# JARVIS-MoCap/JARVIS-HybridNet

Hardware: AMD Instinct MI355X
Metric: multi-view frames/s (12cam 1280x1024, 23kpt, 64^3 grid) (higher is better)
Workload: dtype f32; 1 GPU; BASELINE configs[2]: HybridNet 12-camera 1280x1024, 23 kpts, 64^3 grid, small/small; cameras=12, joints=23, grid=64, streams=3, parallelism=single GPU, 3 time batches in flight on 3 HIP streams, hipgraph=False

## Files before the change

include/jarvis_hip.h:

```cpp
#ifndef JARVIS_HIP_H
#define JARVIS_HIP_H
#include <stdint.h>

#ifdef __cplusplus
extern "C" {
#endif

#define JH_ABI_VERSION 4

const char* jh_last_error(void);
int jh_abi_version(void);

#define JH_PRECISION_DEFAULT (-1)
#define JH_PRECISION_F32 0
#define JH_PRECISION_BF16X3 1
#define JH_PRECISION_BF16X3_WIDE 2
int jh_set_precision(int mode);
int jh_get_precision(void);

typedef struct jh_params jh_params;
int jh_params_create(jh_params** out);
int jh_params_set(jh_params* p, const char* key, const float* host, int64_t numel);
void jh_params_destroy(jh_params* p);

typedef struct jh_efftrack jh_efftrack;
int jh_efftrack_create(const jh_params* p, const char* prefix, int model_size, int joints, int n,
                       int h, int w, int want_res1, jh_efftrack** out);
int jh_efftrack_forward(jh_efftrack* net, const float* x_dev, float* res1_dev, float* res2_dev,
                        void* stream);
int64_t jh_efftrack_launches(const jh_efftrack* net);
void jh_efftrack_destroy(jh_efftrack* net);

typedef struct jh_v2v jh_v2v;
int jh_v2v_create(const jh_params* p, const char* prefix, int joints, int t, int g, jh_v2v** out);
int jh_v2v_forward(jh_v2v* net, const float* x_dev, float* y_dev, void* stream);
void jh_v2v_destroy(jh_v2v* net);

int64_t jh_reproject_workspace_bytes(int cams, int joints, int hs, int grid_size);
int jh_reproject_forward(const float* heatmaps_padded_dev, int cams, int joints, int hs,
                         const int32_t* center3d_dev, const int32_t* center_hm_dev,
                         const float* cam_dev, const float* intr_dev, const float* dist_dev,
                         int grid_size, float grid_spacing, float* vol_dev, int32_t* idx_dev,
                         void* workspace_dev, int64_t workspace_bytes, void* stream);

int64_t jh_softargmax_workspace_bytes(int t, int joints, int gh);
int jh_softargmax(const float* v2v_out_dev, int t, int joints, int gh, float grid_spacing,
                  float roi_cube_size, const int32_t* center3d_dev, float* heatmap_final_dev,
                  float* points_dev, float* conf_dev, void* workspace_dev, int64_t workspace_bytes,
                  void* stream);

int jh_reproject_point(const float* points_dev, int npoints, int cams, const float* cam_dev,
                       const float* intr_dev, const float* dist_dev, float* uv_dev, void* stream);
int64_t jh_reconstruct_workspace_bytes(int cams);
int jh_reconstruct_point(const float* points2d_dev, const float* maxvals_dev, int cams,
                         const float* cam_dev, const float* intr_dev, const float* dist_dev,
                         float* point3d_dev, void* workspace_dev, int64_t workspace_bytes,
                         void* stream);

typedef struct jh_predictor jh_predictor;
typedef struct {
  int32_t num_cameras, num_joints;
  int32_t center_size;
  int32_t bbox;
  float roi_cube_size;
  float grid_spacing;
  int32_t center_model, kp_model;
  int32_t img_h, img_w;
  int32_t time_batch;
  int32_t time_batch_3d;
  int32_t cam_lo, cam_n;
  float mean[3], std[3];
  int32_t precision;
} jh_predictor_config;

int jh_predictor_create(const jh_params* center_params, const jh_params* hybrid_params,
                        const jh_predictor_config* cfg, jh_predictor** out);
void jh_predictor_destroy(jh_predictor* pr);
int64_t jh_predictor_launches(const jh_predictor* pr);
int64_t jh_predictor_device_bytes(const jh_predictor* pr);
int jh_predictor_precision(const jh_predictor* pr);

int jh_predictor_set_calibration(jh_predictor* pr, const float* cam_dev, const float* intr_dev,
                                 const float* dist_dev, void* stream);
int jh_predictor_set_calibration_frames(jh_predictor* pr, const float* cam_dev ,
                                        const float* intr_dev , const float* dist_dev ,
                                        void* stream);

int jh_predictor_stage_center(jh_predictor* pr, const float* frames_dev, float* det_dev,
                              void* stream);
int jh_predictor_stage_keypoints(jh_predictor* pr, const float* frames_dev,
                                 const float* det_all_dev, float* heat_dev, void* stream);
int jh_predictor_stage_3d(jh_predictor* pr, const float* heat_all_dev, int t0, float* points_dev,
                          float* conf_dev, int32_t* valid_dev, void* stream);
int jh_predictor_stage_keypoints_gathered(jh_predictor* pr, const void* frames_dev, int frames_u8,
                                          const float* det_gathered_dev, int n_blocks,
                                          float* heat_dev, void* stream);
int jh_predictor_stage_3d_blocks(jh_predictor* pr, const float* heat_blocks_dev, int n_blocks,
                                 int frames_per_block, int t_off, int t0, float* points_dev,
                                 float* conf_dev, int32_t* valid_dev, void* stream);
int jh_predictor_forward(jh_predictor* pr, const float* frames_dev, float* points_dev,
                         float* conf_dev, int32_t* valid_dev, void* stream);
int jh_predictor_set_graph_replay(jh_predictor* pr, int on);
int jh_predictor_graph_replay(const jh_predictor* pr);
int jh_predictor_stage_center_u8(jh_predictor* pr, const uint8_t* frames_dev, float* det_dev,
                                 void* stream);
int jh_predictor_stage_keypoints_u8(jh_predictor* pr, const uint8_t* frames_dev,
                                    const float* det_all_dev, float* heat_dev, void* stream);
int jh_predictor_forward_u8(jh_predictor* pr, const uint8_t* frames_dev, float* points_dev,
                            float* conf_dev, int32_t* valid_dev, void* stream);

#define JH_FRAME_RGB_F32 0
#define JH_FRAME_BGR_U8 1
#define JH_FRAME_I420 2
#define JH_FRAME_NV12 3
int jh_predictor_forward_yuv(jh_predictor* pr, const uint8_t* frames_dev, int format, float* points_dev,
                             float* conf_dev, int32_t* valid_dev, void* stream);

#define JH_YUV_BT601 0
#define JH_YUV_BT709 1
#define JH_YUV_LIMITED 0
#define JH_YUV_FULL 1
typedef struct jh_yuv_surface {
  int64_t image_stride;
  int64_t y_offset, y_pitch;
  int64_t u_offset, v_offset;
  int64_t c_pitch;
  int32_t c_step;
  int32_t matrix;
  int32_t range;
  int32_t reserved;
} jh_yuv_surface;
int jh_yuv_surface_check(const jh_yuv_surface* surface, int h, int w);
int jh_predictor_forward_surface(jh_predictor* pr, const uint8_t* frames_dev, const jh_yuv_surface* surface,
                                 const uint8_t* mask_dev, float* points_dev, float* conf_dev, int32_t* valid_dev,
                                 void* stream);

#define JH_SENSOR_MONO 0
#define JH_SENSOR_RGGB 1
#define JH_SENSOR_BGGR 2
#define JH_SENSOR_GRBG 3
#define JH_SENSOR_GBRG 4
typedef struct jh_sensor_surface {
  int64_t image_stride;
  int64_t offset, pitch;
  int32_t pattern;
  int32_t reserved;
} jh_sensor_surface;
int jh_sensor_surface_check(const jh_sensor_surface* surface, int h, int w);
int jh_predictor_forward_sensor(jh_predictor* pr, const uint8_t* frames_dev, const jh_sensor_surface* surface,
                                const uint8_t* mask_dev, float* points_dev, float* conf_dev, int32_t* valid_dev,
                                void* stream);

int jh_predictor_debug(jh_predictor* pr, float* center3d_f_dev, int32_t* center3d_i_dev,
                       int32_t* center_hm_dev, float* det_dev, void* stream);

int jh_predictor_forward_masked(jh_predictor* pr, const void* frames_dev, int format, const uint8_t* mask_dev,
                                float* points_dev, float* conf_dev, int32_t* valid_dev, void* stream);
int jh_predictor_stage_keypoints_masked(jh_predictor* pr, const void* frames_dev, int format,
                                        const float* det_all_dev, const uint8_t* mask_dev, float* heat_dev,
                                        void* stream);
int jh_predictor_stage_3d_masked(jh_predictor* pr, const float* heat_all_dev, int t0, const uint8_t* mask_dev,
                                 float* points_dev, float* conf_dev, int32_t* valid_dev, void* stream);
int jh_predictor_debug_mask(jh_predictor* pr, int32_t* n_active_dev, int32_t* num_cams_detect_dev, void* stream);

int jh_predictor_views2d(jh_predictor* pr, const float* heat_all_dev, int t0, const float* points_dev,
                         const uint8_t* mask_dev, int32_t* points2d_dev, float* conf2d_dev, float* reproj_dev,
                         float* err_dev, uint8_t* used_dev, void* stream);

#define JH_FRAME_SURFACE  4
#define JH_FRAME_SENSOR   5
int jh_predictor_forward_images(jh_predictor* pr, const void* const* images_host, int n_images, int format,
                                const jh_yuv_surface* yuv, const jh_sensor_surface* sensor, const uint8_t* mask_dev,
                                float* points_dev, float* conf_dev, int32_t* valid_dev, void* stream);

int jh_predictor_hybridnet_forward(jh_predictor* pr, const float* crops_dev,
                                   const int32_t* center_hm_dev, const int32_t* center3d_dev,
                                   float* heatmap_final_dev, float* heatmaps_padded_dev,
                                   float* points_dev, float* conf_dev, void* stream);

typedef struct jh_predictor2d jh_predictor2d;
int jh_predictor2d_create(const jh_params* center_params, const jh_params* kp_params,
                          const jh_predictor_config* cfg, jh_predictor2d** out);
void jh_predictor2d_destroy(jh_predictor2d* pr);
int jh_predictor2d_forward(jh_predictor2d* pr, const float* frames_dev, int32_t* points_dev,
                           float* conf_dev, int32_t* valid_dev, void* stream);
int jh_predictor2d_forward_u8(jh_predictor2d* pr, const uint8_t* frames_dev, int32_t* points_dev,
                              float* conf_dev, int32_t* valid_dev, void* stream);

int jh_predictor2d_forward_yuv(jh_predictor2d* pr, const uint8_t* frames_dev, int format, int32_t* points_dev,
                               float* conf_dev, int32_t* valid_dev, void* stream);
int jh_predictor2d_forward_surface(jh_predictor2d* pr, const uint8_t* frames_dev, const jh_yuv_surface* surface,
                                   int32_t* points_dev, float* conf_dev, int32_t* valid_dev, void* stream);
int jh_predictor2d_forward_sensor(jh_predictor2d* pr, const uint8_t* frames_dev, const jh_sensor_surface* surface,
                                  int32_t* points_dev, float* conf_dev, int32_t* valid_dev, void* stream);

int jh_predictor2d_forward_images(jh_predictor2d* pr, const void* const* images_host, int n_images, int format,
                                  const jh_yuv_surface* yuv, const jh_sensor_surface* sensor,
                                  int32_t* points_dev, float* conf_dev, int32_t* valid_dev, void* stream);

int jh_profile_begin(void);
int jh_profile_end(int* n_records);
int jh_profile_get(int i, char* name, int name_cap, double* ms, double* flops, double* bytes);

int jh_op_conv(int nd, int kind, int k, int stride, int pad, int cin, int cout,
               const float* w_host, const float* b_host, const float* x_dev, int n, int d, int h,
               int w, const float* gate_dev, int norm_act, float* y_dev, void* stream);
int jh_op_depthwise(int k, int c, const float* w_host, const float* x_dev, int n, int h, int w,
                    int norm_act, float* y_dev, void* stream);
int jh_op_depthwise_pool(int k, int c, const float* w_host, const float* x_dev, int n, int h, int w,
                         float* y_dev, float* pool_dev, void* stream);

int jh_op_yuv420_to_bgr(const uint8_t* frames_dev, int format, int n, int h, int w, uint8_t* out_bgr_dev,
                        void* stream);
int jh_op_yuv_surface_to_bgr(const uint8_t* frames_dev, const jh_yuv_surface* surface, int n, int h, int w,
                             uint8_t* out_bgr_dev, void* stream);
int jh_op_sensor_to_bgr(const uint8_t* frames_dev, const jh_sensor_surface* surface, int n, int h, int w,
                        uint8_t* out_bgr_dev, void* stream);

int64_t jh_joint_argmax_all_workspace_bytes(int n, int hh, int wh, int jp);
int jh_op_joint_argmax_all(const float* heat_dev, int n, int hh, int wh, int j, int jp, int32_t* idx_dev,
                           float* max_dev, void* workspace_dev, int64_t workspace_bytes, void* stream);

int jh_op_bifpn_node(int n_in, const int* modes, const float* weights, int act, int n, int c, int cout,
                     int h, int w, const float* x0_dev, const float* x1_dev, const float* x2_dev,
                     const float* dw_host, const float* pw_host, const float* bias_host, float* y_dev,
                     void* stream);

#ifdef __cplusplus
}
#endif
#endif
```

jarvis-hybridnet_amd/_native.py:

```python
import ctypes
import math
import os
from typing import NamedTuple

import torch

_HERE = os.path.dirname(os.path.abspath(__file__))
LIB_PATH = os.environ.get("JH_LIBRARY_PATH") or os.path.join(_HERE, "libjarvis_hip.so")
_lib = None

c_void_p, c_int, c_float, c_int64 = ctypes.c_void_p, ctypes.c_int, ctypes.c_float, ctypes.c_int64
c_char_p = ctypes.c_char_p


class PredictorConfig(ctypes.Structure):
    _fields_ = [("num_cameras", ctypes.c_int32), ("num_joints", ctypes.c_int32),
                ("center_size", ctypes.c_int32), ("bbox", ctypes.c_int32),
                ("roi_cube_size", c_float), ("grid_spacing", c_float),
                ("center_model", ctypes.c_int32), ("kp_model", ctypes.c_int32),
                ("img_h", ctypes.c_int32), ("img_w", ctypes.c_int32),
                ("time_batch", ctypes.c_int32), ("time_batch_3d", ctypes.c_int32),
                ("cam_lo", ctypes.c_int32),
                ("cam_n", ctypes.c_int32), ("mean", c_float * 3), ("std", c_float * 3),
                ("precision", ctypes.c_int32)]


class YuvSurfaceStruct(ctypes.Structure):
    _fields_ = [("image_stride", ctypes.c_int64), ("y_offset", ctypes.c_int64), ("y_pitch", ctypes.c_int64),
                ("u_offset", ctypes.c_int64), ("v_offset", ctypes.c_int64), ("c_pitch", ctypes.c_int64),
                ("c_step", ctypes.c_int32), ("matrix", ctypes.c_int32), ("range", ctypes.c_int32),
                ("reserved", ctypes.c_int32)]


assert ctypes.sizeof(YuvSurfaceStruct) == 64


class SensorSurfaceStruct(ctypes.Structure):
    _fields_ = [("image_stride", ctypes.c_int64), ("offset", ctypes.c_int64), ("pitch", ctypes.c_int64),
                ("pattern", ctypes.c_int32), ("reserved", ctypes.c_int32)]


assert ctypes.sizeof(SensorSurfaceStruct) == 32

ABI_VERSION = 4
assert ctypes.sizeof(PredictorConfig) == 84

_WORKSPACES = {}


def workspace(nbytes, device):
    key = (str(device), torch.cuda.current_stream(device).cuda_stream)
    bufs = _WORKSPACES.setdefault(key, [])
    if not bufs or bufs[-1].numel() < nbytes:
        bufs.append(torch.empty((max(int(nbytes), 256),), dtype=torch.uint8, device=device))
    return bufs[-1]


_SIGS = {
    "jh_last_error": (c_char_p, []),
    "jh_abi_version": (c_int, []),
    "jh_set_precision": (c_int, [c_int]),
    "jh_get_precision": (c_int, []),
    "jh_params_create": (c_int, [ctypes.POINTER(c_void_p)]),
    "jh_params_set": (c_int, [c_void_p, c_char_p, c_void_p, c_int64]),
    "jh_params_destroy": (None, [c_void_p]),
    "jh_efftrack_create": (c_int, [c_void_p, c_char_p, c_int, c_int, c_int, c_int, c_int, c_int,
                                   ctypes.POINTER(c_void_p)]),
    "jh_efftrack_forward": (c_int, [c_void_p, c_void_p, c_void_p, c_void_p, c_void_p]),
    "jh_efftrack_launches": (c_int64, [c_void_p]),
    "jh_efftrack_destroy": (None, [c_void_p]),
    "jh_v2v_create": (c_int, [c_void_p, c_char_p, c_int, c_int, c_int, ctypes.POINTER(c_void_p)]),
    "jh_v2v_forward": (c_int, [c_void_p, c_void_p, c_void_p, c_void_p]),
    "jh_v2v_destroy": (None, [c_void_p]),
    "jh_reproject_workspace_bytes": (c_int64, [c_int, c_int, c_int, c_int]),
    "jh_reproject_forward": (c_int, [c_void_p, c_int, c_int, c_int, c_void_p, c_void_p, c_void_p,
                                     c_void_p, c_void_p, c_int, c_float, c_void_p, c_void_p,
                                     c_void_p, c_int64, c_void_p]),
    "jh_softargmax_workspace_bytes": (c_int64, [c_int, c_int, c_int]),
    "jh_softargmax": (c_int, [c_void_p, c_int, c_int, c_int, c_float, c_float, c_void_p, c_void_p,
                              c_void_p, c_void_p, c_void_p, c_int64, c_void_p]),
    "jh_reproject_point": (c_int, [c_void_p, c_int, c_int, c_void_p, c_void_p, c_void_p, c_void_p,
                                   c_void_p]),
    "jh_reconstruct_workspace_bytes": (c_int64, [c_int]),
    "jh_reconstruct_point": (c_int, [c_void_p, c_void_p, c_int, c_void_p, c_void_p, c_void_p,
                                     c_void_p, c_void_p, c_int64, c_void_p]),
    "jh_predictor_create": (c_int, [c_void_p, c_void_p, ctypes.POINTER(PredictorConfig),
                                    ctypes.POINTER(c_void_p)]),
    "jh_predictor_destroy": (None, [c_void_p]),
    "jh_predictor_set_graph_replay": (c_int, [c_void_p, c_int]),
    "jh_predictor_graph_replay": (c_int, [c_void_p]),
    "jh_predictor_launches": (c_int64, [c_void_p]),
    "jh_predictor_device_bytes": (c_int64, [c_void_p]),
    "jh_predictor_precision": (c_int, [c_void_p]),
    "jh_predictor_set_calibration": (c_int, [c_void_p, c_void_p, c_void_p, c_void_p, c_void_p]),
    "jh_predictor_set_calibration_frames": (c_int, [c_void_p, c_void_p, c_void_p, c_void_p, c_void_p]),
    "jh_predictor_stage_center": (c_int, [c_void_p, c_void_p, c_void_p, c_void_p]),
    "jh_predictor_stage_keypoints": (c_int, [c_void_p, c_void_p, c_void_p, c_void_p, c_void_p]),
    "jh_predictor_stage_3d": (c_int, [c_void_p, c_void_p, c_int, c_void_p, c_void_p, c_void_p,
                                      c_void_p]),
    "jh_predictor_stage_keypoints_gathered": (c_int, [c_void_p, c_void_p, c_int, c_void_p, c_int, c_void_p,
                                                      c_void_p]),
    "jh_predictor_stage_3d_blocks": (c_int, [c_void_p, c_void_p, c_int, c_int, c_int, c_int, c_void_p,
                                             c_void_p, c_void_p, c_void_p]),
    "jh_profile_begin": (c_int, []),
    "jh_profile_end": (c_int, [ctypes.POINTER(c_int)]),
    "jh_profile_get": (c_int, [c_int, c_char_p, c_int, ctypes.POINTER(ctypes.c_double),
                               ctypes.POINTER(ctypes.c_double), ctypes.POINTER(ctypes.c_double)]),
    "jh_predictor_forward": (c_int, [c_void_p, c_void_p, c_void_p, c_void_p, c_void_p, c_void_p]),
    "jh_predictor_stage_center_u8": (c_int, [c_void_p, c_void_p, c_void_p, c_void_p]),
    "jh_predictor_stage_keypoints_u8": (c_int, [c_void_p, c_void_p, c_void_p, c_void_p, c_void_p]),
    "jh_predictor_forward_u8": (c_int, [c_void_p, c_void_p, c_void_p, c_void_p, c_void_p, c_void_p]),
    "jh_predictor_forward_yuv": (c_int, [c_void_p, c_void_p, c_int, c_void_p, c_void_p, c_void_p, c_void_p]),
    "jh_yuv_surface_check": (c_int, [ctypes.POINTER(YuvSurfaceStruct), c_int, c_int]),
    "jh_predictor_forward_surface": (c_int, [c_void_p, c_void_p, ctypes.POINTER(YuvSurfaceStruct), c_void_p, c_void_p,
                                             c_void_p, c_void_p, c_void_p]),
    "jh_predictor2d_forward_surface": (c_int, [c_void_p, c_void_p, ctypes.POINTER(YuvSurfaceStruct), c_void_p,
                                               c_void_p, c_void_p, c_void_p]),
    "jh_op_yuv_surface_to_bgr": (c_int, [c_void_p, ctypes.POINTER(YuvSurfaceStruct), c_int, c_int, c_int, c_void_p,
                                         c_void_p]),
    "jh_sensor_surface_check": (c_int, [ctypes.POINTER(SensorSurfaceStruct), c_int, c_int]),
    "jh_predictor_forward_sensor": (c_int, [c_void_p, c_void_p, ctypes.POINTER(SensorSurfaceStruct), c_void_p, c_void_p,
                                            c_void_p, c_void_p, c_void_p]),
    "jh_predictor2d_forward_sensor": (c_int, [c_void_p, c_void_p, ctypes.POINTER(SensorSurfaceStruct), c_void_p,
                                              c_void_p, c_void_p, c_void_p]),
    "jh_op_sensor_to_bgr": (c_int, [c_void_p, ctypes.POINTER(SensorSurfaceStruct), c_int, c_int, c_int, c_void_p,
                                    c_void_p]),
    "jh_predictor_forward_masked": (c_int, [c_void_p, c_void_p, c_int, c_void_p, c_void_p, c_void_p, c_void_p,
                                            c_void_p]),
    "jh_predictor_forward_images": (c_int, [c_void_p, ctypes.POINTER(c_void_p), c_int, c_int,
                                            ctypes.POINTER(YuvSurfaceStruct), ctypes.POINTER(SensorSurfaceStruct),
                                            c_void_p, c_void_p, c_void_p, c_void_p, c_void_p]),
    "jh_predictor2d_forward_images": (c_int, [c_void_p, ctypes.POINTER(c_void_p), c_int, c_int,
                                              ctypes.POINTER(YuvSurfaceStruct), ctypes.POINTER(SensorSurfaceStruct),
                                              c_void_p, c_void_p, c_void_p, c_void_p]),
    "jh_predictor_stage_keypoints_masked": (c_int, [c_void_p, c_void_p, c_int, c_void_p, c_void_p, c_void_p,
                                                    c_void_p]),
    "jh_predictor_stage_3d_masked": (c_int, [c_void_p, c_void_p, c_int, c_void_p, c_void_p, c_void_p, c_void_p,
                                             c_void_p]),
    "jh_predictor_debug_mask": (c_int, [c_void_p, c_void_p, c_void_p, c_void_p]),
    "jh_predictor_views2d": (c_int, [c_void_p, c_void_p, c_int] + [c_void_p] * 8),
    "jh_joint_argmax_all_workspace_bytes": (c_int64, [c_int, c_int, c_int, c_int]),
    "jh_op_joint_argmax_all": (c_int, [c_void_p, c_int, c_int, c_int, c_int, c_int, c_void_p, c_void_p, c_void_p,
                                       c_int64, c_void_p]),
    "jh_predictor2d_create": (c_int, [c_void_p, c_void_p, ctypes.POINTER(PredictorConfig),
                                      ctypes.POINTER(c_void_p)]),
    "jh_predictor2d_destroy": (None, [c_void_p]),
    "jh_predictor2d_forward": (c_int, [c_void_p] * 6),
    "jh_predictor2d_forward_u8": (c_int, [c_void_p] * 6),
    "jh_predictor2d_forward_yuv": (c_int, [c_void_p, c_void_p, c_int, c_void_p, c_void_p, c_void_p, c_void_p]),
    "jh_predictor_debug": (c_int, [c_void_p, c_void_p, c_void_p, c_void_p, c_void_p, c_void_p]),
    "jh_predictor_hybridnet_forward": (c_int, [c_void_p] * 9),
    "jh_op_conv": (c_int, [c_int] * 7 + [c_void_p, c_void_p, c_void_p] + [c_int] * 4 +
                   [c_void_p, c_int, c_void_p, c_void_p]),
    "jh_op_depthwise": (c_int, [c_int, c_int, c_void_p, c_void_p, c_int, c_int, c_int, c_int,
                                c_void_p, c_void_p]),
    "jh_op_depthwise_pool": (c_int, [c_int, c_int, c_void_p, c_void_p, c_int, c_int, c_int, c_void_p, c_void_p,
                                     c_void_p]),
    "jh_op_yuv420_to_bgr": (c_int, [c_void_p, c_int, c_int, c_int, c_int, c_void_p, c_void_p]),
    "jh_op_bifpn_node": (c_int, [c_int, ctypes.POINTER(c_int), ctypes.POINTER(c_float), c_int, c_int, c_int,
                                 c_int, c_int, c_int, c_void_p, c_void_p, c_void_p, c_void_p, c_void_p,
                                 c_void_p, c_void_p, c_void_p]),
}


def symbols():
    return sorted(_SIGS)


def lib():
    global _lib
    if _lib is None:
        if not os.path.isfile(LIB_PATH):
            raise RuntimeError(
                "jarvis_hybridnet_amd: %s is missing -- build it with "
                "`python -c 'import __graft_entry__ as g; g.build()'` (hipcc, gfx950). "
                "There is no CPU fallback." % LIB_PATH)
        handle = ctypes.CDLL(LIB_PATH)
        for name, (res, args) in _SIGS.items():
            fn = getattr(handle, name)
            fn.restype, fn.argtypes = res, args
        if handle.jh_abi_version() != ABI_VERSION:
            raise RuntimeError("libjarvis_hip.so ABI version mismatch")
        _lib = handle
    return _lib


FRAME_CODES = {"rgb": 0, "bgr": 1, "i420": 2, "nv12": 3, "surface": 4, "sensor": 5}
FRAME_FORMATS = {k: FRAME_CODES[k] for k in ("bgr", "i420", "nv12")}
YUV_FORMATS = ("i420", "nv12")
FRAME_SURFACE, FRAME_SENSOR = FRAME_CODES["surface"], FRAME_CODES["sensor"]


class Frames(NamedTuple):
    fmt: int
    height: int
    width: int
    layout: object
    lead: tuple
    data: object = None
    images: object = None

    @property
    def device(self):
        return self.data.device if self.images is None else self.images[0].device


def yuv_format(name):
    if name not in YUV_FORMATS:
        raise ValueError("frame_format must be one of %s, got %r" % (list(YUV_FORMATS), name))
    return name


def surface(layout):
    if layout is None:
        raise ValueError("surface must be a YuvSurface or a SensorSurface, got None")
    return layout


def check_layout(layout, frame_format=None, hw=None):
    if layout is None:
        return None
    from .sensor_surface import SensorSurface
    from .yuv_surface import YuvSurface
    if not isinstance(layout, (YuvSurface, SensorSurface)):
        raise ValueError("frame_layout must be a YuvSurface or a SensorSurface or None, got %r"
                         % (type(layout).__name__,))
    if frame_format in YUV_FORMATS:
        raise ValueError("frame_layout describes the bytes itself: do not combine it with frame_format=%r"
                         % (frame_format,))
    if hw is not None and (layout.height, layout.width) != tuple(hw):
        raise ValueError("frame_layout is %d x %d; this predictor is %d x %d" % (layout.height, layout.width, *hw))
    return layout


def describe_shape(shape, dtype, lead, frame_format=None, frame_layout=None, hw=None, error=ValueError,
                   in_place=False, at_least=False):
    if frame_format is not None and frame_format not in FRAME_FORMATS:
        raise ValueError("frame_format must be one of %s or None, got %r" % (sorted(FRAME_FORMATS), frame_format))
    layout = check_layout(frame_layout, frame_format, hw)
    H, W = hw if hw is not None else ("H", "W")
    hint = ""
    if layout is not None:
        from .sensor_surface import SensorSurface
# ... 223 lines not shown
```

jarvis-hybridnet_amd/_predictor.py:

```python
import collections
import ctypes

import torch

from . import _native as N
from . import arch


Views2D = collections.namedtuple("Views2D", "points2D confidences2D reprojections errors used")


class NativePredictor:

    def __init__(self, center_state, hybrid_state, *, num_cameras, num_joints, center_size, bbox,
                 roi_cube_size, grid_spacing, img_h, img_w, mean, std, center_model="small",
                 kp_model="small", time_batch=1, time_batch_3d=0, cam_lo=0, cam_n=None, precision=None):
        cam_n = num_cameras if cam_n is None else cam_n
        cfg = N.PredictorConfig(
            num_cameras, num_joints, center_size, bbox, float(roi_cube_size), float(grid_spacing),
            arch.SIZE_IDS[center_model], arch.SIZE_IDS[kp_model], img_h, img_w, time_batch,
            time_batch_3d, cam_lo, cam_n, (ctypes.c_float * 3)(*mean), (ctypes.c_float * 3)(*std),
            N.precision_id(precision))
        self.cfg = cfg
        self.T, self.C, self.Cloc, self.J = time_batch, num_cameras, cam_n, num_joints
        self.T3 = time_batch_3d if time_batch_3d > 0 else time_batch
        self.Jp = (num_joints + 7) // 8 * 8
        self.Hh = bbox // 2
        self.handle = ctypes.c_void_p()
        pc = N.Params(center_state) if center_state is not None else None
        ph = N.Params(hybrid_state)
        N.check(N.lib().jh_predictor_create(pc.handle if pc else None, ph.handle,
                                            ctypes.byref(cfg), ctypes.byref(self.handle)))
        self.precision = {v: k for k, v in N.PRECISIONS.items()}[N.lib().jh_predictor_precision(self.handle)]
        self.launches = N.lib().jh_predictor_launches(self.handle)
        self.device_bytes = N.lib().jh_predictor_device_bytes(self.handle)

    def close(self):
        if getattr(self, "handle", None) and N is not None and N._lib is not None:
            N.lib().jh_predictor_destroy(self.handle)
            self.handle = None

    __del__ = close

    @property
    def graph_replay(self):
        return bool(N.lib().jh_predictor_graph_replay(self.handle))

    @graph_replay.setter
    def graph_replay(self, on):
        N.check(N.lib().jh_predictor_set_graph_replay(self.handle, int(bool(on))))

    def set_calibration(self, cam, intr, dist):
        N.check(N.lib().jh_predictor_set_calibration(
            self.handle, N.ptr(N.dev(cam)), N.ptr(N.dev(intr)), N.ptr(N.dev(dist)), N.stream()))

    def set_calibration_frames(self, cam, intr, dist):
        form, cam, intr, dist = N.calibration((cam, intr, dist), self.T, self.C)
        if form != "frames":
            raise ValueError("set_calibration_frames takes (%d, %d, 4, 3) / (%d, %d, 3, 3) / (%d, %d, 1, 5) tensors; "
                             "got %s" % (self.T, self.C, self.T, self.C, self.T, self.C, tuple(cam.shape)))
        N.check(N.lib().jh_predictor_set_calibration_frames(
            self.handle, N.ptr(N.dev(cam)), N.ptr(N.dev(intr)), N.ptr(N.dev(dist)), N.stream()))

    def forward(self, frames, out=None, frame_format=None, camera_mask=None, frame_layout=None):
        return self._forward(self._describe(frames, frame_format, frame_layout), out,
                             N.camera_mask(camera_mask, (self.T, self.C)))

    def forward_images(self, frames, out=None, camera_mask=None):
        if len(frames.images) != self.T * self.C:
            raise ValueError("expected %d images (time_batch * num_cameras), got %d" % (self.T * self.C,
                                                                                         len(frames.images)))
        return self._forward(frames, out, N.camera_mask(camera_mask, (self.T, self.C)))

    def _describe(self, frames, frame_format=None, frame_layout=None):
        return N.describe_frames(frames, (self.T, self.Cloc), frame_format, frame_layout,
                                 (self.cfg.img_h, self.cfg.img_w), error=RuntimeError, in_place=True)

    def _forward(self, frames, out, mask):
        dev = frames.device
        if out is None:
            out = (torch.empty((self.T, self.J, 3), device=dev),
                   torch.empty((self.T, self.J), device=dev),
                   torch.empty((self.T,), device=dev, dtype=torch.int32))
        if mask is not None:
            mask = mask.to(dev, non_blocking=True)
        N.call_forward("jh_predictor", self.handle, frames, mask, out)
        if mask is not None and mask.is_cuda:
            mask.record_stream(torch.cuda.current_stream())
        return out

    def stage_center(self, frames, det):
        frames = self._describe(frames).data
        fn = N.lib().jh_predictor_stage_center_u8 if frames.dtype == torch.uint8 else \
            N.lib().jh_predictor_stage_center
        N.check(fn(self.handle, N.ptr(frames), N.ptr(det), N.stream()))

    def stage_keypoints(self, frames, det_all, heat, camera_mask=None):
        frames = self._describe(frames).data
        if camera_mask is not None:
            mask = self._device_mask(camera_mask)
            N.check(N.lib().jh_predictor_stage_keypoints_masked(
                self.handle, N.ptr(frames), int(frames.dtype == torch.uint8), N.ptr(det_all), N.ptr(mask), N.ptr(heat),
                N.stream()))
            return
        fn = N.lib().jh_predictor_stage_keypoints_u8 if frames.dtype == torch.uint8 else \
            N.lib().jh_predictor_stage_keypoints
        N.check(fn(self.handle, N.ptr(frames), N.ptr(det_all), N.ptr(heat), N.stream()))

    def _device_mask(self, camera_mask):
        if not (torch.is_tensor(camera_mask) and camera_mask.is_cuda and camera_mask.dtype == torch.uint8
                and camera_mask.is_contiguous() and tuple(camera_mask.shape) == (self.T, self.C)):
            raise ValueError("the staged calls take camera_mask as a contiguous (%d, %d) uint8 device tensor"
                             % (self.T, self.C))
        return camera_mask

    def stage_3d(self, heat_all, t0, points, conf, valid, camera_mask=None):
        if camera_mask is not None:
            mask = self._device_mask(camera_mask)
            N.check(N.lib().jh_predictor_stage_3d_masked(self.handle, N.ptr(heat_all), t0, N.ptr(mask), N.ptr(points),
                                                         N.ptr(conf), N.ptr(valid), N.stream()))
            return
        N.check(N.lib().jh_predictor_stage_3d(self.handle, N.ptr(heat_all), t0, N.ptr(points),
                                              N.ptr(conf), N.ptr(valid), N.stream()))

    def stage_keypoints_gathered(self, frames, det_gathered, n_blocks, heat):
        frames = self._describe(frames).data
        N.check(N.lib().jh_predictor_stage_keypoints_gathered(
            self.handle, N.ptr(frames), int(frames.dtype == torch.uint8), N.ptr(det_gathered), n_blocks,
            N.ptr(heat), N.stream()))

    def stage_3d_blocks(self, heat_blocks, n_blocks, frames_per_block, t_off, t0, points, conf, valid):
        N.check(N.lib().jh_predictor_stage_3d_blocks(
            self.handle, N.ptr(heat_blocks), n_blocks, frames_per_block, t_off, t0, N.ptr(points),
            N.ptr(conf), N.ptr(valid), N.stream()))

    def views2d(self, points, heat=None, t0=0, camera_mask=None, out=None):
        dev, T3 = points.device, self.T3
        if not (points.is_cuda and points.is_contiguous() and points.dtype == torch.float32
                and tuple(points.shape) == (T3, self.J, 3)):
            raise ValueError("points must be the contiguous (%d, %d, 3) float32 device tensor of the 3D stage" % (T3, self.J))
        if heat is not None and not (heat.is_cuda and heat.is_contiguous() and heat.dtype == torch.float32 and
                                     tuple(heat.shape) == (T3, self.C, self.Hh, self.Hh, self.Jp)):
            raise ValueError("heat must be a contiguous (%d, %d, %d, %d, %d) float32 device tensor"
                             % (T3, self.C, self.Hh, self.Hh, self.Jp))
        mask = N.camera_mask(camera_mask, (self.T, self.C))
        if mask is not None:
            mask = mask.to(dev, non_blocking=True)
        if out is None:
            out = Views2D(torch.empty((T3, self.C, self.J, 2), device=dev, dtype=torch.int32),
                          torch.empty((T3, self.C, self.J), device=dev),
                          torch.empty((T3, self.C, self.J, 2), device=dev),
                          torch.empty((T3, self.C, self.J), device=dev),
                          torch.empty((T3, self.C), device=dev, dtype=torch.uint8))
        N.check(N.lib().jh_predictor_views2d(self.handle, N.ptr(heat), int(t0), N.ptr(points), N.ptr(mask),
                                             *(N.ptr(t) for t in out), N.stream()))
        if mask is not None:
            mask.record_stream(torch.cuda.current_stream())
        return Views2D(*out)

    def debug(self, device):
        c3f = torch.empty((self.T, 3), device=device)
        c3i = torch.empty((self.T, 3), device=device, dtype=torch.int32)
        chm = torch.empty((self.T, self.C, 2), device=device, dtype=torch.int32)
        det = torch.empty((self.T, self.C, 3), device=device)
        N.check(N.lib().jh_predictor_debug(self.handle, N.ptr(c3f), N.ptr(c3i), N.ptr(chm),
                                           N.ptr(det), N.stream()))
        return dict(center3d=c3f, center3d_int=c3i, center_hm=chm, det=det)

    def debug_mask(self, device):
        n_act = torch.empty((self.T,), device=device, dtype=torch.int32)
        n_det = torch.empty((self.T,), device=device, dtype=torch.int32)
        N.check(N.lib().jh_predictor_debug_mask(self.handle, N.ptr(n_act), N.ptr(n_det), N.stream()))
        return dict(n_active=n_act, num_cams_detect=n_det)

    def hybridnet_forward(self, crops, center_hm, center3d, want_final=True, want_padded=True):
        dev = crops.device
        Gh = int(self.cfg.roi_cube_size / self.cfg.grid_spacing) // 2
        hs = self.Hh + 2
        final = torch.empty((self.T, self.J, Gh, Gh, Gh), device=dev) if want_final else None
        padded = torch.empty((self.T, self.C, self.J, hs, hs), device=dev) if want_padded else None
        pts = torch.empty((self.T, self.J, 3), device=dev)
        conf = torch.empty((self.T, self.J), device=dev)
        N.check(N.lib().jh_predictor_hybridnet_forward(
            self.handle, N.ptr(crops), N.ptr(center_hm), N.ptr(center3d), N.ptr(final),
            N.ptr(padded), N.ptr(pts), N.ptr(conf), N.stream()))
        return final, padded, pts, conf


class MultiStreamPredictor:

    def __init__(self, make_predictor, streams=3, timing=False):
        self.timing = timing
        self.preds = [make_predictor() for _ in range(streams)]
        self.streams = [torch.cuda.Stream() for _ in range(streams)]
        self.events = [None] * streams
        self._next = 0
        self._calib = None
        self._calib_of = [None] * streams

    def set_calibration(self, *calib):
        p0 = self.preds[0]
        form = N.calibration(calib, p0.T, p0.C)[0] if len(calib) == 3 and calib[0].dim() == 4 else "shared"
        key = (form,) + tuple((t.data_ptr(), t._version, tuple(t.shape)) for t in calib)
# ... 59 lines not shown
```

jarvis-hybridnet_amd/csrc/api.hip:

```cpp
#include <cstring>
#include <memory>
#include "../../include/jarvis_hip.h"
#include <cstdlib>
#include "nets.h"
#include "bifpn_node.h"
#include "camera_mask.h"
#include "views2d.h"

namespace jh {
static thread_local std::string g_err;
void set_error(const std::string& msg) { g_err = msg; }
}

using namespace jh;

struct jh_params { ParamMap map; };
struct jh_efftrack { EffTrackPlan plan; };
struct jh_v2v { V2VPlan plan; };

namespace {

struct Scratch {
  std::vector<void*> ptrs;
  ~Scratch() { for (void* p : ptrs) (void)hipFree(p); }
// ... 8 lines not shown
  }
};

struct Carver {
  char* base;
  size_t cap, off = 0;
  Carver(void* b, size_t c) : base(static_cast<char*>(b)), cap(c) {}
  template <typename T> T* take(size_t count) {
    const size_t at = off;
    off += (count * sizeof(T) + 255) / 256 * 256;
    return base ? reinterpret_cast<T*>(base + at) : nullptr;
  }
  void act(int N, int D, int H, int W, int C, Act* a) {
    a->N = N; a->D = D; a->H = H; a->W = W; a->C = C; a->Cp = cpad(C);
    a->p = take<float>(a->elems());
  }
  bool fits() const { return off <= cap; }
};

struct ReproWs { Act heat, vol; float2* coarse; };
static size_t carve_reproject(Carver& c, int cams, int joints, int hs, int g, ReproWs* w) {
  const int gh = g / 2;
  c.act(cams, 1, hs, hs, joints, &w->heat);
  c.act(1, g, g, g, joints, &w->vol);
  w->coarse = c.take<float2>((size_t)cams * gh * gh * gh);
  return c.off;
}
struct SoftWs { Act x; double* partial; int* pmax; };
static size_t carve_softargmax(Carver& c, int t, int joints, int gh, SoftWs* w) {
  c.act(t, gh, gh, gh, joints, &w->x);
  w->partial = c.take<double>((size_t)t * w->x.Cp * 4 * kLimbs);
  w->pmax = c.take<int>((size_t)t * w->x.Cp);
  return c.off;
}
struct ReconWs { float* det; int *c3i, *chm, *valid; };
static size_t carve_reconstruct(Carver& c, int cams, ReconWs* w) {
  w->det = c.take<float>((size_t)cams * 3);
  w->c3i = c.take<int>(3);
  w->chm = c.take<int>((size_t)cams * 2);
  w->valid = c.take<int>(1);
  return c.off;
}

__global__ void export_padded_kernel(const float* __restrict__ heat, float* __restrict__ out, int N,
                                     int J, int Jp, int Hh) {
  const int hs = Hh + 2;
  const size_t total = (size_t)N * J * hs * hs;
  for (size_t i = (size_t)blockIdx.x * blockDim.x + threadIdx.x; i < total;
       i += (size_t)gridDim.x * blockDim.x) {
    const int x = (int)(i % hs), y = (int)((i / hs) % hs);
    const int j = (int)((i / ((size_t)hs * hs)) % J);
    const size_t n = i / ((size_t)hs * hs * J);
    float v = 0.f;
    if (x >= 1 && y >= 1 && x <= Hh && y <= Hh)
      v = heat[((n * Hh + (y - 1)) * Hh + (x - 1)) * Jp + j];
    out[i] = v;
  }
}

__global__ void det_unblock_kernel(const float* __restrict__ src, float* __restrict__ dst, int T, int C,
                                   int cpb) {
  const int i = blockIdx.x * blockDim.x + threadIdx.x;
  if (i >= T * C * 3) return;
  const int k = i % 3, c = (i / 3) % C, t = i / (3 * C);
  dst[i] = src[(((size_t)(c / cpb) * T + t) * cpb + c % cpb) * 3 + k];
}

__global__ void set_cell_kernel(const void** cell, const void* value) { *cell = value; }
constexpr int kPtrChunk = 256;
struct PtrChunk { const void* p[kPtrChunk]; };
__global__ __launch_bounds__(kPtrChunk) void set_table_kernel(const void** table, int count, PtrChunk c) {
  const int i = threadIdx.x;
  if (i < count) table[i] = c.p[i];
}
__global__ void copy_out_kernel(const float* __restrict__ gp, const float* __restrict__ gc,
                                const int* __restrict__ gv, float* __restrict__ points,
                                float* __restrict__ conf, int* __restrict__ valid, int n_pts, int n_conf,
                                int n_valid) {
  const int i = blockIdx.x * blockDim.x + threadIdx.x;
  if (i < n_pts) points[i] = gp[i];
  if (i < n_conf) conf[i] = gc[i];
  if (valid && i < n_valid) valid[i] = gv[i];
}

__global__ void pack_det_kernel(const float* __restrict__ pts2d, const float* __restrict__ maxvals,
                                float* __restrict__ det, int C) {
  const int c = threadIdx.x;
  if (c < C) {
    det[c * 3 + 0] = pts2d[c];
    det[c * 3 + 1] = pts2d[C + c];
    det[c * 3 + 2] = maxvals[c];
  }
}

}

extern "C" {

const char* jh_last_error(void) { return g_err.c_str(); }
int jh_abi_version(void) { return JH_ABI_VERSION; }

int jh_set_precision(int mode) {
  JH_REQUIRE(mode == JH_PRECISION_F32 || mode == JH_PRECISION_BF16X3 || mode == JH_PRECISION_BF16X3_WIDE,
             "unknown precision mode");
  set_precision_mode(mode);
  return 0;
}
int jh_get_precision(void) { return precision_mode(); }

int jh_params_create(jh_params** out) {
  *out = new jh_params();
  return 0;
}
int jh_params_set(jh_params* p, const char* key, const float* host, int64_t numel) {
  JH_REQUIRE(p && key && host && numel >= 0, "bad argument");
  p->map[key] = std::vector<float>(host, host + numel);
  return 0;
}
void jh_params_destroy(jh_params* p) { delete p; }

int jh_efftrack_create(const jh_params* p, const char* prefix, int model_size, int joints, int n,
                       int h, int w, int want_res1, jh_efftrack** out) {
  JH_REQUIRE(p && out, "bad argument");
  std::unique_ptr<jh_efftrack> net(new jh_efftrack());
  if (net->plan.build(p->map, prefix ? prefix : "", model_size, joints, n, h, w, want_res1 != 0)) return 1;
  *out = net.release();
  return 0;
}
int jh_efftrack_forward(jh_efftrack* net, const float* x_dev, float* res1_dev, float* res2_dev,
                        void* stream) {
  hipStream_t s = static_cast<hipStream_t>(stream);
  JH_REQUIRE(net && x_dev && res2_dev, "bad argument");
  JH_REQUIRE(!res1_dev || net->plan.res1.p, "res1 requested from a network created with want_res1 = 0");
  if (launch_to_channel_last(x_dev, net->plan.input, s)) return 1;
  if (net->plan.run(s)) return 1;
  if (res1_dev && launch_from_channel_last(net->plan.res1, res1_dev, s)) return 1;
  return launch_from_channel_last(net->plan.heat, res2_dev, s);
}
int64_t jh_efftrack_launches(const jh_efftrack* net) { return (int64_t)net->plan.launches(); }
void jh_efftrack_destroy(jh_efftrack* net) { delete net; }

int jh_v2v_create(const jh_params* p, const char* prefix, int joints, int t, int g, jh_v2v** out) {
  JH_REQUIRE(p && out, "bad argument");
  std::unique_ptr<jh_v2v> net(new jh_v2v());
  if (net->plan.build(p->map, prefix ? prefix : "", joints, t, g)) return 1;
  *out = net.release();
  return 0;
}
int jh_v2v_forward(jh_v2v* net, const float* x_dev, float* y_dev, void* stream) {
  hipStream_t s = static_cast<hipStream_t>(stream);
  if (launch_to_channel_last(x_dev, net->plan.input, s)) return 1;
  if (net->plan.run(s)) return 1;
  return launch_from_channel_last(net->plan.output, y_dev, s);
}
void jh_v2v_destroy(jh_v2v* net) { delete net; }

int64_t jh_reproject_workspace_bytes(int cams, int joints, int hs, int grid_size) {
  Carver c(nullptr, 0);
  ReproWs w;
  return (int64_t)carve_reproject(c, cams, joints, hs, grid_size, &w);
}

int jh_reproject_forward(const float* heatmaps_padded_dev, int cams, int joints, int hs,
                         const int32_t* center3d_dev, const int32_t* center_hm_dev,
                         const float* cam_dev, const float* intr_dev, const float* dist_dev,
                         int grid_size, float grid_spacing, float* vol_dev, int32_t* idx_dev,
                         void* workspace_dev, int64_t workspace_bytes, void* stream) {
  hipStream_t s = static_cast<hipStream_t>(stream);
  JH_REQUIRE(workspace_dev && workspace_bytes >= 0, "workspace (see jh_reproject_workspace_bytes)");
  JH_REQUIRE(grid_size > 0 && grid_size % 2 == 0, "grid size must be even");
  Carver c(workspace_dev, (size_t)workspace_bytes);
  ReproWs w;
  carve_reproject(c, cams, joints, hs, grid_size, &w);
  JH_REQUIRE(c.fits(), "workspace smaller than jh_reproject_workspace_bytes()");
  if (launch_to_channel_last(heatmaps_padded_dev, w.heat, s)) return 1;
  if (launch_reproject(cam_dev, intr_dev, dist_dev, 0, center3d_dev, center_hm_dev, w.heat.p, w.coarse,
                       w.vol.p, idx_dev, 1, cams, grid_size, grid_spacing, hs, w.heat.Cp,
                       1, 0, s)) return 1;
  return launch_from_channel_last(w.vol, vol_dev, s);
}

int64_t jh_softargmax_workspace_bytes(int t, int joints, int gh) {
  Carver c(nullptr, 0);
  SoftWs w;
  return (int64_t)carve_softargmax(c, t, joints, gh, &w);
}

int jh_softargmax(const float* v2v_out_dev, int t, int joints, int gh, float grid_spacing,
                  float roi_cube_size, const int32_t* center3d_dev, float* heatmap_final_dev,
                  float* points_dev, float* conf_dev, void* workspace_dev, int64_t workspace_bytes,
                  void* stream) {
  hipStream_t s = static_cast<hipStream_t>(stream);
  JH_REQUIRE(workspace_dev && workspace_bytes >= 0, "workspace (see jh_softargmax_workspace_bytes)");
  Carver c(workspace_dev, (size_t)workspace_bytes);
  SoftWs w;
  carve_softargmax(c, t, joints, gh, &w);
  JH_REQUIRE(c.fits(), "workspace smaller than jh_softargmax_workspace_bytes()");
  if (launch_to_channel_last(v2v_out_dev, w.x, s)) return 1;
  return launch_softargmax(w.x.p, center3d_dev, w.partial, w.pmax, points_dev, conf_dev,
                           heatmap_final_dev, t, joints, w.x.Cp, gh, grid_spacing, roi_cube_size, s);
}

int jh_reproject_point(const float* points_dev, int npoints, int cams, const float* cam_dev,
                       const float* intr_dev, const float* dist_dev, float* uv_dev, void* stream) {
  return launch_project_points(points_dev, cam_dev, intr_dev, dist_dev, uv_dev, npoints, cams,
                               static_cast<hipStream_t>(stream));
}

int64_t jh_reconstruct_workspace_bytes(int cams) {
  Carver c(nullptr, 0);
  ReconWs w;
  return (int64_t)carve_reconstruct(c, cams, &w);
}

int jh_reconstruct_point(const float* points2d_dev, const float* maxvals_dev, int cams,
                         const float* cam_dev, const float* intr_dev, const float* dist_dev,
                         float* point3d_dev, void* workspace_dev, int64_t workspace_bytes,
                         void* stream) {
  hipStream_t s = static_cast<hipStream_t>(stream);
  JH_REQUIRE(cams >= 1 && cams <= 64, "at most 64 cameras");
  JH_REQUIRE(workspace_dev && workspace_bytes >= 0, "workspace (see jh_reconstruct_workspace_bytes)");
  Carver c(workspace_dev, (size_t)workspace_bytes);
  ReconWs w;
  carve_reconstruct(c, cams, &w);
  JH_REQUIRE(c.fits(), "workspace smaller than jh_reconstruct_workspace_bytes()");
  hipLaunchKernelGGL(pack_det_kernel, dim3(1), dim3(64), 0, s, points2d_dev, maxvals_dev, w.det, cams);
  JH_CHECK_HIP(hipGetLastError());
  return launch_triangulate(w.det, cam_dev, intr_dev, dist_dev, 0, point3d_dev, w.c3i, w.chm, w.valid, 1,
                            cams, 1.f, 1.f, 1.f, 0, 1 << 20, 1 << 20, s);
}

}

#define JH_PROF(name, flops, bytes, call)                      \
  do {                                                         \
    Profiler& _pf = profiler();                                \
    if (_pf.on) _pf.begin(name, flops, bytes, s);              \
    if (call) return 1;                                        \
    if (_pf.on) _pf.end(s);                                    \
  } while (0)

static int yuv_surface_check(const jh_yuv_surface* sp, int h, int w) {
  JH_REQUIRE(sp, "null jh_yuv_surface");
  const jh_yuv_surface& q = *sp;
  JH_REQUIRE(h > 0 && w > 0 && h % 2 == 0 && w % 2 == 0, "YUV 4:2:0 frames need an even, positive height and width");
  JH_REQUIRE(q.c_step == 1 || q.c_step == 2, "jh_yuv_surface.c_step must be 1 (planar) or 2 (semi-planar)");
  JH_REQUIRE(q.y_pitch >= w, "jh_yuv_surface.y_pitch is smaller than the width");
  JH_REQUIRE(q.c_pitch >= (int64_t)(w / 2) * q.c_step, "jh_yuv_surface.c_pitch is smaller than a chroma row");
  JH_REQUIRE(q.y_offset >= 0 && q.u_offset >= 0 && q.v_offset >= 0 && q.image_stride >= 0,
             "jh_yuv_surface offsets must not be negative");
  if (q.c_step == 2) {
    JH_REQUIRE(q.u_offset - q.v_offset == 1 || q.v_offset - q.u_offset == 1,
               "jh_yuv_surface: semi-planar U and V are neighbouring bytes");
    JH_REQUIRE((q.u_offset < q.v_offset ? q.u_offset : q.v_offset) % 2 == 0 && q.c_pitch % 2 == 0,
               "jh_yuv_surface: a semi-planar chroma pair starts at an even offset and c_pitch is even");
  }
  const __int128 y_end = (__int128)q.y_offset + (__int128)(h - 1) * q.y_pitch + w;
  const __int128 c_span = (__int128)(h / 2 - 1) * q.c_pitch + (__int128)(w / 2 - 1) * q.c_step + 1;
  JH_REQUIRE(y_end <= q.image_stride && q.u_offset + c_span <= q.image_stride && q.v_offset + c_span <= q.image_stride,
             "jh_yuv_surface: a plane ends beyond image_stride");
  JH_REQUIRE(q.matrix == JH_YUV_BT601 || q.matrix == JH_YUV_BT709, "jh_yuv_surface.matrix: unknown");
  JH_REQUIRE(q.range == JH_YUV_LIMITED || q.range == JH_YUV_FULL, "jh_yuv_surface.range: unknown");
  JH_REQUIRE(q.reserved == 0, "jh_yuv_surface.reserved must be 0");
  return 0;
}

static int frame_source(const jh_yuv_surface* sp, int h, int w, FrameSource* out) {
  if (yuv_surface_check(sp, h, w)) return 1;
  const jh_yuv_surface& q = *sp;
  static const int k[2][2][6] = {{{16, 1220542, 1673527, 2116026, -409993, -852492},
                                  {0, 1048576, 1470104, 1858077, -360853, -748826}},
                                 {{16, 1220945, 1879825, 2215014, -223607, -558796},
                                  {0, 1048576, 1651297, 1945738, -196424, -490864}}};
  const int* c = k[q.matrix][q.range];
  SrcDesc<kSrcYuvSurface> a;
  a.image_stride = q.image_stride; a.y_offset = q.y_offset; a.y_pitch = q.y_pitch;
  a.u_offset = q.u_offset; a.v_offset = q.v_offset; a.c_pitch = q.c_pitch; a.c_step = q.c_step;
  a.pair = q.c_step == 2 && q.image_stride % 2 == 0;
  a.y0 = c[0]; a.cy = c[1]; a.cvr = c[2]; a.cub = c[3]; a.cug = c[4]; a.cvg = c[5];
  out->fmt = kSrcYuvSurface; out->desc = a;
  return 0;
}

static int sensor_surface_check(const jh_sensor_surface* sp, int h, int w) {
  JH_REQUIRE(sp, "null jh_sensor_surface");
  const jh_sensor_surface& q = *sp;
  JH_REQUIRE(h > 0 && w > 0, "raw sensor frames need a positive height and width");
  JH_REQUIRE(q.pattern >= JH_SENSOR_MONO && q.pattern <= JH_SENSOR_GBRG, "jh_sensor_surface.pattern: unknown");
  if (q.pattern != JH_SENSOR_MONO)
    JH_REQUIRE(h % 2 == 0 && w % 2 == 0 && h >= 4 && w >= 4,
               "Bayer frames need an even height and width of at least 4");
  JH_REQUIRE(q.pitch >= w, "jh_sensor_surface.pitch is smaller than the width");
  JH_REQUIRE(q.offset >= 0, "jh_sensor_surface.offset must not be negative");
  JH_REQUIRE((__int128)q.offset + (__int128)(h - 1) * q.pitch + w <= q.image_stride,
             "jh_sensor_surface: the image ends beyond image_stride");
  JH_REQUIRE(q.reserved == 0, "jh_sensor_surface.reserved must be 0");
  return 0;
}

static int frame_source(const jh_sensor_surface* sp, int h, int w, FrameSource* out) {
  if (sensor_surface_check(sp, h, w)) return 1;
  const jh_sensor_surface& q = *sp;
  SrcDesc<kSrcSensor> a;
  a.image_stride = q.image_stride; a.offset = q.offset; a.pitch = q.pitch; a.pattern = q.pattern; a.h = h; a.w = w;
  out->fmt = kSrcSensor; out->desc = a;
  return 0;
}

static_assert(JH_FRAME_RGB_F32 == kSrcRgbF32 && JH_FRAME_BGR_U8 == kSrcBgrU8 && JH_FRAME_I420 == kSrcI420 &&
                  JH_FRAME_NV12 == kSrcNV12, "frame format codes of the C ABI are preprocess.h's SRC");

static FrameSource fixed_source(int format) {
  FrameSource fs;
  fs.fmt = format;
  return fs;
}
static int frame_source(int format, int h, int w, FrameSource* out) {
  JH_REQUIRE(format >= JH_FRAME_RGB_F32 && format <= JH_FRAME_NV12, "frame format");
  if (format == JH_FRAME_I420 || format == JH_FRAME_NV12)
    JH_REQUIRE(h % 2 == 0 && w % 2 == 0, "YUV 4:2:0 frames need an even height and width");
  *out = fixed_source(format);
  return 0;
}

static_assert(JH_FRAME_SURFACE == kSrcYuvSurface && JH_FRAME_SENSOR == kSrcSensor,
              "frame format codes of the C ABI are preprocess.h's SRC");

static int images_source(int format, const jh_yuv_surface* yuv, const jh_sensor_surface* sensor, int h, int w,
                         FrameSource* out) {
  JH_REQUIRE(format >= JH_FRAME_RGB_F32 && format <= JH_FRAME_SENSOR, "forward_images: unknown frame format");
  JH_REQUIRE((yuv != nullptr) == (format == JH_FRAME_SURFACE),
             "forward_images: JH_FRAME_SURFACE, and no other format, comes with a jh_yuv_surface");
  JH_REQUIRE((sensor != nullptr) == (format == JH_FRAME_SENSOR),
             "forward_images: JH_FRAME_SENSOR, and no other format, comes with a jh_sensor_surface");
  if (format == JH_FRAME_SURFACE) {
    if (frame_source(yuv, h, w, out)) return 1;
    auto& d = std::get<SrcDesc<kSrcYuvSurface>>(out->desc);
    d.pair = d.c_step == 2;
  } else if (format == JH_FRAME_SENSOR) {
    if (frame_source(sensor, h, w, out)) return 1;
  } else if (frame_source(format, h, w, out)) {
    return 1;
  }
  out->per_image = true;
  return 0;
}

static int upload_images(Scratch& mem, const void*** table, const void* const* images_host, int n_images, int want,
                         int format, hipStream_t s) {
  JH_REQUIRE(images_host, "forward_images: null image table");
  JH_REQUIRE(n_images == want, "forward_images: n_images must be time_batch * num_cameras (2D predictor: time_batch)");
  for (int i = 0; i < n_images; ++i) {
    JH_REQUIRE(images_host[i], "forward_images: a null image pointer");
    JH_REQUIRE(format != JH_FRAME_RGB_F32 || reinterpret_cast<uintptr_t>(images_host[i]) % 4 == 0,
               "forward_images: an fp32 image that is not 4-byte aligned");
  }
  if (!*table) {
    hipStreamCaptureStatus cs = hipStreamCaptureStatusNone;
    (void)hipStreamIsCapturing(s, &cs);
    JH_REQUIRE(cs == hipStreamCaptureStatusNone, "the first forward_images call of a predictor allocates its pointer "
               "table: make it outside a stream capture");
    if (mem.get(reinterpret_cast<void**>(table), (size_t)want * sizeof(void*))) return 1;
  }
  for (int off = 0; off < n_images; off += kPtrChunk) {
    PtrChunk c{};
    const int count = n_images - off < kPtrChunk ? n_images - off : kPtrChunk;
    for (int i = 0; i < count; ++i) c.p[i] = images_host[off + i];
    hipLaunchKernelGGL(set_table_kernel, dim3(1), dim3(kPtrChunk), 0, s, *table + off, count, c);
  }
  JH_CHECK_HIP(hipGetLastError());
  return 0;
}

struct jh_predictor {
  jh_predictor_config cfg{};
  int T3 = 0;
  int T = 0, C = 0, Cloc = 0, J = 0, Jp = 0, B = 0, Hh = 0, G = 0, Gh = 0, hs = 0;
  std::unique_ptr<EffTrackPlan> center, kp;
  std::unique_ptr<V2VPlan> v2v;
  Scratch mem;
  float *cam = nullptr, *intr = nullptr, *dist = nullptr;
  float *cam_f = nullptr, *intr_f = nullptr, *dist_f = nullptr;
  int calib_fs = 0;
  const float* cam_at(int t0) const { return calib_fs ? cam_f + (size_t)t0 * calib_fs * 12 : cam; }
  const float* intr_at(int t0) const { return calib_fs ? intr_f + (size_t)t0 * calib_fs * 9 : intr; }
  const float* dist_at(int t0) const { return calib_fs ? dist_f + (size_t)t0 * calib_fs * 5 : dist; }
  float *det_all = nullptr, *c3f = nullptr;
  int *c3i_[2] = {nullptr, nullptr}, *chm_[2] = {nullptr, nullptr}, *valid_[2] = {nullptr, nullptr};
  int slot = 0;
  int* c3i_cur() const { return c3i_[slot]; }
  int* chm_cur() const { return chm_[slot]; }
  int* valid_cur() const { return valid_[slot]; }
  float2* coarse = nullptr;
  double* sa_partial = nullptr;
  int* sa_max = nullptr;
  int use_graph = 0;
  const void** frames_cell = nullptr;
  const void* const* cur_cell = nullptr;
  const void** frames_table = nullptr;
  const void* const* cell_for(const FrameSource& fs) const { return fs.per_image ? frames_table : cur_cell; }
  float *g_points = nullptr, *g_conf = nullptr;
  hipStream_t gstream = nullptr;
  static constexpr int kGraphFmts = kSrcSensor + 1;
  struct GraphSlot { hipGraphExec_t exec = nullptr; FrameSource src; int calib_fs = 0; };
  GraphSlot gslot[4 * kGraphFmts];
  unsigned char* mask_buf = nullptr;
  const unsigned char* mask_cur = nullptr;
  int *n_active = nullptr, *n_detect = nullptr;
  float* v2d_max = nullptr;
  int* v2d_idx = nullptr;
  ~jh_predictor() {
    for (auto& g : gslot) if (g.exec) (void)hipGraphExecDestroy(g.exec);
    if (gstream) (void)hipStreamDestroy(gstream);
  }

  int run_3d(const float* heat_all, int t0, float* heatmap_final, float* points, float* conf,
             hipStream_t s, const HeatLayout* layout = nullptr) {
    const double g3 = (double)G * G * G;
    if (mask_cur) {
      JH_PROF("reproject_gather_masked", 0.0, 4.0 * T3 * ((double)C * Hh * Hh * J + g3 * J),
              launch_reproject_masked(cam_at(t0), intr_at(t0), dist_at(t0), calib_fs, c3i_cur() + t0 * 3,
                                      chm_cur() + t0 * C * 2, heat_all, coarse, v2v->input.p, nullptr, T3, C, G,
                                      cfg.grid_spacing, hs, Jp,
                                      0, 1, mask_cur + (size_t)t0 * C, s, layout));
    } else {
    JH_PROF("reproject_gather", 0.0, 4.0 * T3 * ((double)C * Hh * Hh * J + g3 * J),
            launch_reproject(cam_at(t0), intr_at(t0), dist_at(t0), calib_fs, c3i_cur() + t0 * 3,
                             chm_cur() + t0 * C * 2, heat_all, coarse, v2v->input.p, nullptr, T3, C, G,
                             cfg.grid_spacing, hs, Jp,
                             0, 1, s, layout));
    }
    if (v2v->run(s)) return 1;
    JH_PROF("softargmax", 0.0, 4.0 * T3 * (g3 / 8) * J,
            launch_softargmax(v2v->output.p, c3i_cur() + t0 * 3, sa_partial, sa_max, points, conf,
                              heatmap_final, T3, J, Jp, Gh, cfg.grid_spacing, cfg.roi_cube_size, s));
    return 0;
  }
};

extern "C" {

int jh_predictor_create(const jh_params* center_params, const jh_params* hybrid_params,
                        const jh_predictor_config* cfg, jh_predictor** out) {
  JH_REQUIRE(hybrid_params && cfg && out, "bad argument");
  std::unique_ptr<jh_predictor> pr(new jh_predictor());
  pr->cfg = *cfg;
  pr->T = cfg->time_batch; pr->C = cfg->num_cameras; pr->Cloc = cfg->cam_n;
  pr->T3 = cfg->time_batch_3d > 0 ? cfg->time_batch_3d : cfg->time_batch;
  JH_REQUIRE(pr->T3 <= pr->T, "time_batch_3d must not exceed time_batch");
  pr->J = cfg->num_joints; pr->Jp = cpad(cfg->num_joints);
  pr->B = cfg->bbox; pr->Hh = cfg->bbox / 2; pr->hs = cfg->bbox / 2 + 2;
  pr->G = (int)(cfg->roi_cube_size / cfg->grid_spacing);
  pr->Gh = pr->G / 2;
  JH_REQUIRE(pr->T >= 1 && pr->C >= 1 && pr->C <= 64, "time batch / camera count");
  JH_REQUIRE(cfg->cam_lo >= 0 && cfg->cam_n >= 1 && cfg->cam_lo + cfg->cam_n <= pr->C, "camera range");
  JH_REQUIRE(pr->G % 4 == 0, "ROI_CUBE_SIZE / GRID_SPACING must be a multiple of 4");
  const int N = pr->T * pr->Cloc;
  const int node_rows = pr->T >= 8 ? 1 : 0;
  const int norm_kb = node_rows && JH_ENV_KNOB("JH_NODE_ROWS") != 0 ? 64 : 0;
  JH_REQUIRE(cfg->precision >= JH_PRECISION_DEFAULT && cfg->precision <= JH_PRECISION_BF16X3_WIDE,
             "jh_predictor_config.precision: unknown mode");
  const int precision = cfg->precision == JH_PRECISION_DEFAULT ? precision_mode() : cfg->precision;
  pr->cfg.precision = precision;
  if (center_params) {
    pr->center.reset(new EffTrackPlan());
    pr->center->precision = precision;
    pr->center->node_rows = node_rows;
    pr->center->norm_block_kb = norm_kb;
    if (pr->center->build(center_params->map, "", cfg->center_model, 1, N, cfg->center_size,
                          cfg->center_size)) return 1;
  }
  pr->kp.reset(new EffTrackPlan());
  pr->kp->precision = precision;
  pr->kp->node_rows = node_rows;
  pr->kp->norm_block_kb = norm_kb;
  if (pr->kp->build(hybrid_params->map, "effTrack.", cfg->kp_model, pr->J, N, pr->B, pr->B)) return 1;
  pr->v2v.reset(new V2VPlan());
  pr->v2v->precision = precision;
  pr->v2v->norm_block_kb = norm_kb;
  if (pr->v2v->build(hybrid_params->map, "v2vNet.", pr->J, pr->T3, pr->G)) return 1;
  auto& m = pr->mem;
  const int T = pr->T, C = pr->C;
  if (m.get(reinterpret_cast<void**>(&pr->cam), (size_t)C * 12 * sizeof(float))) return 1;
  if (m.get(reinterpret_cast<void**>(&pr->intr), (size_t)C * 9 * sizeof(float))) return 1;
  if (m.get(reinterpret_cast<void**>(&pr->dist), (size_t)C * 5 * sizeof(float))) return 1;
  if (m.get(reinterpret_cast<void**>(&pr->det_all), (size_t)T * C * 3 * sizeof(float))) return 1;
  if (m.get(reinterpret_cast<void**>(&pr->c3f), (size_t)T * 3 * sizeof(float))) return 1;
  for (int k = 0; k < 2; ++k) {
    if (m.get(reinterpret_cast<void**>(&pr->c3i_[k]), (size_t)T * 3 * sizeof(int))) return 1;
    if (m.get(reinterpret_cast<void**>(&pr->chm_[k]), (size_t)T * C * 2 * sizeof(int))) return 1;
    if (m.get(reinterpret_cast<void**>(&pr->valid_[k]), (size_t)T * sizeof(int))) return 1;
  }
  if (m.get(reinterpret_cast<void**>(&pr->coarse),
            (size_t)pr->T3 * C * pr->Gh * pr->Gh * pr->Gh * sizeof(float2))) return 1;
  {
    const size_t pb = (size_t)T * pr->Jp * 4 * kLimbs * sizeof(double), mb = (size_t)T * pr->Jp * sizeof(int);
    if (m.get(reinterpret_cast<void**>(&pr->sa_partial), pb + mb)) return 1;
    pr->sa_max = reinterpret_cast<int*>(reinterpret_cast<char*>(pr->sa_partial) + pb);
  }
  for (int k = 0; k < 2; ++k) JH_CHECK_HIP(hipMemset(pr->valid_[k], 0, (size_t)T * sizeof(int)));
  if (m.get(reinterpret_cast<void**>(&pr->mask_buf), (size_t)T * C)) return 1;
  if (m.get(reinterpret_cast<void**>(&pr->n_active), (size_t)T * sizeof(int))) return 1;
  if (m.get(reinterpret_cast<void**>(&pr->n_detect), (size_t)T * sizeof(int))) return 1;
  JH_CHECK_HIP(hipMemset(pr->mask_buf, 1, (size_t)T * C));
  JH_CHECK_HIP(hipMemset(pr->n_active, 0, (size_t)T * sizeof(int)));
  JH_CHECK_HIP(hipMemset(pr->n_detect, 0, (size_t)T * sizeof(int)));
  const int knob = JH_ENV_KNOB("JH_GRAPH");
  pr->use_graph = knob >= 0 ? (knob != 0) : (pr->T == 1);
  if (pr->Cloc == pr->C && pr->T3 == pr->T && pr->center) {
    if (m.get(reinterpret_cast<void**>(&pr->frames_cell), 256)) return 1;
    if (m.get(reinterpret_cast<void**>(&pr->g_points), (size_t)T * pr->J * 3 * sizeof(float))) return 1;
    if (m.get(reinterpret_cast<void**>(&pr->g_conf), (size_t)T * pr->J * sizeof(float))) return 1;
  } else {
    pr->use_graph = 0;
  }
  JH_CHECK_HIP(hipDeviceSynchronize());
  *out = pr.release();
  return 0;
}

void jh_predictor_destroy(jh_predictor* pr) { delete pr; }

int jh_predictor_set_graph_replay(jh_predictor* pr, int on) {
  JH_REQUIRE(pr, "bad argument");
  JH_REQUIRE(!on || pr->frames_cell, "graph replay needs a predictor that owns all cameras and CenterDetect");
  pr->use_graph = on != 0;
  return 0;
}
int jh_predictor_graph_replay(const jh_predictor* pr) { return pr ? pr->use_graph : 0; }

int64_t jh_predictor_launches(const jh_predictor* pr) {
  return (int64_t)((pr->center ? pr->center->launches() : 0) + pr->kp->launches() +
                   pr->v2v->launches());
}
int jh_predictor_precision(const jh_predictor* pr) { return pr ? pr->cfg.precision : -1; }

int64_t jh_predictor_device_bytes(const jh_predictor* pr) {
  return (int64_t)((pr->center ? pr->center->device_bytes() : 0) + pr->kp->device_bytes() +
                   pr->v2v->device_bytes());
}

int jh_predictor_set_calibration(jh_predictor* pr, const float* cam_dev, const float* intr_dev,
                                 const float* dist_dev, void* stream) {
  hipStream_t s = static_cast<hipStream_t>(stream);
  JH_CHECK_HIP(hipMemcpyAsync(pr->cam, cam_dev, (size_t)pr->C * 12 * sizeof(float), hipMemcpyDeviceToDevice, s));
  JH_CHECK_HIP(hipMemcpyAsync(pr->intr, intr_dev, (size_t)pr->C * 9 * sizeof(float), hipMemcpyDeviceToDevice, s));
  JH_CHECK_HIP(hipMemcpyAsync(pr->dist, dist_dev, (size_t)pr->C * 5 * sizeof(float), hipMemcpyDeviceToDevice, s));
  pr->calib_fs = 0;
  return 0;
}

int jh_predictor_set_calibration_frames(jh_predictor* pr, const float* cam_dev, const float* intr_dev,
                                        const float* dist_dev, void* stream) {
  hipStream_t s = static_cast<hipStream_t>(stream);
  JH_REQUIRE(pr, "jh_predictor_set_calibration_frames: null predictor");
  JH_REQUIRE(cam_dev && intr_dev && dist_dev, "jh_predictor_set_calibration_frames: null calibration pointer");
  const size_t rows = (size_t)pr->T * pr->C;
  if (!pr->cam_f) {
    hipStreamCaptureStatus cs = hipStreamCaptureStatusNone;
    (void)hipStreamIsCapturing(s, &cs);
    JH_REQUIRE(cs == hipStreamCaptureStatusNone, "the first jh_predictor_set_calibration_frames call of a predictor "
               "allocates its per-frame calibration: make it outside a stream capture");
    float* base = nullptr;
    if (pr->mem.get(reinterpret_cast<void**>(&base), rows * 26 * sizeof(float))) return 1;
    pr->intr_f = base + rows * 12;
    pr->dist_f = base + rows * 21;
    pr->cam_f = base;
  }
  JH_CHECK_HIP(hipMemcpyAsync(pr->cam_f, cam_dev, rows * 12 * sizeof(float), hipMemcpyDeviceToDevice, s));
  JH_CHECK_HIP(hipMemcpyAsync(pr->intr_f, intr_dev, rows * 9 * sizeof(float), hipMemcpyDeviceToDevice, s));
  JH_CHECK_HIP(hipMemcpyAsync(pr->dist_f, dist_dev, rows * 5 * sizeof(float), hipMemcpyDeviceToDevice, s));
  pr->calib_fs = pr->C;
  return 0;
}

static int stage_center_impl(jh_predictor* pr, const void* frames_dev, const FrameSource& fs, float* det_dev,
                             void* stream) {
  hipStream_t s = static_cast<hipStream_t>(stream);
  JH_REQUIRE(pr->center, "predictor was created without CenterDetect weights");
  const int N = pr->T * pr->Cloc, S = pr->cfg.center_size;
  if (pr->center->stem_fusable) {
    StemSource& src = pr->center->stem_src;
    src.mode = 1; src.frames = frames_dev; src.frames_cell = pr->cell_for(fs); src.source = fs;
    src.H = pr->cfg.img_h; src.W = pr->cfg.img_w;
    for (int i = 0; i < 3; ++i) { src.mean[i] = pr->cfg.mean[i]; src.stdv[i] = pr->cfg.std[i]; }
    pr->center->set_stem_traffic((double)N * S * S * (4.0 * fs.px_bytes() + pr->center->stem_channels()));
  } else {
    JH_PROF("preprocess_resize", 0.0, (double)N * S * S * (4.0 * fs.px_bytes() + 3 * 4),
            launch_preprocess_resize(frames_dev, fs, pr->center->input.p, N, pr->cfg.img_h,
                                     pr->cfg.img_w, S, pr->cfg.mean, pr->cfg.std, s, pr->cell_for(fs)));
  }
  if (pr->center->run(s)) return 1;
  const Act& h = pr->center->heat;
  JH_PROF("center_argmax", 0.0, 4.0 * N * h.H * h.W,
          launch_center_argmax(h.p, det_dev, N, h.H, h.W, h.Cp, s));
  return 0;
}

int jh_predictor_stage_center(jh_predictor* pr, const float* frames_dev, float* det_dev,
                              void* stream) {
  return stage_center_impl(pr, frames_dev, fixed_source(kSrcRgbF32), det_dev, stream);
}
int jh_predictor_stage_center_u8(jh_predictor* pr, const uint8_t* frames_dev, float* det_dev,
                                 void* stream) {
  return stage_center_impl(pr, frames_dev, fixed_source(kSrcBgrU8), det_dev, stream);
}

static int stage_keypoints_impl(jh_predictor* pr, const void* frames_dev, const FrameSource& fs,
                                const float* det_all_dev, float* heat_dev, void* stream,
                                int det_blocks = 1, bool next_centre_set = false) {
  hipStream_t s = static_cast<hipStream_t>(stream);
  const auto& c = pr->cfg;
  if (next_centre_set) pr->slot ^= 1;
  if (det_blocks > 1) {
    JH_REQUIRE(pr->C % det_blocks == 0, "cameras must divide evenly over the detection blocks");
    const int n = pr->T * pr->C * 3;
    hipLaunchKernelGGL(det_unblock_kernel, dim3((n + 255) / 256), dim3(256), 0, s, det_all_dev, pr->det_all,
                       pr->T, pr->C, pr->C / det_blocks);
    JH_CHECK_HIP(hipGetLastError());
    det_all_dev = pr->det_all;
  }
  const float sx2 = (float)((double)c.img_w / (double)c.center_size) * 2.f;
  const float sy2 = (float)((double)c.img_h / (double)c.center_size) * 2.f;
  if (pr->mask_cur) {
    JH_PROF("triangulate_masked", 0.0, 0.0,
            launch_triangulate_masked(det_all_dev, pr->cam_at(0), pr->intr_at(0), pr->dist_at(0), pr->calib_fs, pr->c3f,
                                      pr->c3i_cur(), pr->chm_cur(), pr->valid_cur(), pr->T, pr->C, sx2, sy2, 255.f,
                                      pr->B / 2,
                                      c.img_w, c.img_h, pr->mask_cur, pr->n_active, pr->n_detect, s));
  } else {
  JH_PROF("triangulate", 0.0, 0.0,
          launch_triangulate(det_all_dev, pr->cam_at(0), pr->intr_at(0), pr->dist_at(0), pr->calib_fs, pr->c3f,
                             pr->c3i_cur(), pr->chm_cur(), pr->valid_cur(), pr->T, pr->C, sx2, sy2, 255.f, pr->B / 2,
                             c.img_w, c.img_h, s));
  }
  if (det_all_dev != pr->det_all)
    JH_CHECK_HIP(hipMemcpyAsync(pr->det_all, det_all_dev, (size_t)pr->T * pr->C * 3 * sizeof(float),
                                hipMemcpyDeviceToDevice, s));
  if (pr->kp->stem_fusable) {
    StemSource& src = pr->kp->stem_src;
    src.mode = 2; src.frames = frames_dev; src.frames_cell = pr->cell_for(fs); src.source = fs;
    src.center_hm = pr->chm_cur(); src.Cloc = pr->Cloc; src.C = pr->C; src.cam0 = c.cam_lo;
    src.H = c.img_h; src.W = c.img_w;
    for (int i = 0; i < 3; ++i) { src.mean[i] = c.mean[i]; src.stdv[i] = c.std[i]; }
    pr->kp->set_stem_traffic((double)pr->T * pr->Cloc * pr->B * pr->B * (fs.px_bytes() + pr->kp->stem_channels()));
  } else {
    JH_PROF("preprocess_crop", 0.0, (double)pr->T * pr->Cloc * pr->B * pr->B * (fs.px_bytes() + 12.0),
            launch_preprocess_crop(frames_dev, fs, pr->chm_cur(), pr->kp->input.p, pr->T, pr->Cloc, pr->C,
                                   c.cam_lo, c.img_h, c.img_w, pr->B, c.mean, c.std, s, pr->cell_for(fs)));
  }
  if (pr->kp->run(s)) return 1;
  if (heat_dev && heat_dev != pr->kp->heat.p)
    JH_CHECK_HIP(hipMemcpyAsync(heat_dev, pr->kp->heat.p, pr->kp->heat.bytes(),
                                hipMemcpyDeviceToDevice, s));
  return 0;
}

int jh_predictor_stage_keypoints(jh_predictor* pr, const float* frames_dev,
                                 const float* det_all_dev, float* heat_dev, void* stream) {
  return stage_keypoints_impl(pr, frames_dev, fixed_source(kSrcRgbF32), det_all_dev, heat_dev, stream, 1, true);
}
int jh_predictor_stage_keypoints_u8(jh_predictor* pr, const uint8_t* frames_dev,
                                    const float* det_all_dev, float* heat_dev, void* stream) {
  return stage_keypoints_impl(pr, frames_dev, fixed_source(kSrcBgrU8), det_all_dev, heat_dev, stream, 1, true);
}

int jh_predictor_stage_keypoints_gathered(jh_predictor* pr, const void* frames_dev, int frames_u8,
                                          const float* det_gathered_dev, int n_blocks, float* heat_dev,
                                          void* stream) {
  JH_REQUIRE(n_blocks >= 1, "block count");
  return stage_keypoints_impl(pr, frames_dev, fixed_source(frames_u8 ? kSrcBgrU8 : kSrcRgbF32), det_gathered_dev, heat_dev,
                              stream, n_blocks, true);
}

int jh_predictor_stage_3d(jh_predictor* pr, const float* heat_all_dev, int t0, float* points_dev,
                          float* conf_dev, int32_t* valid_dev, void* stream) {
  hipStream_t s = static_cast<hipStream_t>(stream);
  JH_REQUIRE(t0 >= 0 && t0 + pr->T3 <= pr->T, "frame range of the 3D stage");
  if (pr->run_3d(heat_all_dev, t0, nullptr, points_dev, conf_dev, s)) return 1;
  if (valid_dev)
    JH_CHECK_HIP(hipMemcpyAsync(valid_dev, pr->valid_cur() + t0, (size_t)pr->T3 * sizeof(int),
                                hipMemcpyDeviceToDevice, s));
  return 0;
}

int jh_predictor_stage_3d_blocks(jh_predictor* pr, const float* heat_blocks_dev, int n_blocks,
                                 int frames_per_block, int t_off, int t0, float* points_dev,
                                 float* conf_dev, int32_t* valid_dev, void* stream) {
  hipStream_t s = static_cast<hipStream_t>(stream);
  JH_REQUIRE(t0 >= 0 && t0 + pr->T3 <= pr->T, "frame range of the 3D stage");
  JH_REQUIRE(n_blocks >= 1 && pr->C % n_blocks == 0, "cameras must divide evenly over the blocks");
  JH_REQUIRE(t_off >= 0 && t_off + pr->T3 <= frames_per_block, "frame range inside a block");
  HeatLayout lay;
  const size_t plane = (size_t)pr->Hh * pr->Hh * pr->Jp;
  lay.cams_per_block = pr->C / n_blocks;
  lay.frame_stride = (size_t)lay.cams_per_block * plane;
  lay.block_stride = (size_t)frames_per_block * lay.frame_stride;
  if (pr->run_3d(heat_blocks_dev + (size_t)t_off * lay.frame_stride, t0, nullptr, points_dev, conf_dev, s,
                 &lay)) return 1;
  if (valid_dev)
    JH_CHECK_HIP(hipMemcpyAsync(valid_dev, pr->valid_cur() + t0, (size_t)pr->T3 * sizeof(int),
                                hipMemcpyDeviceToDevice, s));
  return 0;
}

static int forward_eager(jh_predictor* pr, const void* frames_dev, const FrameSource& fs, float* points_dev,
                         float* conf_dev, int32_t* valid_dev, void* stream) {
  if (stage_center_impl(pr, frames_dev, fs, pr->det_all, stream)) return 1;
  if (stage_keypoints_impl(pr, frames_dev, fs, pr->det_all, nullptr, stream)) return 1;
  return jh_predictor_stage_3d(pr, pr->kp->heat.p, 0, points_dev, conf_dev, valid_dev, stream);
}

static int forward_graph(jh_predictor* pr, const void* frames_dev, const FrameSource& fs, float* points_dev,
                         float* conf_dev, int32_t* valid_dev, hipStream_t s) {
  jh_predictor::GraphSlot& slot = pr->gslot[fs.fmt + (pr->mask_cur ? jh_predictor::kGraphFmts : 0) +
                                            (fs.per_image ? 2 * jh_predictor::kGraphFmts : 0)];
  if (slot.exec && (slot.src != fs || slot.calib_fs != pr->calib_fs)) {
    JH_CHECK_HIP(hipStreamSynchronize(s));
    (void)hipGraphExecDestroy(slot.exec);
    slot.exec = nullptr;
  }
  if (!slot.exec) {
    hipGraph_t g = nullptr;
    if (!pr->gstream) JH_CHECK_HIP(hipStreamCreateWithFlags(&pr->gstream, hipStreamNonBlocking));
    JH_CHECK_HIP(hipStreamBeginCapture(pr->gstream, hipStreamCaptureModeRelaxed));
    pr->cur_cell = pr->frames_cell;
    const int rc = forward_eager(pr, nullptr, fs, pr->g_points, pr->g_conf, nullptr, pr->gstream);
    pr->cur_cell = nullptr;
    const hipError_t e = hipStreamEndCapture(pr->gstream, &g);
    if (rc) { if (g) (void)hipGraphDestroy(g); return 1; }
    JH_CHECK_HIP(e);
    const hipError_t ei = hipGraphInstantiate(&slot.exec, g, nullptr, nullptr, 0);
    (void)hipGraphDestroy(g);
    if (ei != hipSuccess) slot.exec = nullptr;
    JH_CHECK_HIP(ei);
    slot.src = fs;
    slot.calib_fs = pr->calib_fs;
  }
  if (!fs.per_image) hipLaunchKernelGGL(set_cell_kernel, dim3(1), dim3(1), 0, s, pr->frames_cell, frames_dev);
  JH_CHECK_HIP(hipGetLastError());
  JH_CHECK_HIP(hipGraphLaunch(slot.exec, s));
  const int n_pts = pr->T * pr->J * 3;
  hipLaunchKernelGGL(copy_out_kernel, dim3((n_pts + 255) / 256), dim3(256), 0, s, pr->g_points, pr->g_conf,
                     pr->valid_[0], points_dev, conf_dev, valid_dev, n_pts, pr->T * pr->J, pr->T);
  JH_CHECK_HIP(hipGetLastError());
  return 0;
}

static int forward_unmasked(jh_predictor* pr, const void* frames_dev, const FrameSource& fs, float* points_dev,
                            float* conf_dev, int32_t* valid_dev, void* stream) {
  JH_REQUIRE(pr->Cloc == pr->C && pr->cfg.cam_lo == 0, "forward needs all cameras local");
  JH_REQUIRE(pr->T3 == pr->T, "forward needs time_batch_3d == time_batch");
  JH_REQUIRE(frames_dev && points_dev && conf_dev, "null frame / output pointer");
  pr->slot = 0;
  hipStreamCaptureStatus cs = hipStreamCaptureStatusNone;
  if (pr->use_graph && !profiler().on) (void)hipStreamIsCapturing(static_cast<hipStream_t>(stream), &cs);
  if (!pr->use_graph || profiler().on || cs != hipStreamCaptureStatusNone)
    return forward_eager(pr, frames_dev, fs, points_dev, conf_dev, valid_dev, stream);
  return forward_graph(pr, frames_dev, fs, points_dev, conf_dev, valid_dev, static_cast<hipStream_t>(stream));
}

static int forward_impl(jh_predictor* pr, const void* frames_dev, const FrameSource& fs, float* points_dev,
                        float* conf_dev, int32_t* valid_dev, void* stream,
                        const unsigned char* mask_dev = nullptr) {
  if (!mask_dev) return forward_unmasked(pr, frames_dev, fs, points_dev, conf_dev, valid_dev, stream);
  JH_CHECK_HIP(hipMemcpyAsync(pr->mask_buf, mask_dev, (size_t)pr->T * pr->C, hipMemcpyDeviceToDevice,
                              static_cast<hipStream_t>(stream)));
  pr->mask_cur = pr->mask_buf;
  const int rc = forward_unmasked(pr, frames_dev, fs, points_dev, conf_dev, valid_dev, stream);
  pr->mask_cur = nullptr;
  return rc;
}
int jh_predictor_forward(jh_predictor* pr, const float* frames_dev, float* points_dev,
                         float* conf_dev, int32_t* valid_dev, void* stream) {
  return forward_impl(pr, frames_dev, fixed_source(kSrcRgbF32), points_dev, conf_dev, valid_dev, stream);
}
int jh_predictor_forward_u8(jh_predictor* pr, const uint8_t* frames_dev, float* points_dev,
                            float* conf_dev, int32_t* valid_dev, void* stream) {
  return forward_impl(pr, frames_dev, fixed_source(kSrcBgrU8), points_dev, conf_dev, valid_dev, stream);
}

int jh_predictor_forward_yuv(jh_predictor* pr, const uint8_t* frames_dev, int format, float* points_dev,
                             float* conf_dev, int32_t* valid_dev, void* stream) {
  JH_REQUIRE(format == JH_FRAME_I420 || format == JH_FRAME_NV12, "jh_predictor_forward_yuv: format must be "
             "JH_FRAME_I420 or JH_FRAME_NV12");
  JH_REQUIRE(pr, "bad argument");
  FrameSource fs;
  if (frame_source(format, pr->cfg.img_h, pr->cfg.img_w, &fs)) return 1;
  return forward_impl(pr, frames_dev, fs, points_dev, conf_dev, valid_dev, stream);
}

int jh_yuv_surface_check(const jh_yuv_surface* surface, int h, int w) { return yuv_surface_check(surface, h, w); }

int jh_predictor_forward_surface(jh_predictor* pr, const uint8_t* frames_dev, const jh_yuv_surface* surface,
                                 const uint8_t* mask_dev, float* points_dev, float* conf_dev, int32_t* valid_dev,
                                 void* stream) {
  JH_REQUIRE(pr, "bad argument");
  FrameSource fs;
  if (frame_source(surface, pr->cfg.img_h, pr->cfg.img_w, &fs)) return 1;
  return forward_impl(pr, frames_dev, fs, points_dev, conf_dev, valid_dev, stream, mask_dev);
}

int jh_sensor_surface_check(const jh_sensor_surface* surface, int h, int w) {
  return sensor_surface_check(surface, h, w);
}

int jh_predictor_forward_sensor(jh_predictor* pr, const uint8_t* frames_dev, const jh_sensor_surface* surface,
                                const uint8_t* mask_dev, float* points_dev, float* conf_dev, int32_t* valid_dev,
                                void* stream) {
  JH_REQUIRE(pr, "bad argument");
  FrameSource fs;
  if (frame_source(surface, pr->cfg.img_h, pr->cfg.img_w, &fs)) return 1;
  return forward_impl(pr, frames_dev, fs, points_dev, conf_dev, valid_dev, stream, mask_dev);
}

int jh_predictor_forward_masked(jh_predictor* pr, const void* frames_dev, int format, const uint8_t* mask_dev,
                                float* points_dev, float* conf_dev, int32_t* valid_dev, void* stream) {
  JH_REQUIRE(pr, "bad argument");
  JH_REQUIRE(format >= JH_FRAME_RGB_F32 && format <= JH_FRAME_NV12, "jh_predictor_forward_masked: unknown frame format");
  FrameSource fs;
  if (frame_source(format, pr->cfg.img_h, pr->cfg.img_w, &fs)) return 1;
  return forward_impl(pr, frames_dev, fs, points_dev, conf_dev, valid_dev, stream, mask_dev);
}

int jh_predictor_forward_images(jh_predictor* pr, const void* const* images_host, int n_images, int format,
                                const jh_yuv_surface* yuv, const jh_sensor_surface* sensor, const uint8_t* mask_dev,
                                float* points_dev, float* conf_dev, int32_t* valid_dev, void* stream) {
  JH_REQUIRE(pr, "bad argument");
  JH_REQUIRE(pr->Cloc == pr->C && pr->cfg.cam_lo == 0, "forward needs all cameras local");
  FrameSource fs;
  if (images_source(format, yuv, sensor, pr->cfg.img_h, pr->cfg.img_w, &fs)) return 1;
  if (upload_images(pr->mem, &pr->frames_table, images_host, n_images, pr->T * pr->C, format,
                    static_cast<hipStream_t>(stream))) return 1;
  return forward_impl(pr, pr->frames_table, fs, points_dev, conf_dev, valid_dev, stream, mask_dev);
}

int jh_predictor_stage_keypoints_masked(jh_predictor* pr, const void* frames_dev, int format,
                                        const float* det_all_dev, const uint8_t* mask_dev, float* heat_dev,
                                        void* stream) {
  JH_REQUIRE(pr && mask_dev, "bad argument");
  JH_REQUIRE(format == JH_FRAME_RGB_F32 || format == JH_FRAME_BGR_U8, "masked stage 2: fp32 RGB or uint8 BGR frames");
  JH_REQUIRE(pr->Cloc == pr->C && pr->cfg.cam_lo == 0, "masked stage 2 needs all cameras local");
  pr->mask_cur = mask_dev;
  const int rc = stage_keypoints_impl(pr, frames_dev, fixed_source(format), det_all_dev, heat_dev, stream, 1, true);
  pr->mask_cur = nullptr;
  return rc;
}

int jh_predictor_stage_3d_masked(jh_predictor* pr, const float* heat_all_dev, int t0, const uint8_t* mask_dev,
                                 float* points_dev, float* conf_dev, int32_t* valid_dev, void* stream) {
  JH_REQUIRE(pr && mask_dev, "bad argument");
  JH_REQUIRE(pr->Cloc == pr->C && pr->cfg.cam_lo == 0, "masked stage 3 needs all cameras local");
  pr->mask_cur = mask_dev;
  const int rc = jh_predictor_stage_3d(pr, heat_all_dev, t0, points_dev, conf_dev, valid_dev, stream);
  pr->mask_cur = nullptr;
  return rc;
}

int jh_predictor_debug_mask(jh_predictor* pr, int32_t* n_active_dev, int32_t* num_cams_detect_dev, void* stream) {
  hipStream_t s = static_cast<hipStream_t>(stream);
  JH_REQUIRE(pr, "bad argument");
  const size_t T = pr->T;
  if (n_active_dev) JH_CHECK_HIP(hipMemcpyAsync(n_active_dev, pr->n_active, T * sizeof(int), hipMemcpyDeviceToDevice, s));
  if (num_cams_detect_dev) JH_CHECK_HIP(hipMemcpyAsync(num_cams_detect_dev, pr->n_detect, T * sizeof(int), hipMemcpyDeviceToDevice, s));
  return 0;
}

int jh_predictor_views2d(jh_predictor* pr, const float* heat_all_dev, int t0, const float* points_dev,
                         const uint8_t* mask_dev, int32_t* points2d_dev, float* conf2d_dev, float* reproj_dev,
                         float* err_dev, uint8_t* used_dev, void* stream) {
  hipStream_t s = static_cast<hipStream_t>(stream);
  JH_REQUIRE(pr && points_dev && points2d_dev && conf2d_dev && reproj_dev && err_dev && used_dev,
             "null pointer");
  JH_REQUIRE(t0 >= 0 && t0 + pr->T3 <= pr->T, "frame range of the 2D views");
  const int N = pr->T3 * pr->C;
  if (!heat_all_dev) {
    JH_REQUIRE(pr->Cloc == pr->C && pr->cfg.cam_lo == 0, "the predictor's own heat maps hold all cameras only when "
               "all cameras are local");
    heat_all_dev = pr->kp->heat.p + (size_t)t0 * pr->C * pr->Hh * pr->Hh * pr->Jp;
  }
  if (!pr->v2d_max) {
    hipStreamCaptureStatus cs = hipStreamCaptureStatusNone;
    (void)hipStreamIsCapturing(s, &cs);
    JH_REQUIRE(cs == hipStreamCaptureStatusNone, "the first jh_predictor_views2d call of a predictor allocates its "
               "workspace: make it outside a stream capture");
    const size_t n = joint_argmax_all_partials(N, pr->Hh, pr->Hh, pr->Jp);
    if (pr->mem.get(reinterpret_cast<void**>(&pr->v2d_max), n * sizeof(float))) return 1;
    if (pr->mem.get(reinterpret_cast<void**>(&pr->v2d_idx), n * sizeof(int))) return 1;
  }
  const double bytes = 4.0 * N * pr->Hh * pr->Hh * pr->Jp;
// ... 445 lines not shown
```

jarvis-hybridnet_amd/csrc/elementwise.hip:

```cpp
#include "jh_common.h"

namespace jh {

__device__ __forceinline__ float act_apply(float v, int act) {
  if (act == ACT_RELU) return fmaxf(v, 0.f);
  if (act == ACT_SILU) return v / (1.f + expf(-v));
  return v;
}

__device__ __forceinline__ void block_channel_reduce(float4 s1, float4 s2, int nvals, int q,
                                                     int rows, int tid, bool active,
                                                     double* dst, int dst_stride, float* sm) {
  if (active) {
    const int c4 = tid % q, r = tid / q;
    float4* p = reinterpret_cast<float4*>(sm) + ((size_t)r * q + c4) * nvals;
    p[0] = s1;
    if (nvals == 2) p[1] = s2;
  }
  __syncthreads();
  for (int i = tid; i < q * 4 * nvals; i += blockDim.x) {
    const int comp = i & 3, v = (i >> 2) % nvals, c4 = (i >> 2) / nvals;
    float acc = 0.f;
    for (int r = 0; r < rows; ++r) acc += sm[(((size_t)r * q + c4) * nvals + v) * 4 + comp];
    exact_add(dst + ((size_t)(c4 * 4 + comp) * dst_stride + v) * kLimbs, (double)acc);
  }
}

template <int ACT, bool R1, bool R2, bool Y, bool R1N = false>
__global__ __launch_bounds__(1024) void norm_apply_kernel(
    const float* __restrict__ x, const double* __restrict__ stats, double eps,
    const float* __restrict__ r1, const float* __restrict__ r2, float* __restrict__ y,
    double* __restrict__ pool, int P, int Cp, int ppb, const double* __restrict__ stats1 = nullptr) {
  extern __shared__ __attribute__((aligned(16))) float sm[];
  const int q = Cp >> 2;
  const int BT = blockDim.x;
  const int rows = BT / q;
  const int tid = threadIdx.x;
  const bool active = tid < rows * q;
  const int c4 = tid % q, row = tid / q;
  const int n = blockIdx.y;
  float4 mean = make_float4(0, 0, 0, 0), rstd = make_float4(1, 1, 1, 1);
  if (stats) {
    float* mr = sm + (pool ? rows * q * 4 : 0);
    for (int c = tid; c < Cp; c += BT) {
      const double* st = stats + ((size_t)n * Cp + c) * kStatW;
      const double mu = exact_read(st) / (double)P;
      double var = exact_read(st + kLimbs) / (double)P - mu * mu;
      if (var < 0.0) var = 0.0;
      mr[c] = (float)mu;
      mr[Cp + c] = (float)(1.0 / sqrt(var + eps));
    }
    __syncthreads();
    if (active) {
      mean = *reinterpret_cast<const float4*>(mr + c4 * 4);
      rstd = *reinterpret_cast<const float4*>(mr + Cp + c4 * 4);
    }
    __syncthreads();
  }
  float4 mean1 = make_float4(0, 0, 0, 0), rstd1 = make_float4(1, 1, 1, 1);
  if (R1N) {
    float* mr = sm + (pool ? rows * q * 4 : 0);
    for (int c = tid; c < Cp; c += BT) {
      const double* st = stats1 + ((size_t)n * Cp + c) * kStatW;
      const double mu = exact_read(st) / (double)P;
      double var = exact_read(st + kLimbs) / (double)P - mu * mu;
      if (var < 0.0) var = 0.0;
      mr[c] = (float)mu;
      mr[Cp + c] = (float)(1.0 / sqrt(var + eps));
    }
    __syncthreads();
    if (active) {
      mean1 = *reinterpret_cast<const float4*>(mr + c4 * 4);
      rstd1 = *reinterpret_cast<const float4*>(mr + Cp + c4 * 4);
    }
    __syncthreads();
  }
  const size_t base = (size_t)n * P * Cp + c4 * 4;
  const int p0 = blockIdx.x * ppb;
  const int p1 = min(P, p0 + ppb);
  float4 ps = make_float4(0, 0, 0, 0);
  auto act1 = [](float v) __attribute__((always_inline)) {
    if (ACT == ACT_RELU) return fmaxf(v, 0.f);
    if (ACT == ACT_SILU) return silu_fast(v);
    return v;
  };
  auto finish = [&](float4 v, float4 a1, float4 a2, size_t off) __attribute__((always_inline)) {
    v.x = (v.x - mean.x) * rstd.x; v.y = (v.y - mean.y) * rstd.y;
    v.z = (v.z - mean.z) * rstd.z; v.w = (v.w - mean.w) * rstd.w;
    if (R1N) {
      a1.x = fmaxf((a1.x - mean1.x) * rstd1.x, 0.f); a1.y = fmaxf((a1.y - mean1.y) * rstd1.y, 0.f);
      a1.z = fmaxf((a1.z - mean1.z) * rstd1.z, 0.f); a1.w = fmaxf((a1.w - mean1.w) * rstd1.w, 0.f);
    }
    if (R1) { v.x += a1.x; v.y += a1.y; v.z += a1.z; v.w += a1.w; }
    v.x = act1(v.x); v.y = act1(v.y); v.z = act1(v.z); v.w = act1(v.w);
    if (R2) { v.x += a2.x; v.y += a2.y; v.z += a2.z; v.w += a2.w; }
    if (Y) *reinterpret_cast<float4*>(y + off) = v;
    ps.x += v.x; ps.y += v.y; ps.z += v.z; ps.w += v.w;
  };
  if (active) {
    constexpr int UN = 4;
    int p = p0 + row;
    for (; p + (UN - 1) * rows < p1; p += UN * rows) {
      float4 v[UN], a1[UN], a2[UN];
#pragma unroll
      for (int u = 0; u < UN; ++u) {
        const size_t off = base + (size_t)(p + u * rows) * Cp;
        v[u] = *reinterpret_cast<const float4*>(x + off);
        if (R1) a1[u] = *reinterpret_cast<const float4*>(r1 + off);
        if (R2) a2[u] = *reinterpret_cast<const float4*>(r2 + off);
      }
#pragma unroll
      for (int u = 0; u < UN; ++u) finish(v[u], a1[u], a2[u], base + (size_t)(p + u * rows) * Cp);
    }
    for (; p < p1; p += rows) {
      const size_t off = base + (size_t)p * Cp;
      float4 a1 = make_float4(0, 0, 0, 0), a2 = a1;
      if (R1) a1 = *reinterpret_cast<const float4*>(r1 + off);
      if (R2) a2 = *reinterpret_cast<const float4*>(r2 + off);
      finish(*reinterpret_cast<const float4*>(x + off), a1, a2, off);
    }
  }
  if (pool)
    block_channel_reduce(ps, ps, 1, q, rows, tid, active, pool + (size_t)n * Cp * kLimbs, 1, sm);
}

int launch_norm_apply(const Act& x, const double* stats, double eps, int act, const float* r1,
                      const float* r2, float* y, double* pool, hipStream_t s, const double* r1_stats,
                      int min_block_kb) {
  const int P = (int)x.pixels();
  const int q = x.Cp / 4;
  JH_REQUIRE(q >= 1 && q <= 256, "channel count out of range for norm_apply");
  int bt = 256;
  for (int cand = 512; cand <= 1024; cand *= 2)
    if ((cand / q) * q * bt > (bt / q) * q * cand + cand * bt / 16) bt = cand;
  const int rows = bt / q;
  int iters = 8;
  while ((P + rows * iters - 1) / (rows * iters) > 64 && iters < 64) iters *= 2;
  while ((long)rows * iters * x.Cp * 4 < (long)min_block_kb * 1024 && iters < 64 && rows * iters < P) iters *= 2;
  const int ppb = rows * iters;
  dim3 grid((P + ppb - 1) / ppb, x.N);
  const size_t sm = ((pool ? (size_t)rows * q * 4 : 0) + (stats ? (size_t)2 * x.Cp : 0)) * sizeof(float);
  if (r1_stats) {
    JH_REQUIRE(stats && r1 && y && act == ACT_RELU && !pool, "norm_apply: normalised residual operand");
    if (r2)
      hipLaunchKernelGGL((norm_apply_kernel<ACT_RELU, true, true, true, true>), grid, dim3(bt), sm, s, x.p, stats, eps,
                         r1, r2, y, pool, P, x.Cp, ppb, r1_stats);
    else
      hipLaunchKernelGGL((norm_apply_kernel<ACT_RELU, true, false, true, true>), grid, dim3(bt), sm, s, x.p, stats, eps,
                         r1, r2, y, pool, P, x.Cp, ppb, r1_stats);
    JH_CHECK_HIP(hipGetLastError());
    return 0;
  }
#define JH_NA(A, B1, B2, BY)                                                                              \
  if (act == A && (r1 != nullptr) == B1 && (r2 != nullptr) == B2 && (y != nullptr) == BY) {             \
    hipLaunchKernelGGL((norm_apply_kernel<A, B1, B2, BY>), grid, dim3(bt), sm, s, x.p, stats, eps, r1, r2, y, \
                       pool, P, x.Cp, ppb, nullptr);                                                               \
    JH_CHECK_HIP(hipGetLastError());                                                                      \
    return 0;                                                                                             \
  }
#define JH_NA_ACT(A) JH_NA(A, false, false, false) JH_NA(A, false, false, true) JH_NA(A, true, false, true) \
                     JH_NA(A, true, true, true) JH_NA(A, false, true, true)
  JH_NA_ACT(ACT_NONE) JH_NA_ACT(ACT_RELU) JH_NA_ACT(ACT_SILU)
#undef JH_NA_ACT
#undef JH_NA
  JH_REQUIRE(false, "norm_apply: residual inputs without an output tensor");
}

__global__ __launch_bounds__(256) void se_gate_kernel(
    const double* __restrict__ pool, int C, int Cp, int S, float inv_hw,
    const float* __restrict__ wr, const float* __restrict__ br, const float* __restrict__ we,
    const float* __restrict__ be, float* __restrict__ gate) {
  extern __shared__ __attribute__((aligned(16))) float sm[];
  float* mean = sm;
  float* hid = sm + C;
  const int n = blockIdx.x;
  for (int c = threadIdx.x; c < C; c += blockDim.x)
    mean[c] = (float)(exact_read(pool + ((size_t)n * Cp + c) * kLimbs) * (double)inv_hw);
  __syncthreads();
  for (int j = threadIdx.x; j < S; j += blockDim.x) {
    float acc = br[j];
    for (int c = 0; c < C; ++c) acc = fmaf(wr[j * C + c], mean[c], acc);
    hid[j] = acc / (1.f + expf(-acc));
  }
  __syncthreads();
  for (int c = threadIdx.x; c < Cp; c += blockDim.x) {
    float g = 0.f;
    if (c < C) {
      float acc = be[c];
      for (int j = 0; j < S; ++j) acc = fmaf(we[c * S + j], hid[j], acc);
      g = 1.f / (1.f + expf(-acc));
    }
    gate[(size_t)n * Cp + c] = g;
  }
}

int launch_se_gate(const double* pool, int N, int C, int Cp, int S, float inv_hw, const float* wr,
                   const float* br, const float* we, const float* be, float* gate,
                   hipStream_t s) {
  hipLaunchKernelGGL(se_gate_kernel, dim3(N), dim3(256), (C + S) * sizeof(float), s, pool, C, Cp,
                     S, inv_hw, wr, br, we, be, gate);
  JH_CHECK_HIP(hipGetLastError());
  return 0;
}

template <int K, int CC, bool POOL = false, int TT = 16>
__global__ __launch_bounds__(256) void depthwise_lds_kernel(
    const float* __restrict__ x, const float* __restrict__ w, float* __restrict__ y,
    double* __restrict__ stats, int H, int W, int Cp, double* __restrict__ pool = nullptr) {
  constexpr int T = TT, HT = T + K - 1, SP = CC + 4;
  static_assert(T % 4 == 0, "tiles are made of 4-pixel strips");
  constexpr int QN = CC / 4, SL = 256 / QN;
  constexpr int QS = QN == 8 ? 3 : 2;
  static_assert(CC == 32 || CC == 16, "channel chunk");
  extern __shared__ __attribute__((aligned(16))) float sm[];
  float* wl = sm + HT * HT * SP;
  const int tid = threadIdx.x;
  const int tiles_x = (W + T - 1) / T;
  const BlockId bid = xcd_block();
  const int ox0 = (bid.x % tiles_x) * T, oy0 = (bid.x / tiles_x) * T;
  const int c0 = bid.y * CC;
  const int n = bid.z;
  const int q = min(CC, Cp - c0) >> 2;
  typedef float df2 __attribute__((ext_vector_type(2)));
  typedef float df4 __attribute__((ext_vector_type(4)));
  const int lc4 = tid & (QN - 1), slot = tid >> QS;
  df4 wv = (df4){0.f, 0.f, 0.f, 0.f};
  if (tid < K * K * QN && lc4 < q)
    wv = *reinterpret_cast<const df4*>(w + (size_t)(tid >> QS) * Cp + c0 + lc4 * 4);
  const __amdgpu_buffer_rsrc_t rs = __builtin_amdgcn_make_buffer_rsrc(
      const_cast<float*>(x + (size_t)n * H * W * Cp), 0, (int)((size_t)H * W * Cp * 4), 0x00020000);
  constexpr int NPX = HT * HT, ITERS = (NPX + SL - 1) / SL;
  df4 v[ITERS];
#pragma unroll
  for (int u = 0; u < ITERS; ++u) {
    const int pix = u * SL + slot;
    const int px = pix % HT, py = pix / HT;
    const int iy = oy0 + py - K / 2, ix = ox0 + px - K / 2;
    const bool ok = pix < NPX && lc4 < q && iy >= 0 && iy < H && ix >= 0 && ix < W;
    const int off = ok ? ((iy * W + ix) * Cp + c0 + lc4 * 4) * 4 : (int)0x80000000;
    v[u] = __builtin_bit_cast(df4, __builtin_amdgcn_raw_buffer_load_b128(rs, off, 0, 0));
  }
  if (tid < K * K * QN) *reinterpret_cast<df4*>(wl + (tid >> QS) * CC + lc4 * 4) = wv;
#pragma unroll
  for (int u = 0; u < ITERS; ++u) {
    const int pix = u * SL + slot;
    if (pix < NPX) *reinterpret_cast<df4*>(sm + pix * SP + lc4 * 4) = v[u];
  }
  const int c4 = tid & (QN - 1);
// ... 316 lines not shown
```

jarvis-hybridnet_amd/csrc/geometry.hip:

```cpp
#include "jh_common.h"
#include "preprocess.h"
#include "camera_mask.h"
#include "views2d.h"

namespace jh {

template <int SRC>
__global__ __launch_bounds__(256) void preprocess_resize_kernel(
    const void* __restrict__ frames, float* __restrict__ out, int N, int H, int W, int S,
    float sy, float sx, float3 mean, float3 stdv, const void* const* __restrict__ frames_cell, int per_image,
    SrcDesc<SRC> d) {
  if (frames_cell && !per_image) frames = *frames_cell;
  const size_t total = (size_t)N * S * S;
  for (size_t i = (size_t)blockIdx.x * blockDim.x + threadIdx.x; i < total;
       i += (size_t)gridDim.x * blockDim.x) {
    const int ox = (int)(i % S), oy = (int)((i / S) % S);
    int n = (int)(i / ((size_t)S * S));
    const void* base = image_base(frames, frames_cell, per_image, n);
    *reinterpret_cast<float4*>(out + i * 4) = resize_px<SRC>(base, n, oy, ox, H, W, sy, sx, mean, stdv, d);
  }
}

int launch_preprocess_resize(const void* frames, const FrameSource& src, float* out, int N, int H, int W, int S,
                             const float* mean, const float* stdv, hipStream_t s,
                             const void* const* frames_cell) {
  const size_t total = (size_t)N * S * S;
  int blocks = (int)((total + 255) / 256);
  if (blocks > 8192) blocks = 8192;
  const float3 m = make_float3(mean[0], mean[1], mean[2]), sd = make_float3(stdv[0], stdv[1], stdv[2]);
  JH_REQUIRE(!src.per_image || frames_cell, "per-image frames come with their pointer table");
  if (dispatch_src(src, [&](auto tag, const auto& d) {
        hipLaunchKernelGGL(preprocess_resize_kernel<decltype(tag)::value>, dim3(blocks), dim3(256), 0, s, frames, out,
                           N, H, W, S, (float)H / (float)S, (float)W / (float)S, m, sd, frames_cell,
                           (int)src.per_image, d);
        return 0;
      }))
    return 1;
  JH_CHECK_HIP(hipGetLastError());
  return 0;
}

template <int SRC>
__global__ __launch_bounds__(256) void preprocess_crop_kernel(
    const void* __restrict__ frames, const int* __restrict__ center_hm, float* __restrict__ out,
    int T, int Cloc, int C, int cam0, int H, int W, int B, float3 mean, float3 stdv,
    const void* const* __restrict__ frames_cell, int per_image, SrcDesc<SRC> d) {
  if (frames_cell && !per_image) frames = *frames_cell;
  const size_t total = (size_t)T * Cloc * B * B;
  for (size_t i = (size_t)blockIdx.x * blockDim.x + threadIdx.x; i < total;
       i += (size_t)gridDim.x * blockDim.x) {
    const int ox = (int)(i % B), oy = (int)((i / B) % B);
    int n = (int)(i / ((size_t)B * B));
    const int t = n / Cloc, cl = n % Cloc;
    const int cx = center_hm[(t * C + cam0 + cl) * 2 + 0], cy = center_hm[(t * C + cam0 + cl) * 2 + 1];
    const void* base = image_base(frames, frames_cell, per_image, n);
    *reinterpret_cast<float4*>(out + i * 4) = crop_px<SRC>(base, n, cx, cy, oy, ox, H, W, B, mean, stdv, d);
  }
}

int launch_preprocess_crop(const void* frames, const FrameSource& src, const int* center_hm, float* out, int T,
                           int Cloc, int C, int cam0, int H, int W, int B, const float* mean,
                           const float* stdv, hipStream_t s, const void* const* frames_cell) {
  const size_t total = (size_t)T * Cloc * B * B;
  int blocks = (int)((total + 255) / 256);
  if (blocks > 8192) blocks = 8192;
  const float3 m = make_float3(mean[0], mean[1], mean[2]), sd = make_float3(stdv[0], stdv[1], stdv[2]);
  JH_REQUIRE(!src.per_image || frames_cell, "per-image frames come with their pointer table");
  if (dispatch_src(src, [&](auto tag, const auto& d) {
        hipLaunchKernelGGL(preprocess_crop_kernel<decltype(tag)::value>, dim3(blocks), dim3(256), 0, s, frames,
                           center_hm, out, T, Cloc, C, cam0, H, W, B, m, sd, frames_cell, (int)src.per_image, d);
        return 0;
      }))
    return 1;
  JH_CHECK_HIP(hipGetLastError());
  return 0;
}

template <int SRC>
__global__ __launch_bounds__(256) void frames_to_bgr_kernel(const void* __restrict__ frames,
                                                            unsigned char* __restrict__ out, int N, int H, int W,
                                                            SrcDesc<SRC> d) {
  const size_t total = (size_t)N * H * W;
  for (size_t i = (size_t)blockIdx.x * blockDim.x + threadIdx.x; i < total;
       i += (size_t)gridDim.x * blockDim.x) {
    const int x = (int)(i % W), y = (int)((i / W) % H);
    const size_t n = i / ((size_t)H * W);
    const Rgb8 p = rgb8_px<SRC>(frames, n, y, x, H, W, d);
    out[i * 3 + 0] = (unsigned char)p.b;
    out[i * 3 + 1] = (unsigned char)p.g;
    out[i * 3 + 2] = (unsigned char)p.r;
  }
}

int launch_frames_to_bgr(const void* frames, const FrameSource& src, unsigned char* out, int N, int H, int W,
                         hipStream_t s) {
  const size_t total = (size_t)N * H * W;
  const int blocks = (int)((total + 255) / 256 < 8192 ? (total + 255) / 256 : 8192);
  JH_REQUIRE(!src.per_image, "the to-BGR helper reads contiguous frames");
  if (dispatch_src(src, [&](auto tag, const auto& d) {
        constexpr int SRC = decltype(tag)::value;
        if constexpr (!kIsRgb8<SRC>) {
          JH_REQUIRE(kIsRgb8<SRC>, "YUV 4:2:0 format");
        } else {
          if constexpr (SRC == kSrcSensor)
            JH_REQUIRE(N >= 1 && H >= 1 && W >= 1 && d.h == H && d.w == W, "raw sensor frames: image size");
          else
            JH_REQUIRE(N >= 1 && H >= 2 && W >= 2 && H % 2 == 0 && W % 2 == 0,
                       "YUV 4:2:0 frames need an even height and width");
          hipLaunchKernelGGL(frames_to_bgr_kernel<SRC>, dim3(blocks), dim3(256), 0, s, frames, out, N, H, W, d);
        }
        return 0;
      }))
    return 1;
  JH_CHECK_HIP(hipGetLastError());
  return 0;
}

__global__ __launch_bounds__(1024) void center_argmax_kernel(const float* __restrict__ heat,
                                                            float* __restrict__ det, int Hh,
                                                            int Wh, int Cp) {
  __shared__ float sv[1024];
  __shared__ int si[1024];
  const int n = blockIdx.x;
  const int P = Hh * Wh;
  const float* h = heat + (size_t)n * P * Cp;
  float best = -INFINITY;
  int bi = 0x7fffffff;
  constexpr int U = 8;
  int p = threadIdx.x;
  for (; p + (U - 1) * (int)blockDim.x < P; p += U * blockDim.x) {
    float v[U];
#pragma unroll
    for (int u = 0; u < U; ++u) v[u] = h[(size_t)(p + u * blockDim.x) * Cp];
#pragma unroll
    for (int u = 0; u < U; ++u) {
      const int pp = p + u * blockDim.x;
      if (v[u] > best || (v[u] == best && pp < bi)) { best = v[u]; bi = pp; }
    }
  }
  for (; p < P; p += blockDim.x) {
    const float v = h[(size_t)p * Cp];
    if (v > best || (v == best && p < bi)) { best = v; bi = p; }
  }
  sv[threadIdx.x] = best; si[threadIdx.x] = bi;
  __syncthreads();
  for (int s = 512; s > 0; s >>= 1) {
    if (threadIdx.x < s) {
      const float v = sv[threadIdx.x + s];
      const int ii = si[threadIdx.x + s];
      if (v > sv[threadIdx.x] || (v == sv[threadIdx.x] && ii < si[threadIdx.x])) {
        sv[threadIdx.x] = v; si[threadIdx.x] = ii;
      }
    }
    __syncthreads();
  }
  if (threadIdx.x == 0) {
// ... 316 lines not shown
      argmax_take(v[u].w, pp, best[3], bi[3]);
    }
  }
  for (; p < p1; p += rows) {
    const float4 v = h[(size_t)p * q];
    argmax_take(v.x, p, best[0], bi[0]);
    argmax_take(v.y, p, best[1], bi[1]);
    argmax_take(v.z, p, best[2], bi[2]);
    argmax_take(v.w, p, best[3], bi[3]);
  }
  *reinterpret_cast<float4*>(sv + tid * 4) = make_float4(best[0], best[1], best[2], best[3]);
  *reinterpret_cast<int4*>(si + tid * 4) = make_int4(bi[0], bi[1], bi[2], bi[3]);
  __syncthreads();
  const int parts = blockDim.x / Jp, ch = tid % Jp, part = tid / Jp;
  float b = -INFINITY;
  int i = 0x7fffffff;
  if (part < parts)
    for (int r = part; r < rows; r += parts) argmax_take(sv[r * Jp + ch], si[r * Jp + ch], b, i);
  __syncthreads();
  if (part < parts) { sv[tid] = b; si[tid] = i; }
  __syncthreads();
  if (tid < Jp) {
    for (int k = 1; k < parts; ++k) argmax_take(sv[k * Jp + tid], si[k * Jp + tid], b, i);
    const size_t o = ((size_t)n * gridDim.x + slice) * Jp + tid;
    pmax[o] = b;
    pidx[o] = i;
  }
}

__device__ __forceinline__ void argmax_combine(const float* __restrict__ pmax, const int* __restrict__ pidx,
                                               int n, int slices, int Jp, int j, float* best, int* bi) {
  float b = -INFINITY;
  int i = 0x7fffffff;
  for (int k = 0; k < slices; ++k) {
    const size_t o = ((size_t)n * slices + k) * Jp + j;
    argmax_take(pmax[o], pidx[o], b, i);
  }
  *best = b;
  *bi = i;
}

__global__ void joint_argmax_all_combine_kernel(const float* __restrict__ pmax, const int* __restrict__ pidx,
                                                int* __restrict__ idx, float* __restrict__ maxv, int slices,
                                                int J, int Jp) {
  const int n = blockIdx.x, j = threadIdx.x;
  if (j >= J) return;
  float b;
  int i;
  argmax_combine(pmax, pidx, n, slices, Jp, j, &b, &i);
  idx[(size_t)n * J + j] = i;
  maxv[(size_t)n * J + j] = b;
}

__global__ void views2d_final_kernel(const float* __restrict__ pmax, const int* __restrict__ pidx,
                                     const int* __restrict__ center_hm, const int* __restrict__ valid,
                                     const unsigned char* __restrict__ mask, const float* __restrict__ pts3d,
                                     const float* __restrict__ cam, const float* __restrict__ intr,
                                     const float* __restrict__ dist, int fs, int* __restrict__ points2d,
                                     float* __restrict__ conf2d, float* __restrict__ reproj, float* __restrict__ err,
                                     unsigned char* __restrict__ used, int C, int J, int Jp, int slices, int Hh,
                                     int Wh, int hw) {
  const int n = blockIdx.x, t = n / C, c = n % C, j = threadIdx.x;
  const bool ok = valid[t] != 0;
  const bool use = ok && (mask == nullptr || mask[(size_t)t * C + c] != 0);
  if (j == 0) used[n] = use ? 1 : 0;
  if (j >= J) return;
  const size_t o = (size_t)n * J + j;
  const float nan = __int_as_float(0x7fc00000);
  float u = nan, v = nan;
  if (ok) {
    const float* p = pts3d + ((size_t)t * J + j) * 3;
    const size_t row = (size_t)t * fs + c;
    project_one(cam + row * 12, intr + row * 9, dist + row * 5, p[0], p[1], p[2], &u, &v);
  }
  reproj[o * 2 + 0] = u;
  reproj[o * 2 + 1] = v;
  if (!use) {
    points2d[o * 2 + 0] = -1;
    points2d[o * 2 + 1] = -1;
    conf2d[o] = 0.f;
    err[o] = nan;
    return;
  }
  float b;
  int m;
  argmax_combine(pmax, pidx, n, slices, Jp, j, &b, &m);
  const int x = (m % Hh) * 2 + center_hm[(size_t)n * 2 + 0] - hw;
  const int y = (m / Wh) * 2 + center_hm[(size_t)n * 2 + 1] - hw;
  points2d[o * 2 + 0] = x;
  points2d[o * 2 + 1] = y;
  conf2d[o] = __fdiv_rn(fminf(b, 255.f), 255.f);
  const float dx = __fsub_rn(u, (float)x), dy = __fsub_rn(v, (float)y);
  err[o] = __fsqrt_rn(__fadd_rn(__fmul_rn(dx, dx), __fmul_rn(dy, dy)));
}

ScanShape joint_argmax_all_shape(int N, int Hh, int Wh, int Jp) {
  ScanShape sh;
  const int q = Jp / 4, rows = kScanThreads / q, P = Hh * Wh;
  sh.threads = rows * q;
  int steps = 4;
  while (steps > 1 && (long long)N * ((P + rows * kScanUnroll * steps - 1) / (rows * kScanUnroll * steps)) < 1024)
    steps /= 2;
  sh.ppb = rows * kScanUnroll * steps;
  sh.slices = (P + sh.ppb - 1) / sh.ppb;
  return sh;
}

size_t joint_argmax_all_partials(int N, int Hh, int Wh, int Jp) {
  return (size_t)N * joint_argmax_all_shape(N, Hh, Wh, Jp).slices * Jp;
}

static int check_scan_shape(int N, int Hh, int Wh, int J, int Jp) {
  JH_REQUIRE(N >= 1 && Hh >= 1 && Wh >= 1, "heat map shape");
  JH_REQUIRE(Jp >= 8 && Jp % 8 == 0 && Jp <= kScanThreads && J >= 1 && J <= Jp, "channel count: J <= Jp, Jp a "
             "multiple of 8 up to 256");
  JH_REQUIRE((long long)Hh * Wh < (1ll << 30) && N <= 65535, "heat map too large for the all-joint argmax");
  return 0;
}

int launch_joint_argmax_all(const float* heat, float* pmax, int* pidx, int N, int Hh, int Wh, int J, int Jp,
                            hipStream_t s) {
  if (check_scan_shape(N, Hh, Wh, J, Jp)) return 1;
  const ScanShape sh = joint_argmax_all_shape(N, Hh, Wh, Jp);
  hipLaunchKernelGGL(joint_argmax_all_kernel, dim3(sh.slices, N), dim3(sh.threads), 0, s, heat, pmax, pidx,
                     Hh * Wh, Jp, sh.ppb);
  JH_CHECK_HIP(hipGetLastError());
  return 0;
}

int launch_joint_argmax_all_combine(const float* pmax, const int* pidx, int* idx, float* maxv, int N, int Hh,
                                    int Wh, int J, int Jp, hipStream_t s) {
  if (check_scan_shape(N, Hh, Wh, J, Jp)) return 1;
  const ScanShape sh = joint_argmax_all_shape(N, Hh, Wh, Jp);
  hipLaunchKernelGGL(joint_argmax_all_combine_kernel, dim3(N), dim3(round_up(J, kWave)), 0, s, pmax, pidx, idx,
                     maxv, sh.slices, J, Jp);
  JH_CHECK_HIP(hipGetLastError());
  return 0;
}

int launch_views2d_final(const float* pmax, const int* pidx, const int* center_hm, const int* valid,
                         const unsigned char* mask, const float* pts3d, const float* cam, const float* intr,
                         const float* dist, int calib_fs, int* points2d, float* conf2d, float* reproj, float* err,
                         unsigned char* used, int T, int C, int J, int Jp, int Hh, int Wh, int hw, hipStream_t s) {
  if (check_scan_shape(T * C, Hh, Wh, J, Jp)) return 1;
  JH_REQUIRE(calib_fs == 0 || calib_fs == C, "calibration frame stride: 0 (shared) or the camera count");
  const ScanShape sh = joint_argmax_all_shape(T * C, Hh, Wh, Jp);
  hipLaunchKernelGGL(views2d_final_kernel, dim3(T * C), dim3(round_up(J, kWave)), 0, s, pmax, pidx, center_hm,
                     valid, mask, pts3d, cam, intr, dist, calib_fs, points2d, conf2d, reproj, err, used, C, J, Jp,
                     sh.slices, Hh, Wh, hw);
  JH_CHECK_HIP(hipGetLastError());
  return 0;
}

__device__ __forceinline__ float softplus_f(float x) { return x > 20.f ? x : log1pf(expf(x)); }

__global__ __launch_bounds__(256) void softargmax_partial_kernel(
    const float* __restrict__ x, double* __restrict__ partial, int* __restrict__ pmax, int Gh,
    int Jp, int ppb) {
  extern __shared__ __attribute__((aligned(16))) float sm[];
  const int q = Jp >> 2, rows = 256 / q, tid = threadIdx.x;
  const bool active = tid < rows * q;
  const int c4 = tid % q, row = tid / q;
  const int t = blockIdx.y;
  const int P = Gh * Gh * Gh;
  const int p0 = blockIdx.x * ppb, p1 = min(P, p0 + ppb);
  float4 s0 = make_float4(0, 0, 0, 0), si = s0, sj = s0, sk = s0, mx = s0;
  if (active) {
    for (int p = p0 + row; p < p1; p += rows) {
      const float4 v = *reinterpret_cast<const float4*>(x + ((size_t)t * P + p) * Jp + c4 * 4);
      const float4 h = make_float4(softplus_f(v.x), softplus_f(v.y), softplus_f(v.z), softplus_f(v.w));
      const float fk = (float)(p % Gh), fj = (float)((p / Gh) % Gh), fi = (float)(p / (Gh * Gh));
      s0.x += h.x; s0.y += h.y; s0.z += h.z; s0.w += h.w;
      si.x += h.x * fi; si.y += h.y * fi; si.z += h.z * fi; si.w += h.w * fi;
      sj.x += h.x * fj; sj.y += h.y * fj; sj.z += h.z * fj; sj.w += h.w * fj;
      sk.x += h.x * fk; sk.y += h.y * fk; sk.z += h.z * fk; sk.w += h.w * fk;
      mx.x = fmaxf(mx.x, h.x); mx.y = fmaxf(mx.y, h.y); mx.z = fmaxf(mx.z, h.z); mx.w = fmaxf(mx.w, h.w);
    }
  }
  if (active) {
    float4* p = reinterpret_cast<float4*>(sm) + ((size_t)row * q + c4) * 5;
    p[0] = s0; p[1] = si; p[2] = sj; p[3] = sk; p[4] = mx;
  }
  __syncthreads();
  for (int i = tid; i < q * 4 * 5; i += 256) {
    const int comp = i & 3, v = (i >> 2) % 5, cq = (i >> 2) / 5;
    const int ch = cq * 4 + comp;
    if (v < 4) {
      float acc = 0.f;
      for (int r = 0; r < rows; ++r) acc += sm[(((size_t)r * q + cq) * 5 + v) * 4 + comp];
      exact_add(partial + (((size_t)t * Jp + ch) * 4 + v) * kLimbs, (double)acc);
    } else {
      float m = 0.f;
      for (int r = 0; r < rows; ++r) m = fmaxf(m, sm[(((size_t)r * q + cq) * 5 + v) * 4 + comp]);
      atomicMax(pmax + (size_t)t * Jp + ch, __float_as_int(m));
    }
  }
}

__global__ void softargmax_final_kernel(const double* __restrict__ partial,
                                        const int* __restrict__ pmax,
                                        const int* __restrict__ center3d, float* __restrict__ points,
                                        float* __restrict__ conf, int J, int Jp, float spacing,
                                        float roi) {
  const int t = blockIdx.x, j = threadIdx.x;
  if (j >= J) return;
  const double* pl = partial + ((size_t)t * Jp + j) * 4 * kLimbs;
  const double p[4] = {exact_read(pl), exact_read(pl + kLimbs), exact_read(pl + 2 * kLimbs),
                       exact_read(pl + 3 * kLimbs)};
  const float norm = (float)p[0];
#pragma unroll
  for (int a = 0; a < 3; ++a) {
    const float idx = __fdiv_rn((float)p[1 + a], norm);
    const float mm = __fadd_rn(__fsub_rn(__fmul_rn(__fmul_rn(idx, spacing), 2.f), __fdiv_rn(roi, 2.f)),
                               (float)center3d[t * 3 + a]);
    points[((size_t)t * J + j) * 3 + a] = mm;
  }
  const float m = __int_as_float(pmax[(size_t)t * Jp + j]);
  conf[(size_t)t * J + j] = __fdiv_rn(fminf(m, 255.f), 255.f);
}

__global__ __launch_bounds__(256) void heatmap_final_kernel(const float* __restrict__ x,
                                                            float* __restrict__ out, int J, int Jp,
                                                            size_t P, int T) {
  const size_t total = (size_t)T * J * P;
  for (size_t i = (size_t)blockIdx.x * blockDim.x + threadIdx.x; i < total;
       i += (size_t)gridDim.x * blockDim.x) {
    const size_t p = i % P;
    const int j = (int)((i / P) % J);
    const size_t t = i / (P * J);
    out[i] = softplus_f(softplus_f(x[(t * P + p) * Jp + j]));
  }
}

int launch_softargmax(const float* x, const int* center3d, double* partial, int* pmax,
                      float* points, float* conf, float* heatmap_final, int T, int J, int Jp,
                      int Gh, float spacing, float roi, hipStream_t s) {
  const int P = Gh * Gh * Gh;
  const int q = Jp / 4;
  JH_REQUIRE(q >= 1 && q <= 64 && J <= 256, "soft-argmax joint count");
  const int rows = 256 / q;
  const size_t pbytes = (size_t)T * Jp * 4 * kLimbs * sizeof(double), mbytes = (size_t)T * Jp * sizeof(int);
  if (reinterpret_cast<char*>(pmax) == reinterpret_cast<char*>(partial) + pbytes) {
    if (launch_zero(partial, pbytes + mbytes, s)) return 1;
  } else {
    if (launch_zero(partial, pbytes, s)) return 1;
    if (launch_zero(pmax, mbytes, s)) return 1;
  }
  const int ppb = rows * 8;
  dim3 grid((P + ppb - 1) / ppb, T);
  hipLaunchKernelGGL(softargmax_partial_kernel, grid, dim3(256), (size_t)rows * q * 20 * sizeof(float),
                     s, x, partial, pmax, Gh, Jp, ppb);
  JH_CHECK_HIP(hipGetLastError());
  hipLaunchKernelGGL(softargmax_final_kernel, dim3(T), dim3(256), 0, s, partial, pmax, center3d,
                     points, conf, J, Jp, spacing, roi);
  JH_CHECK_HIP(hipGetLastError());
  if (heatmap_final) {
    const size_t total = (size_t)T * J * P;
    int blocks = (int)((total + 255) / 256);
    if (blocks > 8192) blocks = 8192;
    hipLaunchKernelGGL(heatmap_final_kernel, dim3(blocks), dim3(256), 0, s, x, heatmap_final, J, Jp,
                       (size_t)P, T);
    JH_CHECK_HIP(hipGetLastError());
  }
  return 0;
}

}
```

jarvis-hybridnet_amd/csrc/nets.h:

```cpp
#pragma once
#include <functional>
#include <map>
#include <string>
#include <vector>
#include "jh_common.h"
#include "preprocess.h"

namespace jh {

int launch_reproject(const float* cam, const float* intr, const float* dist, int calib_fs, const int* center3d,
                     const int* center_hm, const float* heat, float2* coarse, float* vol,
                     int* idx_out, int T, int C, int G, float spacing, int hs, int Jp,
                     int heat_pad, int div255, hipStream_t s, const HeatLayout* layout = nullptr);
int launch_preprocess_resize(const void* frames, const FrameSource& src, float* out, int N, int H, int W, int S,
                             const float* mean, const float* stdv, hipStream_t s,
                             const void* const* frames_cell = nullptr);
int launch_preprocess_crop(const void* frames, const FrameSource& src, const int* center_hm, float* out, int T,
                           int Cloc, int C, int cam0, int H, int W, int B, const float* mean,
                           const float* stdv, hipStream_t s, const void* const* frames_cell = nullptr);
int launch_frames_to_bgr(const void* frames, const FrameSource& src, unsigned char* out, int N, int H, int W,
                         hipStream_t s);
int launch_center_argmax(const float* heat, float* det, int N, int Hh, int Wh, int Cp,
                         hipStream_t s);
int launch_center2d(const float* det, int* center_hm, int* valid, int T, float sx, float sy, int hw,
                    int W, int H, hipStream_t s);
int launch_joint_argmax(const float* heat, const int* center_hm, int* points, float* conf, int T,
                        int J, int Jp, int Hh, int Wh, int hw, hipStream_t s);
int launch_triangulate(const float* det, const float* cam, const float* intr, const float* dist, int calib_fs,
                       float* center3d_f, int* center3d_i, int* center_hm, int* valid, int T, int C,
                       float sx2, float sy2, float wdiv, int hw, int W, int H, hipStream_t s);
int launch_project_points(const float* pts, const float* cam, const float* intr, const float* dist,
                          float* uv, int P, int C, hipStream_t s);
int launch_softargmax(const float* x, const int* center3d, double* partial, int* pmax,
                      float* points, float* conf, float* heatmap_final, int T, int J, int Jp,
                      int Gh, float spacing, float roi, hipStream_t s);

typedef std::map<std::string, std::vector<float>> ParamMap;

class Plan {
 public:
  ~Plan();
  int run(hipStream_t s);
  size_t launches() const { return ops_.size(); }
  size_t device_bytes() const { return bytes_; }
  int precision = precision_mode();
  int norm_block_kb = 0;

 protected:
  int alloc(void** p, size_t bytes);
  int new_act(int N, int D, int H, int W, int C, Act* out);
  size_t scratch(size_t doubles);
  int finish();
  double* sc(size_t off) const { return arena_ + off; }
  int upload(const std::vector<float>& host, float** dev);
  int get(const ParamMap& pm, const std::string& key, size_t numel, const float** out);

  struct Op { std::function<int(hipStream_t)> fn; std::string name; double flops, bytes; };
  std::vector<Op> ops_;
  void push(const std::string& name, double flops, double bytes, std::function<int(hipStream_t)> fn) {
    ops_.push_back(Op{std::move(fn), name, flops, bytes});
  }
  std::vector<void*> owned_;
  std::vector<ConvWeights> convs_;
  double* arena_ = nullptr;
  size_t arena_doubles_ = 0;
  size_t bytes_ = 0;

  int add_conv(const ParamMap& pm, const ConvDesc& d, const std::string& wkey,
               const std::string& bkey, bool transposed, const Act& x, const Act& y,
               const float* gate, bool want_stats, size_t* stats_off, long in_stats_off = -1,
               float in_inv = 0.f, int in_act = 0, const SeGate* se = nullptr, long se_pool_off = -1);
  void add_norm(const Act& x, size_t stats_off, int act, const float* r1, const float* r2,
                float* y, long pool_off, long r1_stats_off = -1);
};

struct Ref {
  Act a;
  long st = -1;
  float inv = 0.f;
  int act = 0;
};

class EffTrackPlan : public Plan {
 public:
  int build(const ParamMap& pm, const std::string& prefix, int size, int J, int N, int H, int W,
            bool want_res1 = false);
  bool stem_fusable = false;
  StemSource stem_src;
  void set_stem_traffic(double bytes);
  int stem_channels() const { return stem_ch_; }
  int node_rows = -1;
  Act input;
  Act heat;
  Act res1;
  int J = 0;
  int stem_op_ = -1, stem_ch_ = 16;

 private:
  int mbconv(const ParamMap& pm, const std::string& p, int stage, int k, int stride, int cin,
             int cout, int expand, Ref* x, Ref* out);
  void materialise(Ref* x);
  int lateral(const ParamMap& pm, const std::string& p, int cout, const Ref& x, Ref* out);
  int pool(const Ref& x, Ref* out);
  int node(const ParamMap& pm, const std::string& conv_prefix, int n_in, const Ref* ins,
           const int* modes, const float* w, int act, const Act& like, int cout, Ref* out,
           Ref* pooled = nullptr);
};

class V2VPlan : public Plan {
 public:
  int build(const ParamMap& pm, const std::string& prefix, int J, int T, int G);
  Act input;
  Act output;

 private:
  int res_block(const ParamMap& pm, const std::string& p, int c, const Act& x, const float* extra,
                Act* out, long x_stats = -1);
};

}
```

jarvis-hybridnet_amd/csrc/nets.hip:

```cpp
#include <cmath>
#include <cstring>
#include <cstdlib>
#include "nets.h"
#include "bifpn_node.h"
#include "conv3d_wino.h"

namespace jh {

Profiler& profiler() {
  static Profiler p;
  return p;
}
void Profiler::begin(const std::string& name, double flops, double bytes, hipStream_t s) {
  ProfRec r{name, flops, bytes, nullptr, nullptr, 0.f};
  (void)hipEventCreate(&r.e0);
  (void)hipEventCreate(&r.e1);
  (void)hipEventRecord(r.e0, s);
  recs.push_back(r);
}
void Profiler::end(hipStream_t s) { (void)hipEventRecord(recs.back().e1, s); }
int Profiler::finish() {
  JH_CHECK_HIP(hipDeviceSynchronize());
  for (auto& r : recs) {
    if (!r.e0) continue;
    JH_CHECK_HIP(hipEventElapsedTime(&r.ms, r.e0, r.e1));
    (void)hipEventDestroy(r.e0);
    (void)hipEventDestroy(r.e1);
    r.e0 = r.e1 = nullptr;
  }
  return 0;
}

Plan::~Plan() {
  for (void* p : owned_) (void)hipFree(p);
  for (auto& c : convs_) free_conv_weights(&c);
}

int Plan::alloc(void** p, size_t bytes) {
  JH_CHECK_HIP(hipMalloc(p, bytes));
  owned_.push_back(*p);
  bytes_ += bytes;
  return 0;
}

int Plan::new_act(int N, int D, int H, int W, int C, Act* out) {
  out->N = N; out->D = D; out->H = H; out->W = W; out->C = C; out->Cp = cpad(C);
  if (alloc(reinterpret_cast<void**>(&out->p), out->bytes())) return 1;
  JH_CHECK_HIP(hipMemset(out->p, 0, out->bytes()));
  return 0;
}

size_t Plan::scratch(size_t doubles) {
  const size_t off = arena_doubles_;
  arena_doubles_ += (doubles + 7) / 8 * 8;
  return off;
}

int Plan::finish() {
  if (arena_doubles_ == 0) arena_doubles_ = 8;
  return alloc(reinterpret_cast<void**>(&arena_), arena_doubles_ * sizeof(double));
}

static int g_precision = [] {
  const char* e = getenv("JH_PRECISION");
  if (!e) return 0;
  return std::string(e) == "bf16x3" ? 1 : (std::string(e) == "bf16x3_wide" ? 2 : 0);
}();
int precision_mode() { return g_precision; }
void set_precision_mode(int m) { g_precision = m; }

int Plan::run(hipStream_t s) {
  if (launch_zero(arena_, arena_doubles_ * sizeof(double), s)) return 1;
  Profiler& pf = profiler();
  for (auto& op : ops_) {
    if (pf.on) pf.begin(op.name, op.flops, op.bytes, s);
    if (op.fn(s)) return 1;
    if (pf.on) pf.end(s);
  }
  return 0;
}

int Plan::upload(const std::vector<float>& host, float** dev) {
  if (alloc(reinterpret_cast<void**>(dev), host.size() * sizeof(float))) return 1;
  JH_CHECK_HIP(hipMemcpy(*dev, host.data(), host.size() * sizeof(float), hipMemcpyHostToDevice));
  return 0;
}

int Plan::get(const ParamMap& pm, const std::string& key, size_t numel, const float** out) {
  auto it = pm.find(key);
  JH_REQUIRE(it != pm.end(), "missing parameter " + key);
  JH_REQUIRE(it->second.size() == numel, "wrong element count for parameter " + key);
  *out = it->second.data();
  return 0;
}

int Plan::add_conv(const ParamMap& pm, const ConvDesc& d, const std::string& wkey,
                   const std::string& bkey, bool transposed, const Act& x, const Act& y,
                   const float* gate, bool want_stats, size_t* stats_off, long in_stats_off,
                   float in_inv, int in_act, const SeGate* se, long se_pool_off) {
  size_t taps;
  if (d.ostride > 1) taps = (d.nd == 2) ? 16 : 8;
  else taps = (size_t)d.k * d.k * (d.nd == 3 ? d.k : 1);
  const float *w = nullptr, *b = nullptr;
  ConvDesc dd = d;
  dd.latency_class = norm_block_kb == 0 ? 1 : 0;
  if (get(pm, wkey, (size_t)d.cin * d.cout * taps, &w)) return 1;
  if (!bkey.empty() && get(pm, bkey, d.cout, &b)) return 1;
  bool wino = d.nd == 3 && d.k == 3 && d.stride == 1 && d.ostride == 1 && !transposed && !gate;
  if (const char* e = getenv("JH_WINO")) wino = wino && atoi(e) != 0;
  const int wino_variant = wino ? wino_variant_from_env() : 0;
  const bool b3 = wino && precision >= 1;
  const bool d4b = d.nd == 2 && d.ostride > 1 && transposed && !b && !want_stats && !gate &&
                   precision >= 1 && deconv4_bf16x3_eligible(d.cout);
  const bool xb = !wino && !d4b && !transposed && !gate && !se && conv_bf16x3_eligible(d) && x.Cp == cpad(d.cin) &&
                  (precision == 2 || (precision == 1 && d.nd == 3));
  ConvWeights cw;
  if (xb) {
    if (pack_conv_bf16x3_weights(d, w, b, &cw)) return 1;
  } else if (d4b) {
    if (pack_deconv4_bf16x3_weights(d.cin, d.cout, w, &cw)) return 1;
  } else if (b3) {
    if (pack_bf16x3_weights(d.cin, d.cout, w, b, &cw)) return 1;
  } else if (wino) {
    if (pack_wino_weights(d.cin, d.cout, w, b, &cw)) return 1;
  } else {
    if (pack_conv_weights(d, w, b, transposed, &cw)) return 1;
  }
  convs_.push_back(cw);
  bytes_ += cw.phase_stride * d.nphase * sizeof(float);
  size_t off = 0;
  if (want_stats) {
    off = scratch((size_t)y.N * y.Cp * kStatW);
    if (stats_off) *stats_off = off;
  }
  const double opix = (double)y.N * y.pixels();
  const double taps_per_out = (d.ostride > 1) ? (double)taps / d.nphase : (double)taps;
  const double flops = 2.0 * opix * d.cin * d.cout * taps_per_out;
  const double bytes = 4.0 * ((double)x.N * x.pixels() * d.cin + opix * d.cout + (double)d.cin * d.cout * taps);
  const int* wino_tiles = nullptr;
  if (wino && !b3) {
    const std::vector<int> tt = wino_tables(y.D, y.H, y.W, x.Cp);
    if (!tt.empty()) {
      void* dev = nullptr;
      if (alloc(&dev, tt.size() * sizeof(int))) return 1;
      JH_CHECK_HIP(hipMemcpy(dev, tt.data(), tt.size() * sizeof(int), hipMemcpyHostToDevice));
      wino_tiles = static_cast<const int*>(dev);
    }
  }
  char nm[96];
  snprintf(nm, sizeof nm, "conv%dd_k%ds%d%s_%dx%d@%d", d.nd, d.ostride > 1 ? (d.nd == 2 ? 4 : 2) : d.k,
           d.ostride > 1 ? 2 : d.stride, d.ostride > 1 ? (d4b ? "Tbf16x3" : "T") : (b3 || xb ? "bf16x3" : (wino ? "wino" : "")), d.cin, d.cout, y.W);
  push(nm, flops, bytes,
       [this, d = dd, cw, x, y, gate, want_stats, off, in_stats_off, in_inv, in_act, wino, wino_variant, b3, d4b, xb,
        wino_tiles, sev = se ? *se : SeGate(), se_pool_off](hipStream_t s) {
    InNorm in;
    if (in_stats_off >= 0) { in.stats = sc((size_t)in_stats_off); in.inv = in_inv; in.act = in_act; }
    SeGate seg = sev;
    if (se_pool_off >= 0) seg.pool = sc((size_t)se_pool_off);
    if (xb) return launch_conv_bf16x3(d, cw, x, y, want_stats ? sc(off) : nullptr, s, &in);
    if (d4b) return launch_deconv4_bf16x3(cw, x, y, s, &in);
    if (b3) return launch_conv3d_bf16x3(cw, x, y, want_stats ? sc(off) : nullptr, s, &in);
    if (wino) return launch_conv3d_wino(cw, x, y, want_stats ? sc(off) : nullptr, s, &in, wino_variant, wino_tiles);
    return launch_conv(d, cw, x, y, gate, want_stats ? sc(off) : nullptr, s, &in, se_pool_off >= 0 ? &seg : nullptr);
  });
  return 0;
}

void Plan::add_norm(const Act& x, size_t stats_off, int act, const float* r1, const float* r2,
                    float* y, long pool_off, long r1_stats_off) {
  const double el = (double)x.N * x.pixels() * x.C;
  push("norm_apply", 8.0 * el, 4.0 * el * (1 + (y ? 1 : 0) + (r1 ? 1 : 0) + (r2 ? 1 : 0)),
       [this, x, stats_off, act, r1, r2, y, pool_off, r1_stats_off](hipStream_t s) {
    return launch_norm_apply(x, sc(stats_off), 1e-5, act, r1, r2, y,
                             pool_off >= 0 ? sc((size_t)pool_off) : nullptr, s,
                             r1_stats_off >= 0 ? sc((size_t)r1_stats_off) : nullptr, norm_block_kb);
  });
}

namespace {
struct SizeSpec { double width, depth; int fpn, cells, head; };
const SizeSpec kSizes[3] = {{0.5, 0.5, 56, 3, 64}, {1.0, 1.0, 88, 4, 88}, {1.1, 1.2, 160, 6, 160}};
const int kStages[7][6] = {{3, 1, 32, 16, 1, 1}, {3, 2, 16, 24, 6, 2}, {5, 2, 24, 40, 6, 2},
                           {3, 3, 40, 80, 6, 2}, {5, 3, 80, 112, 6, 1}, {5, 4, 112, 192, 6, 2},
                           {3, 1, 192, 320, 6, 1}};
struct Block { int stage, k, stride, cin, cout, expand; };

int scale_ch(int c, double width) {
  const double f = c * width;
  int o = std::max(8, (int)(f + 4) / 8 * 8);
  if (o < 0.9 * f) o += 8;
  return o;
}

void trunk(int size, int* stem, std::vector<Block>* blocks, int taps[3]) {
  const SizeSpec& s = kSizes[size];
  std::vector<Block> all;
  for (int st = 0; st < 7; ++st) {
    const int cin = scale_ch(kStages[st][2], s.width), cout = scale_ch(kStages[st][3], s.width);
    const int rep = (int)std::ceil(s.depth * kStages[st][1]);
    for (int r = 0; r < rep; ++r)
      all.push_back({st, kStages[st][0], r == 0 ? kStages[st][5] : 1, r == 0 ? cin : cout, cout,
                     kStages[st][4]});
  }
  int seen = 0, nt = 0;
  for (size_t i = 0; i < all.size() && nt < 3; ++i)
    if (all[i].stride == 2 && seen++ >= 1) taps[nt++] = (int)i - 1;
  blocks->assign(all.begin(), all.begin() + taps[2] + 1);
  *stem = scale_ch(32, s.width);
}

void fuse_weights(const float* p, int n, float* w) {
  float r[3], sum = 0.f;
  for (int i = 0; i < n; ++i) { r[i] = p[i] > 0.f ? p[i] : 0.f; sum += r[i]; }
  for (int i = 0; i < n; ++i) w[i] = r[i] / (sum + 1e-4f);
}
}

void EffTrackPlan::materialise(Ref* x) {
  if (x->st < 0) return;
  add_norm(x->a, (size_t)x->st, x->act, nullptr, nullptr, x->a.p, -1);
  x->st = -1;
}

int EffTrackPlan::mbconv(const ParamMap& pm, const std::string& p, int stage, int k, int stride,
                         int cin, int cout, int expand, Ref* xin, Ref* outr) {
  const bool skip = (stride == 1 && cin == cout);
  if (skip || (stage >= 4 && expand == 1)) materialise(xin);
  const Ref xr = *xin;
  const Act& x = xr.a;
  Act* out = &outr->a;
// ... 179 lines not shown
  st = scratch((size_t)N * stem * kStatW);
  const Act xin = input, xo = x.a;
  const double opix = (double)N * xo.pixels();
  stem_op_ = (int)ops_.size();
  stem_ch_ = stem;
  push("stem_conv_k3s2_3x" + std::to_string(stem) + "@" + std::to_string(xo.W), 2.0 * opix * 27 * stem,
       4.0 * ((double)N * xin.pixels() * 3 + opix * stem + 27 * stem),
       [this, xin, xo, wd, st](hipStream_t s) {
         if (stem_src.mode) return launch_stem_conv_src(stem_src, xin, wd, xo, sc(st), s);
         return launch_stem_conv(xin, wd, xo, sc(st), s);
       });
  const char* fuse = getenv("JH_STEM_FUSE");
  stem_fusable = !(fuse && atoi(fuse) == 0);
  x.st = (long)st;
  x.inv = 1.f / (float)((H / 2) * (W / 2));
  x.act = ACT_SILU;
  std::vector<Ref> outs(blocks.size() + 1);
  outs[0] = x;
  for (size_t i = 0; i < blocks.size(); ++i) {
    const Block& b = blocks[i];
    if (mbconv(pm, bb + "_blocks." + std::to_string(i) + ".", b.stage, b.k, b.stride, b.cin,
               b.cout, b.expand, &outs[i], &outs[i + 1])) return 1;
  }
  Ref feats[3];
  for (int f = 0; f < 3; ++f) {
    JH_REQUIRE(taps[f] >= 0 && taps[f] < (int)blocks.size(), "feature taps");
    feats[f] = outs[taps[f] + 1];
  }

  const int Wf = ss.fpn;
  Ref p3, p4, p5, p6, p7;
  for (int cell = 0; cell < ss.cells; ++cell) {
    const std::string p = pre + "bifpn." + std::to_string(cell) + ".";
    Ref p3_in, p4_in, p5_in, p6_in, p7_in, p4_in2, p5_in2;
    if (cell == 0) {
      Ref t6;
      if (lateral(pm, p + "p5_to_p6", Wf, feats[2], &t6)) return 1;
      if (pool(t6, &p6_in)) return 1;
      if (pool(p6_in, &p7_in)) return 1;
      if (lateral(pm, p + "p3_down_channel", Wf, feats[0], &p3_in)) return 1;
      if (lateral(pm, p + "p4_down_channel", Wf, feats[1], &p4_in)) return 1;
      if (lateral(pm, p + "p5_down_channel", Wf, feats[2], &p5_in)) return 1;
      if (lateral(pm, p + "p4_down_channel_2", Wf, feats[1], &p4_in2)) return 1;
      if (lateral(pm, p + "p5_down_channel_2", Wf, feats[2], &p5_in2)) return 1;
    } else {
      p3_in = p3; p4_in = p4; p5_in = p5; p6_in = p6; p7_in = p7;
      p4_in2 = p4; p5_in2 = p5;
    }
    auto fnode = [&](const char* wname, int n_in, const Ref* ins, const int* modes, const Ref& like,
                     const char* conv, Ref* out, Ref* pooled = nullptr) -> int {
      const float* wp = nullptr;
      if (get(pm, p + wname, n_in, &wp)) return 1;
      float w[3];
      fuse_weights(wp, n_in, w);
      return node(pm, p + conv + ".", n_in, ins, modes, w, ACT_SILU, like.a, Wf, out, pooled);
    };
    const int m_up[2] = {FUSE_SAME, FUSE_UP2};
    const int m_dn3[3] = {FUSE_SAME, FUSE_SAME, FUSE_POOL2};
    const int m_dn2[2] = {FUSE_SAME, FUSE_POOL2};
    Ref p6_up, p5_up, p4_up, p3_out, p4_out, p5_out, p6_out, p7_out;
    { const Ref in[2] = {p6_in, p7_in}; if (fnode("p6_w1", 2, in, m_up, p6_in, "conv6_up", &p6_up)) return 1; }
    { const Ref in[2] = {p5_in, p6_up}; if (fnode("p5_w1", 2, in, m_up, p5_in, "conv5_up", &p5_up)) return 1; }
    { const Ref in[2] = {p4_in, p5_up}; if (fnode("p4_w1", 2, in, m_up, p4_in, "conv4_up", &p4_up)) return 1; }
    Ref p3_pool;
    { const Ref in[2] = {p3_in, p4_up}; if (fnode("p3_w1", 2, in, m_up, p3_in, "conv3_up", &p3_out, &p3_pool)) return 1; }
    const int m_same3[3] = {FUSE_SAME, FUSE_SAME, FUSE_SAME};
    Ref p4_pool;
    if (p3_pool.a.p) {
      const Ref in[3] = {p4_in2, p4_up, p3_pool};
      if (fnode("p4_w2", 3, in, m_same3, p4_in2, "conv4_down", &p4_out, &p4_pool)) return 1;
    } else {
      const Ref in[3] = {p4_in2, p4_up, p3_out};
      if (fnode("p4_w2", 3, in, m_dn3, p4_in2, "conv4_down", &p4_out)) return 1;
    }
    const bool more = cell + 1 < ss.cells;
    Ref p5_pool, p6_pool;
    if (p4_pool.a.p) {
      const Ref in[3] = {p5_in2, p5_up, p4_pool};
      if (fnode("p5_w2", 3, in, m_same3, p5_in2, "conv5_down", &p5_out, more ? &p5_pool : nullptr)) return 1;
    } else {
      const Ref in[3] = {p5_in2, p5_up, p4_out};
      if (fnode("p5_w2", 3, in, m_dn3, p5_in2, "conv5_down", &p5_out)) return 1;
    }
    if (more) {
      if (p5_pool.a.p) {
        const Ref in[3] = {p6_in, p6_up, p5_pool};
        if (fnode("p6_w2", 3, in, m_same3, p6_in, "conv6_down", &p6_out, &p6_pool)) return 1;
      } else {
        const Ref in[3] = {p6_in, p6_up, p5_out};
        if (fnode("p6_w2", 3, in, m_dn3, p6_in, "conv6_down", &p6_out)) return 1;
      }
      if (p6_pool.a.p) {
        const int m_same2[2] = {FUSE_SAME, FUSE_SAME};
        const Ref in[2] = {p7_in, p6_pool};
        if (fnode("p7_w2", 2, in, m_same2, p7_in, "conv7_down", &p7_out)) return 1;
      } else {
        const Ref in[2] = {p7_in, p6_out};
        if (fnode("p7_w2", 2, in, m_dn2, p7_in, "conv7_down", &p7_out)) return 1;
      }
    }
    p3 = p3_out; p4 = p4_out; p5 = p5_out; p6 = p6_out; p7 = p7_out;
  }

  const float* wc = nullptr;
  if (get(pm, pre + "weights_cat", 3, &wc)) return 1;
  float w[3], sum = 0.f;
  for (int i = 0; i < 3; ++i) { w[i] = wc[i] > 20.f ? wc[i] : log1pf(expf(wc[i])); sum += w[i]; }
  for (int i = 0; i < 3; ++i) w[i] = w[i] / (sum + 0.0001f);
  const Ref hin[3] = {p3, p4, p5};
  const int hmodes[3] = {FUSE_SAME, FUSE_UP2, FUSE_UP4};
  Ref mid;
  if (node(pm, pre + "first_conv.", 3, hin, hmodes, w, ACT_NONE, p3.a, ss.head, &mid)) return 1;
  if (new_act(N, 1, mid.a.H * 2, mid.a.W * 2, J, &heat)) return 1;
  if (want_res1) {
    if (new_act(N, 1, mid.a.H, mid.a.W, J, &res1)) return 1;
    if (add_conv(pm, conv_desc(2, 3, 1, 1, ss.head, J), pre + "final_conv1.weight", "", false, mid.a,
                 res1, nullptr, false, nullptr, mid.st, mid.inv, ACT_NONE)) return 1;
  }
  if (J == 1) {
    const float* wh = nullptr;
    if (get(pm, pre + "deconv1.weight", (size_t)ss.head * 16, &wh)) return 1;
    std::vector<float> wt((size_t)16 * mid.a.Cp, 0.f);
    for (int c = 0; c < ss.head; ++c)
      for (int t = 0; t < 16; ++t) wt[(size_t)t * mid.a.Cp + c] = wh[(size_t)c * 16 + t];
    float* wd = nullptr;
    if (upload(wt, &wd)) return 1;
    const Act m = mid.a, h = heat;
    const long mst = mid.st;
    const float minv = mid.inv;
    push("deconv_k4s2T_c1", 2.0 * N * h.pixels() * ss.head * 4,
         4.0 * N * (m.pixels() * ss.head + (double)h.pixels() * h.Cp), [this, m, h, mst, minv, wd](hipStream_t s) {
      return launch_deconv_c1(m, mst >= 0 ? sc((size_t)mst) : nullptr, minv, ACT_NONE, wd, h, s);
    });
    return finish();
  }
  if (add_conv(pm, deconv2d_k4s2p1_desc(ss.head, J), pre + "deconv1.weight", "", true, mid.a, heat,
               nullptr, false, nullptr, mid.st, mid.inv, ACT_NONE)) return 1;
  return finish();
}

int V2VPlan::res_block(const ParamMap& pm, const std::string& p, int c, const Act& x,
                       const float* extra, Act* out, long x_stats) {
  Act a;
  if (new_act(x.N, x.D, x.H, x.W, c, &a)) return 1;
  size_t s1 = 0, s2 = 0;
  const float inv = 1.f / (float)(x.D * x.H * x.W);
  if (add_conv(pm, conv_desc(3, 3, 1, 1, c, c), p + "res_branch.0.weight", p + "res_branch.0.bias",
               false, x, a, nullptr, true, &s1, x_stats, inv, ACT_RELU)) return 1;
  if (new_act(x.N, x.D, x.H, x.W, c, out)) return 1;
  if (add_conv(pm, conv_desc(3, 3, 1, 1, c, c), p + "res_branch.3.weight", p + "res_branch.3.bias",
               false, a, *out, nullptr, true, &s2, (long)s1, 1.f / (float)(x.D * x.H * x.W),
               ACT_RELU)) return 1;
  add_norm(*out, s2, ACT_RELU, x.p, extra, out->p, -1, x_stats);
  return 0;
}

int V2VPlan::build(const ParamMap& pm, const std::string& pre, int J, int T, int G) {
  JH_REQUIRE(G % 4 == 0, "grid size must be a multiple of 4");
  const int Gh = G / 2, Gq = G / 4;
  if (new_act(T, G, G, G, J, &input)) return 1;
  Act f0, f1, skip, e0, e1, u0, d1;
  size_t st = 0;
  if (new_act(T, Gh, Gh, Gh, 2 * J, &f0)) return 1;
  if (add_conv(pm, conv_desc(3, 3, 2, 1, J, 2 * J), pre + "front_layers.0.block.0.weight",
               pre + "front_layers.0.block.0.bias", false, input, f0, nullptr, true, &st)) return 1;
  if (res_block(pm, pre + "front_layers.1.", 2 * J, f0, nullptr, &f1, (long)st)) return 1;
  const std::string e = pre + "encoder_decoder.";
  if (res_block(pm, e + "skip_res1.", 2 * J, f1, nullptr, &skip)) return 1;
  if (new_act(T, Gq, Gq, Gq, 4 * J, &e0)) return 1;
  if (add_conv(pm, conv_desc(3, 2, 2, 0, 2 * J, 4 * J), e + "encoder_pool1.block.0.weight",
               e + "encoder_pool1.block.0.bias", false, f1, e0, nullptr, true, &st)) return 1;
  if (res_block(pm, e + "mid_res.", 4 * J, e0, nullptr, &e1, (long)st)) return 1;
  if (new_act(T, Gh, Gh, Gh, 2 * J, &u0)) return 1;
  if (add_conv(pm, deconv3d_k2s2_desc(4 * J, 2 * J), e + "decoder_upsample1.block.0.weight",
               e + "decoder_upsample1.block.0.bias", true, e1, u0, nullptr, true, &st)) return 1;
  if (res_block(pm, e + "decoder_res1.", 2 * J, u0, skip.p, &d1, (long)st)) return 1;
  if (new_act(T, Gh, Gh, Gh, J, &output)) return 1;
  if (add_conv(pm, conv_desc(3, 1, 1, 0, 2 * J, J), pre + "output_layer.weight",
               pre + "output_layer.bias", false, d1, output, nullptr, false, nullptr)) return 1;
  return finish();
}

}
```

Measured before the change: 2131 multi-view frames/s.

## Fuse V2V final norm, output 1x1 conv and soft-argmax into one tail kernel

Adds a fused tail kernel for the V2V network. In one pass over LDS tiles it applies the last residual-block normalisation and residual adds, runs the 1x1x1 output convolution with MFMA, and accumulates the soft-argmax partial sums. This avoids writing the decoder activation and the V2V output volume to global memory and reading them back, and drops several launches. The path is on by default when no final heatmap is requested, and it needs a large dynamic LDS allocation, which may lower occupancy.

```diff
diff --git a/include/jarvis_hip.h b/include/jarvis_hip.h
--- a/include/jarvis_hip.h
+++ b/include/jarvis_hip.h
@@ -34,6 +34,10 @@
 typedef struct jh_v2v jh_v2v;
 int jh_v2v_create(const jh_params* p, const char* prefix, int joints, int t, int g, jh_v2v** out);
 int jh_v2v_forward(jh_v2v* net, const float* x_dev, float* y_dev, void* stream);
+int64_t jh_v2v_points_workspace_bytes(const jh_v2v* net);
+int jh_v2v_forward_points(jh_v2v* net, const float* x_dev, const int32_t* center3d_dev, float grid_spacing,
+                          float roi_cube_size, float* points_dev, float* conf_dev, void* workspace_dev,
+                          int64_t workspace_bytes, void* stream);
 void jh_v2v_destroy(jh_v2v* net);
 
 int64_t jh_reproject_workspace_bytes(int cams, int joints, int hs, int grid_size);
@@ -102,6 +106,8 @@
                          float* conf_dev, int32_t* valid_dev, void* stream);
 int jh_predictor_set_graph_replay(jh_predictor* pr, int on);
 int jh_predictor_graph_replay(const jh_predictor* pr);
+int jh_predictor_set_fused_tail(jh_predictor* pr, int on);
+int jh_predictor_fused_tail(const jh_predictor* pr);
 int jh_predictor_stage_center_u8(jh_predictor* pr, const uint8_t* frames_dev, float* det_dev,
                                  void* stream);
 int jh_predictor_stage_keypoints_u8(jh_predictor* pr, const uint8_t* frames_dev,
diff --git a/jarvis-hybridnet_amd/_native.py b/jarvis-hybridnet_amd/_native.py
--- a/jarvis-hybridnet_amd/_native.py
+++ b/jarvis-hybridnet_amd/_native.py
@@ -71,6 +71,9 @@
     "jh_efftrack_destroy": (None, [c_void_p]),
     "jh_v2v_create": (c_int, [c_void_p, c_char_p, c_int, c_int, c_int, ctypes.POINTER(c_void_p)]),
     "jh_v2v_forward": (c_int, [c_void_p, c_void_p, c_void_p, c_void_p]),
+    "jh_v2v_points_workspace_bytes": (c_int64, [c_void_p]),
+    "jh_v2v_forward_points": (c_int, [c_void_p, c_void_p, c_void_p, c_float, c_float, c_void_p, c_void_p, c_void_p,
+                                      c_int64, c_void_p]),
     "jh_v2v_destroy": (None, [c_void_p]),
     "jh_reproject_workspace_bytes": (c_int64, [c_int, c_int, c_int, c_int]),
     "jh_reproject_forward": (c_int, [c_void_p, c_int, c_int, c_int, c_void_p, c_void_p, c_void_p,
@@ -89,6 +92,8 @@
     "jh_predictor_destroy": (None, [c_void_p]),
     "jh_predictor_set_graph_replay": (c_int, [c_void_p, c_int]),
     "jh_predictor_graph_replay": (c_int, [c_void_p]),
+    "jh_predictor_set_fused_tail": (c_int, [c_void_p, c_int]),
+    "jh_predictor_fused_tail": (c_int, [c_void_p]),
     "jh_predictor_launches": (c_int64, [c_void_p]),
     "jh_predictor_device_bytes": (c_int64, [c_void_p]),
     "jh_predictor_precision": (c_int, [c_void_p]),
diff --git a/jarvis-hybridnet_amd/_predictor.py b/jarvis-hybridnet_amd/_predictor.py
--- a/jarvis-hybridnet_amd/_predictor.py
+++ b/jarvis-hybridnet_amd/_predictor.py
@@ -49,6 +49,14 @@
     @graph_replay.setter
     def graph_replay(self, on):
         N.check(N.lib().jh_predictor_set_graph_replay(self.handle, int(bool(on))))
+
+    @property
+    def fused_tail(self):
+        return bool(N.lib().jh_predictor_fused_tail(self.handle))
+
+    @fused_tail.setter
+    def fused_tail(self, on):
+        N.check(N.lib().jh_predictor_set_fused_tail(self.handle, int(bool(on))))
 
     def set_calibration(self, cam, intr, dist):
         N.check(N.lib().jh_predictor_set_calibration(
diff --git a/jarvis-hybridnet_amd/csrc/api.hip b/jarvis-hybridnet_amd/csrc/api.hip
--- a/jarvis-hybridnet_amd/csrc/api.hip
+++ b/jarvis-hybridnet_amd/csrc/api.hip
@@ -184,6 +184,28 @@
   if (launch_to_channel_last(x_dev, net->plan.input, s)) return 1;
   if (net->plan.run(s)) return 1;
   return launch_from_channel_last(net->plan.output, y_dev, s);
+}
+int64_t jh_v2v_points_workspace_bytes(const jh_v2v* net) {
+  if (!net) return 0;
+  Carver c(nullptr, 0);
+  const Act& o = net->plan.output;
+  c.take<double>((size_t)o.N * o.Cp * 4 * kLimbs);
+  c.take<int>((size_t)o.N * o.Cp);
+  return (int64_t)c.off;
+}
+int jh_v2v_forward_points(jh_v2v* net, const float* x_dev, const int32_t* center3d_dev, float grid_spacing,
+                          float roi_cube_size, float* points_dev, float* conf_dev, void* workspace_dev,
+                          int64_t workspace_bytes, void* stream) {
+  hipStream_t s = static_cast<hipStream_t>(stream);
+  JH_REQUIRE(net && x_dev && center3d_dev && points_dev && conf_dev, "bad argument");
+  JH_REQUIRE(workspace_dev && workspace_bytes >= 0, "workspace (see jh_v2v_points_workspace_bytes)");
+  Carver c(workspace_dev, (size_t)workspace_bytes);
+  const Act& o = net->plan.output;
+  double* partial = c.take<double>((size_t)o.N * o.Cp * 4 * kLimbs);
+  int* pmax = c.take<int>((size_t)o.N * o.Cp);
+  JH_REQUIRE(c.fits(), "workspace smaller than jh_v2v_points_workspace_bytes()");
+  if (launch_to_channel_last(x_dev, net->plan.input, s)) return 1;
+  return net->plan.run_points(center3d_dev, partial, pmax, points_dev, conf_dev, grid_spacing, roi_cube_size, s);
 }
 void jh_v2v_destroy(jh_v2v* net) { delete net; }
 
@@ -427,6 +449,7 @@
   double* sa_partial = nullptr;
   int* sa_max = nullptr;
   int use_graph = 0;
+  int fused_tail = 1;
   const void** frames_cell = nullptr;
   const void* const* cur_cell = nullptr;
   const void** frames_table = nullptr;
@@ -434,7 +457,7 @@
   float *g_points = nullptr, *g_conf = nullptr;
   hipStream_t gstream = nullptr;
   static constexpr int kGraphFmts = kSrcSensor + 1;
-  struct GraphSlot { hipGraphExec_t exec = nullptr; FrameSource src; int calib_fs = 0; };
+  struct GraphSlot { hipGraphExec_t exec = nullptr; FrameSource src; int calib_fs = 0, fused_tail = 1; };
   GraphSlot gslot[4 * kGraphFmts];
   unsigned char* mask_buf = nullptr;
   const unsigned char* mask_cur = nullptr;
@@ -462,6 +485,9 @@
                              cfg.grid_spacing, hs, Jp,
                              0, 1, s, layout));
     }
+    if (!heatmap_final && fused_tail)
+      return v2v->run_points(c3i_cur() + t0 * 3, sa_partial, sa_max, points, conf, cfg.grid_spacing,
+                             cfg.roi_cube_size, s);
     if (v2v->run(s)) return 1;
     JH_PROF("softargmax", 0.0, 4.0 * T3 * (g3 / 8) * J,
             launch_softargmax(v2v->output.p, c3i_cur() + t0 * 3, sa_partial, sa_max, points, conf,
@@ -561,6 +587,13 @@
 }
 int jh_predictor_graph_replay(const jh_predictor* pr) { return pr ? pr->use_graph : 0; }
 
+int jh_predictor_set_fused_tail(jh_predictor* pr, int on) {
+  JH_REQUIRE(pr, "bad argument");
+  pr->fused_tail = on != 0;
+  return 0;
+}
+int jh_predictor_fused_tail(const jh_predictor* pr) { return pr ? pr->fused_tail : 0; }
+
 int64_t jh_predictor_launches(const jh_predictor* pr) {
   return (int64_t)((pr->center ? pr->center->launches() : 0) + pr->kp->launches() +
                    pr->v2v->launches());
@@ -747,7 +780,7 @@
                          float* conf_dev, int32_t* valid_dev, hipStream_t s) {
   jh_predictor::GraphSlot& slot = pr->gslot[fs.fmt + (pr->mask_cur ? jh_predictor::kGraphFmts : 0) +
                                             (fs.per_image ? 2 * jh_predictor::kGraphFmts : 0)];
-  if (slot.exec && (slot.src != fs || slot.calib_fs != pr->calib_fs)) {
+  if (slot.exec && (slot.src != fs || slot.calib_fs != pr->calib_fs || slot.fused_tail != pr->fused_tail)) {
     JH_CHECK_HIP(hipStreamSynchronize(s));
     (void)hipGraphExecDestroy(slot.exec);
     slot.exec = nullptr;
@@ -768,6 +801,7 @@
     JH_CHECK_HIP(ei);
     slot.src = fs;
     slot.calib_fs = pr->calib_fs;
+    slot.fused_tail = pr->fused_tail;
   }
   if (!fs.per_image) hipLaunchKernelGGL(set_cell_kernel, dim3(1), dim3(1), 0, s, pr->frames_cell, frames_dev);
   JH_CHECK_HIP(hipGetLastError());
diff --git a/jarvis-hybridnet_amd/csrc/elementwise.hip b/jarvis-hybridnet_amd/csrc/elementwise.hip
--- a/jarvis-hybridnet_amd/csrc/elementwise.hip
+++ b/jarvis-hybridnet_amd/csrc/elementwise.hip
@@ -1,4 +1,5 @@
 #include "jh_common.h"
+#include "norm_elem.h"
 
 namespace jh {
 
@@ -42,14 +43,8 @@
   float4 mean = make_float4(0, 0, 0, 0), rstd = make_float4(1, 1, 1, 1);
   if (stats) {
     float* mr = sm + (pool ? rows * q * 4 : 0);
-    for (int c = tid; c < Cp; c += BT) {
-      const double* st = stats + ((size_t)n * Cp + c) * kStatW;
-      const double mu = exact_read(st) / (double)P;
-      double var = exact_read(st + kLimbs) / (double)P - mu * mu;
-      if (var < 0.0) var = 0.0;
-      mr[c] = (float)mu;
-      mr[Cp + c] = (float)(1.0 / sqrt(var + eps));
-    }
+    for (int c = tid; c < Cp; c += BT)
+      norm_mean_rstd(stats + ((size_t)n * Cp + c) * kStatW, P, eps, mr + c, mr + Cp + c);
     __syncthreads();
     if (active) {
       mean = *reinterpret_cast<const float4*>(mr + c4 * 4);
@@ -60,14 +55,8 @@
   float4 mean1 = make_float4(0, 0, 0, 0), rstd1 = make_float4(1, 1, 1, 1);
   if (R1N) {
     float* mr = sm + (pool ? rows * q * 4 : 0);
-    for (int c = tid; c < Cp; c += BT) {
-      const double* st = stats1 + ((size_t)n * Cp + c) * kStatW;
-      const double mu = exact_read(st) / (double)P;
-      double var = exact_read(st + kLimbs) / (double)P - mu * mu;
-      if (var < 0.0) var = 0.0;
-      mr[c] = (float)mu;
-      mr[Cp + c] = (float)(1.0 / sqrt(var + eps));
-    }
+    for (int c = tid; c < Cp; c += BT)
+      norm_mean_rstd(stats1 + ((size_t)n * Cp + c) * kStatW, P, eps, mr + c, mr + Cp + c);
     __syncthreads();
     if (active) {
       mean1 = *reinterpret_cast<const float4*>(mr + c4 * 4);
@@ -79,21 +68,8 @@
   const int p0 = blockIdx.x * ppb;
   const int p1 = min(P, p0 + ppb);
   float4 ps = make_float4(0, 0, 0, 0);
-  auto act1 = [](float v) __attribute__((always_inline)) {
-    if (ACT == ACT_RELU) return fmaxf(v, 0.f);
-    if (ACT == ACT_SILU) return silu_fast(v);
-    return v;
-  };
   auto finish = [&](float4 v, float4 a1, float4 a2, size_t off) __attribute__((always_inline)) {
-    v.x = (v.x - mean.x) * rstd.x; v.y = (v.y - mean.y) * rstd.y;
-    v.z = (v.z - mean.z) * rstd.z; v.w = (v.w - mean.w) * rstd.w;
-    if (R1N) {
-      a1.x = fmaxf((a1.x - mean1.x) * rstd1.x, 0.f); a1.y = fmaxf((a1.y - mean1.y) * rstd1.y, 0.f);
-      a1.z = fmaxf((a1.z - mean1.z) * rstd1.z, 0.f); a1.w = fmaxf((a1.w - mean1.w) * rstd1.w, 0.f);
-    }
-    if (R1) { v.x += a1.x; v.y += a1.y; v.z += a1.z; v.w += a1.w; }
-    v.x = act1(v.x); v.y = act1(v.y); v.z = act1(v.z); v.w = act1(v.w);
-    if (R2) { v.x += a2.x; v.y += a2.y; v.z += a2.z; v.w += a2.w; }
+    v = norm_residual<ACT, R1, R2, R1N>(v, mean, rstd, a1, mean1, rstd1, a2);
     if (Y) *reinterpret_cast<float4*>(y + off) = v;
     ps.x += v.x; ps.y += v.y; ps.z += v.z; ps.w += v.w;
   };
diff --git a/jarvis-hybridnet_amd/csrc/geometry.hip b/jarvis-hybridnet_amd/csrc/geometry.hip
--- a/jarvis-hybridnet_amd/csrc/geometry.hip
+++ b/jarvis-hybridnet_amd/csrc/geometry.hip
@@ -2,6 +2,7 @@
 #include "preprocess.h"
 #include "camera_mask.h"
 #include "views2d.h"
+#include "softargmax_chunk.h"
 
 namespace jh {
 
@@ -624,49 +625,17 @@
   return 0;
 }
 
-__device__ __forceinline__ float softplus_f(float x) { return x > 20.f ? x : log1pf(expf(x)); }
-
 __global__ __launch_bounds__(256) void softargmax_partial_kernel(
     const float* __restrict__ x, double* __restrict__ partial, int* __restrict__ pmax, int Gh,
     int Jp, int ppb) {
   extern __shared__ __attribute__((aligned(16))) float sm[];
-  const int q = Jp >> 2, rows = 256 / q, tid = threadIdx.x;
-  const bool active = tid < rows * q;
-  const int c4 = tid % q, row = tid / q;
+  const int c4 = threadIdx.x % (Jp >> 2);
   const int t = blockIdx.y;
   const int P = Gh * Gh * Gh;
   const int p0 = blockIdx.x * ppb, p1 = min(P, p0 + ppb);
-  float4 s0 = make_float4(0, 0, 0, 0), si = s0, sj = s0, sk = s0, mx = s0;
-  if (active) {
-    for (int p = p0 + row; p < p1; p += rows) {
-      const float4 v = *reinterpret_cast<const float4*>(x + ((size_t)t * P + p) * Jp + c4 * 4);
-      const float4 h = make_float4(softplus_f(v.x), softplus_f(v.y), softplus_f(v.z), softplus_f(v.w));
-      const float fk = (float)(p % Gh), fj = (float)((p / Gh) % Gh), fi = (float)(p / (Gh * Gh));
-      s0.x += h.x; s0.y += h.y; s0.z += h.z; s0.w += h.w;
-      si.x += h.x * fi; si.y += h.y * fi; si.z += h.z * fi; si.w += h.w * fi;
-      sj.x += h.x * fj; sj.y += h.y * fj; sj.z += h.z * fj; sj.w += h.w * fj;
-      sk.x += h.x * fk; sk.y += h.y * fk; sk.z += h.z * fk; sk.w += h.w * fk;
-      mx.x = fmaxf(mx.x, h.x); mx.y = fmaxf(mx.y, h.y); mx.z = fmaxf(mx.z, h.z); mx.w = fmaxf(mx.w, h.w);
-    }
-  }
-  if (active) {
-    float4* p = reinterpret_cast<float4*>(sm) + ((size_t)row * q + c4) * 5;
-    p[0] = s0; p[1] = si; p[2] = sj; p[3] = sk; p[4] = mx;
-  }
-  __syncthreads();
-  for (int i = tid; i < q * 4 * 5; i += 256) {
-    const int comp = i & 3, v = (i >> 2) % 5, cq = (i >> 2) / 5;
-    const int ch = cq * 4 + comp;
-    if (v < 4) {
-      float acc = 0.f;
-      for (int r = 0; r < rows; ++r) acc += sm[(((size_t)r * q + cq) * 5 + v) * 4 + comp];
-      exact_add(partial + (((size_t)t * Jp + ch) * 4 + v) * kLimbs, (double)acc);
-    } else {
-      float m = 0.f;
-      for (int r = 0; r < rows; ++r) m = fmaxf(m, sm[(((size_t)r * q + cq) * 5 + v) * 4 + comp]);
-      atomicMax(pmax + (size_t)t * Jp + ch, __float_as_int(m));
-    }
-  }
+  softargmax_chunk<false>(
+      [&](int p) { return *reinterpret_cast<const float4*>(x + ((size_t)t * P + p) * Jp + c4 * 4); }, partial, pmax,
+      Gh, Jp, t, p0, p1, sm);
 }
 
 __global__ void softargmax_final_kernel(const double* __restrict__ partial,
@@ -704,6 +673,23 @@
   }
 }
 
+int launch_softargmax_zero(double* partial, int* pmax, int T, int Jp, hipStream_t s) {
+  const size_t pbytes = (size_t)T * Jp * 4 * kLimbs * sizeof(double), mbytes = (size_t)T * Jp * sizeof(int);
+  if (reinterpret_cast<char*>(pmax) == reinterpret_cast<char*>(partial) + pbytes)
+    return launch_zero(partial, pbytes + mbytes, s);
+  if (launch_zero(partial, pbytes, s)) return 1;
+  return launch_zero(pmax, mbytes, s);
+}
+
+int launch_softargmax_final(const double* partial, const int* pmax, const int* center3d, float* points, float* conf,
+                            int T, int J, int Jp, float spacing, float roi, hipStream_t s) {
+  JH_REQUIRE(J <= 256, "soft-argmax joint count");
+  hipLaunchKernelGGL(softargmax_final_kernel, dim3(T), dim3(256), 0, s, partial, pmax, center3d,
+                     points, conf, J, Jp, spacing, roi);
+  JH_CHECK_HIP(hipGetLastError());
+  return 0;
+}
+
 int launch_softargmax(const float* x, const int* center3d, double* partial, int* pmax,
                       float* points, float* conf, float* heatmap_final, int T, int J, int Jp,
                       int Gh, float spacing, float roi, hipStream_t s) {
@@ -711,21 +697,13 @@
   const int q = Jp / 4;
   JH_REQUIRE(q >= 1 && q <= 64 && J <= 256, "soft-argmax joint count");
   const int rows = 256 / q;
-  const size_t pbytes = (size_t)T * Jp * 4 * kLimbs * sizeof(double), mbytes = (size_t)T * Jp * sizeof(int);
-  if (reinterpret_cast<char*>(pmax) == reinterpret_cast<char*>(partial) + pbytes) {
-    if (launch_zero(partial, pbytes + mbytes, s)) return 1;
-  } else {
-    if (launch_zero(partial, pbytes, s)) return 1;
-    if (launch_zero(pmax, mbytes, s)) return 1;
-  }
-  const int ppb = rows * 8;
+  if (launch_softargmax_zero(partial, pmax, T, Jp, s)) return 1;
+  const int ppb = softargmax_ppb(Jp);
   dim3 grid((P + ppb - 1) / ppb, T);
   hipLaunchKernelGGL(softargmax_partial_kernel, grid, dim3(256), (size_t)rows * q * 20 * sizeof(float),
                      s, x, partial, pmax, Gh, Jp, ppb);
   JH_CHECK_HIP(hipGetLastError());
-  hipLaunchKernelGGL(softargmax_final_kernel, dim3(T), dim3(256), 0, s, partial, pmax, center3d,
-                     points, conf, J, Jp, spacing, roi);
-  JH_CHECK_HIP(hipGetLastError());
+  if (launch_softargmax_final(partial, pmax, center3d, points, conf, T, J, Jp, spacing, roi, s)) return 1;
   if (heatmap_final) {
     const size_t total = (size_t)T * J * P;
     int blocks = (int)((total + 255) / 256);
diff --git a/jarvis-hybridnet_amd/csrc/nets.h b/jarvis-hybridnet_amd/csrc/nets.h
--- a/jarvis-hybridnet_amd/csrc/nets.h
+++ b/jarvis-hybridnet_amd/csrc/nets.h
@@ -35,12 +35,26 @@
                       float* points, float* conf, float* heatmap_final, int T, int J, int Jp,
                       int Gh, float spacing, float roi, hipStream_t s);
 
+int launch_softargmax_zero(double* partial, int* pmax, int T, int Jp, hipStream_t s);
+int launch_softargmax_final(const double* partial, const int* pmax, const int* center3d, float* points, float* conf,
+                            int T, int J, int Jp, float spacing, float roi, hipStream_t s);
+
+struct V2VTailArgs {
+  const float *c2_skip, *f1, *c2_dec, *u0;
+  const double *st_skip, *st_dec, *st_u0;
+  const float *w, *bias;
+  int Gh, Cp, Jp, cout_p16;
+  int ppb;
+};
+bool v2v_tail_eligible(int Cp, int Jp, int cout_p16);
+int launch_v2v_tail(const V2VTailArgs& a, double* partial, int* pmax, int T, hipStream_t s);
+
 typedef std::map<std::string, std::vector<float>> ParamMap;
 
 class Plan {
  public:
   ~Plan();
-  int run(hipStream_t s);
+  int run(hipStream_t s, bool points_only = false);
   size_t launches() const { return ops_.size(); }
   size_t device_bytes() const { return bytes_; }
   int precision = precision_mode();
@@ -55,7 +69,7 @@
   int upload(const std::vector<float>& host, float** dev);
   int get(const ParamMap& pm, const std::string& key, size_t numel, const float** out);
 
-  struct Op { std::function<int(hipStream_t)> fn; std::string name; double flops, bytes; };
+  struct Op { std::function<int(hipStream_t)> fn; std::string name; double flops, bytes; bool tail = false; };
   std::vector<Op> ops_;
   void push(const std::string& name, double flops, double bytes, std::function<int(hipStream_t)> fn) {
     ops_.push_back(Op{std::move(fn), name, flops, bytes});
@@ -112,8 +126,16 @@
   int build(const ParamMap& pm, const std::string& prefix, int J, int T, int G);
   Act input;
   Act output;
+  int run_points(const int* center3d, double* partial, int* pmax, float* points, float* conf, float spacing,
+                 float roi, hipStream_t s);
 
  private:
+  V2VTailArgs tail_{};
+  size_t tail_st_[3] = {0, 0, 0};
+  bool tail_ok_ = false;
+  std::string tail_name_;
+  int J_ = 0;
+  size_t res_stats_ = 0;
   int res_block(const ParamMap& pm, const std::string& p, int c, const Act& x, const float* extra,
                 Act* out, long x_stats = -1);
 };
diff --git a/jarvis-hybridnet_amd/csrc/nets.hip b/jarvis-hybridnet_amd/csrc/nets.hip
--- a/jarvis-hybridnet_amd/csrc/nets.hip
+++ b/jarvis-hybridnet_amd/csrc/nets.hip
@@ -69,13 +69,15 @@
 int precision_mode() { return g_precision; }
 void set_precision_mode(int m) { g_precision = m; }
 
-int Plan::run(hipStream_t s) {
+int Plan::run(hipStream_t s, bool points_only) {
   if (launch_zero(arena_, arena_doubles_ * sizeof(double), s)) return 1;
   Profiler& pf = profiler();
   for (auto& op : ops_) {
+    if (points_only && op.tail) continue;
     if (pf.on) pf.begin(op.name, op.flops, op.bytes, s);
-    if (op.fn(s)) return 1;
+    const int rc = op.fn(s);
     if (pf.on) pf.end(s);
+    if (rc) return 1;
   }
   return 0;
 }
@@ -561,6 +563,7 @@
                false, a, *out, nullptr, true, &s2, (long)s1, 1.f / (float)(x.D * x.H * x.W),
                ACT_RELU)) return 1;
   add_norm(*out, s2, ACT_RELU, x.p, extra, out->p, -1, x_stats);
+  res_stats_ = s2;
   return 0;
 }
 
@@ -576,6 +579,8 @@
   if (res_block(pm, pre + "front_layers.1.", 2 * J, f0, nullptr, &f1, (long)st)) return 1;
   const std::string e = pre + "encoder_decoder.";
   if (res_block(pm, e + "skip_res1.", 2 * J, f1, nullptr, &skip)) return 1;
+  const size_t skip_close = ops_.size() - 1;
+  tail_st_[0] = res_stats_;
   if (new_act(T, Gq, Gq, Gq, 4 * J, &e0)) return 1;
   if (add_conv(pm, conv_desc(3, 2, 2, 0, 2 * J, 4 * J), e + "encoder_pool1.block.0.weight",
                e + "encoder_pool1.block.0.bias", false, f1, e0, nullptr, true, &st)) return 1;
@@ -584,10 +589,51 @@
   if (add_conv(pm, deconv3d_k2s2_desc(4 * J, 2 * J), e + "decoder_upsample1.block.0.weight",
                e + "decoder_upsample1.block.0.bias", true, e1, u0, nullptr, true, &st)) return 1;
   if (res_block(pm, e + "decoder_res1.", 2 * J, u0, skip.p, &d1, (long)st)) return 1;
+  const size_t dec_close = ops_.size() - 1;
+  tail_st_[1] = res_stats_;
+  tail_st_[2] = st;
   if (new_act(T, Gh, Gh, Gh, J, &output)) return 1;
   if (add_conv(pm, conv_desc(3, 1, 1, 0, 2 * J, J), pre + "output_layer.weight",
                pre + "output_layer.bias", false, d1, output, nullptr, false, nullptr)) return 1;
+  const ConvWeights& ow = convs_.back();
+  J_ = J;
+  tail_ = V2VTailArgs{skip.p, f1.p, d1.p, u0.p, nullptr, nullptr, nullptr, ow.w, ow.bias,
+                      Gh, d1.Cp, output.Cp, ow.cout_p16, 0};
+  tail_ok_ = ow.paired == 0 && ow.cin_p == d1.Cp && v2v_tail_eligible(d1.Cp, output.Cp, ow.cout_p16);
+  if (tail_ok_) {
+    ops_[skip_close].tail = ops_[dec_close].tail = ops_.back().tail = true;
+    char nm[64];
+    snprintf(nm, sizeof nm, "v2v_tail_%dx%d@%d", 2 * J, J, Gh);
+    tail_name_ = nm;
+  }
   return finish();
 }
 
-}
+int V2VPlan::run_points(const int* center3d, double* partial, int* pmax, float* points, float* conf, float spacing,
+                        float roi, hipStream_t s) {
+  const int T = output.N, Gh = output.D, Jp = output.Cp;
+  const double vox = (double)T * Gh * Gh * Gh;
+  Profiler& pf = profiler();
+  if (!tail_ok_) {
+    if (run(s)) return 1;
+    if (pf.on) pf.begin("softargmax", 0.0, 4.0 * vox * J_, s);
+    const int rc = launch_softargmax(output.p, center3d, partial, pmax, points, conf, nullptr, T, J_, Jp, Gh, spacing,
+                                     roi, s);
+    if (pf.on) pf.end(s);
+    return rc;
+  }
+  if (run(s, true)) return 1;
+  V2VTailArgs a = tail_;
+  a.st_skip = sc(tail_st_[0]); a.st_dec = sc(tail_st_[1]); a.st_u0 = sc(tail_st_[2]);
+  if (launch_softargmax_zero(partial, pmax, T, Jp, s)) return 1;
+  if (pf.on) pf.begin(tail_name_, 2.0 * vox * 2 * J_ * J_, 4.0 * vox * 2 * J_ * 4, s);
+  int rc = launch_v2v_tail(a, partial, pmax, T, s);
+  if (pf.on) pf.end(s);
+  if (rc) return 1;
+  if (pf.on) pf.begin("softargmax_final", 0.0, 4.0 * T * J_ * 4 * 4, s);
+  rc = launch_softargmax_final(partial, pmax, center3d, points, conf, T, J_, Jp, spacing, roi, s);
+  if (pf.on) pf.end(s);
+  return rc;
+}
+
+}
diff --git a/jarvis-hybridnet_amd/csrc/norm_elem.h b/jarvis-hybridnet_amd/csrc/norm_elem.h
--- /dev/null
+++ b/jarvis-hybridnet_amd/csrc/norm_elem.h
@@ -0,0 +1,34 @@
+#pragma once
+#include "jh_common.h"
+
+namespace jh {
+
+__device__ __forceinline__ void norm_mean_rstd(const double* st, int P, double eps, float* mean, float* rstd) {
+  const double mu = exact_read(st) / (double)P;
+  double var = exact_read(st + kLimbs) / (double)P - mu * mu;
+  if (var < 0.0) var = 0.0;
+  *mean = (float)mu;
+  *rstd = (float)(1.0 / sqrt(var + eps));
+}
+
+template <int ACT, bool R1, bool R2, bool R1N>
+__device__ __forceinline__ float4 norm_residual(float4 v, const float4& mean, const float4& rstd, float4 a1,
+                                                const float4& mean1, const float4& rstd1, const float4& a2) {
+  auto act1 = [](float x) __attribute__((always_inline)) {
+    if (ACT == ACT_RELU) return fmaxf(x, 0.f);
+    if (ACT == ACT_SILU) return silu_fast(x);
+    return x;
+  };
+  v.x = (v.x - mean.x) * rstd.x; v.y = (v.y - mean.y) * rstd.y;
+  v.z = (v.z - mean.z) * rstd.z; v.w = (v.w - mean.w) * rstd.w;
+  if (R1N) {
+    a1.x = fmaxf((a1.x - mean1.x) * rstd1.x, 0.f); a1.y = fmaxf((a1.y - mean1.y) * rstd1.y, 0.f);
+    a1.z = fmaxf((a1.z - mean1.z) * rstd1.z, 0.f); a1.w = fmaxf((a1.w - mean1.w) * rstd1.w, 0.f);
+  }
+  if (R1) { v.x += a1.x; v.y += a1.y; v.z += a1.z; v.w += a1.w; }
+  v.x = act1(v.x); v.y = act1(v.y); v.z = act1(v.z); v.w = act1(v.w);
+  if (R2) { v.x += a2.x; v.y += a2.y; v.z += a2.z; v.w += a2.w; }
+  return v;
+}
+
+}
diff --git a/jarvis-hybridnet_amd/csrc/softargmax_chunk.h b/jarvis-hybridnet_amd/csrc/softargmax_chunk.h
--- /dev/null
+++ b/jarvis-hybridnet_amd/csrc/softargmax_chunk.h
@@ -0,0 +1,50 @@
+#pragma once
+#include "jh_common.h"
+
+namespace jh {
+
+__device__ __forceinline__ float softplus_f(float x) { return x > 20.f ? x : log1pf(expf(x)); }
+
+inline int softargmax_ppb(int Jp) { return (256 / (Jp / 4)) * 8; }
+
+template <bool SYNC, class LOAD>
+__device__ __forceinline__ void softargmax_chunk(LOAD load, double* __restrict__ partial, int* __restrict__ pmax,
+                                                 int Gh, int Jp, int t, int p0, int p1, float* sm) {
+  const int q = Jp >> 2, rows = 256 / q, tid = threadIdx.x;
+  const bool active = tid < rows * q;
+  const int c4 = tid % q, row = tid / q;
+  float4 s0 = make_float4(0, 0, 0, 0), si = s0, sj = s0, sk = s0, mx = s0;
+  if (active) {
+    for (int p = p0 + row; p < p1; p += rows) {
+      const float4 v = load(p);
+      const float4 h = make_float4(softplus_f(v.x), softplus_f(v.y), softplus_f(v.z), softplus_f(v.w));
+      const float fk = (float)(p % Gh), fj = (float)((p / Gh) % Gh), fi = (float)(p / (Gh * Gh));
+      s0.x += h.x; s0.y += h.y; s0.z += h.z; s0.w += h.w;
+      si.x += h.x * fi; si.y += h.y * fi; si.z += h.z * fi; si.w += h.w * fi;
+      sj.x += h.x * fj; sj.y += h.y * fj; sj.z += h.z * fj; sj.w += h.w * fj;
+      sk.x += h.x * fk; sk.y += h.y * fk; sk.z += h.z * fk; sk.w += h.w * fk;
+      mx.x = fmaxf(mx.x, h.x); mx.y = fmaxf(mx.y, h.y); mx.z = fmaxf(mx.z, h.z); mx.w = fmaxf(mx.w, h.w);
+    }
+  }
+  if (SYNC) __syncthreads();
+  if (active) {
+    float4* p = reinterpret_cast<float4*>(sm) + ((size_t)row * q + c4) * 5;
+    p[0] = s0; p[1] = si; p[2] = sj; p[3] = sk; p[4] = mx;
+  }
+  __syncthreads();
+  for (int i = tid; i < q * 4 * 5; i += 256) {
+    const int comp = i & 3, v = (i >> 2) % 5, cq = (i >> 2) / 5;
+    const int ch = cq * 4 + comp;
+    if (v < 4) {
+      float acc = 0.f;
+      for (int r = 0; r < rows; ++r) acc += sm[(((size_t)r * q + cq) * 5 + v) * 4 + comp];
+      exact_add(partial + (((size_t)t * Jp + ch) * 4 + v) * kLimbs, (double)acc);
+    } else {
+      float m = 0.f;
+      for (int r = 0; r < rows; ++r) m = fmaxf(m, sm[(((size_t)r * q + cq) * 5 + v) * 4 + comp]);
+      atomicMax(pmax + (size_t)t * Jp + ch, __float_as_int(m));
+    }
+  }
+}
+
+}
diff --git a/jarvis-hybridnet_amd/csrc/v2v_tail.hip b/jarvis-hybridnet_amd/csrc/v2v_tail.hip
--- /dev/null
+++ b/jarvis-hybridnet_amd/csrc/v2v_tail.hip
@@ -0,0 +1,172 @@
+#include <atomic>
+#include "conv_mfma.h"
+#include "norm_elem.h"
+#include "softargmax_chunk.h"
+#include "nets.h"
+
+namespace jh {
+
+namespace {
+
+template <int NCB> struct TailRbw { static constexpr int value = 16 / NCB; };
+
+template <int NCB>
+__global__ __launch_bounds__(256) void v2v_tail_kernel(const V2VTailArgs a, double* __restrict__ partial,
+                                                       int* __restrict__ pmax) {
+  constexpr int RBW = TailRbw<NCB>::value;
+  extern __shared__ __attribute__((aligned(16))) float sm[];
+  const int Cp = a.Cp, S = Cp + 4, S2 = S >> 1, Q4 = Cp >> 2, Jp = a.Jp;
+  float* nrm = sm;
+  float* tile = sm + 6 * Cp;
+  const int tid = threadIdx.x;
+  const int lane = tid & 63;
+  const int wave = __builtin_amdgcn_readfirstlane(tid >> 6);
+  const int mrow = lane & 15, kq = lane >> 4;
+  const int t = blockIdx.y;
+  const int P = a.Gh * a.Gh * a.Gh;
+  const int p0 = blockIdx.x * a.ppb, p1 = min(P, p0 + a.ppb);
+  const int np = p1 - p0;
+
+  for (int i = tid; i < 3 * Cp; i += 256) {
+    const int k = i / Cp, c = i - k * Cp;
+    const double* st = (k == 0 ? a.st_skip : (k == 1 ? a.st_dec : a.st_u0)) + ((size_t)t * Cp + c) * kStatW;
+    norm_mean_rstd(st, P, 1e-5, nrm + k * 2 * Cp + c, nrm + k * 2 * Cp + Cp + c);
+  }
+  __syncthreads();
+
+  {
+    const size_t base = ((size_t)t * P + p0) * Cp;
+    const float4* __restrict__ xs = reinterpret_cast<const float4*>(a.c2_skip + base);
+    const float4* __restrict__ xf = reinterpret_cast<const float4*>(a.f1 + base);
+    const float4* __restrict__ xd = reinterpret_cast<const float4*>(a.c2_dec + base);
+    const float4* __restrict__ xu = reinterpret_cast<const float4*>(a.u0 + base);
+    const int items = np * Q4;
+    constexpr int UN = 4;
+    const float4 z4 = make_float4(0.f, 0.f, 0.f, 0.f);
+    for (int i0 = tid; i0 < items; i0 += UN * 256) {
+      float4 vs[UN], vf[UN], vd[UN], vu[UN];
+#pragma unroll
+      for (int u = 0; u < UN; ++u) {
+        const int idx = i0 + u * 256;
+        const bool ok = idx < items;
+        vs[u] = ok ? xs[idx] : z4; vf[u] = ok ? xf[idx] : z4; vd[u] = ok ? xd[idx] : z4; vu[u] = ok ? xu[idx] : z4;
+      }
+#pragma unroll
+      for (int u = 0; u < UN; ++u) {
+        const int idx = i0 + u * 256;
+        if (idx < items) {
+          const int pix = idx / Q4, c = (idx - pix * Q4) * 4;
+          const float4 m_s = *reinterpret_cast<const float4*>(nrm + c);
+          const float4 r_s = *reinterpret_cast<const float4*>(nrm + Cp + c);
+          const float4 m_d = *reinterpret_cast<const float4*>(nrm + 2 * Cp + c);
+          const float4 r_d = *reinterpret_cast<const float4*>(nrm + 3 * Cp + c);
+          const float4 m_u = *reinterpret_cast<const float4*>(nrm + 4 * Cp + c);
+          const float4 r_u = *reinterpret_cast<const float4*>(nrm + 5 * Cp + c);
+          const float4 sk = norm_residual<ACT_RELU, true, false, false>(vs[u], m_s, r_s, vf[u], z4, z4, z4);
+          const float4 d = norm_residual<ACT_RELU, true, true, true>(vd[u], m_d, r_d, vu[u], m_u, r_u, sk);
+          *reinterpret_cast<float4*>(tile + pix * S + c) = d;
+        }
+      }
+    }
+  }
+  __syncthreads();
+
+  const int nrb = (np + 15) >> 4;
+  const int nk8 = Cp >> 3;
+  const float2* lds2 = reinterpret_cast<const float2*>(tile);
+  const float2* __restrict__ w2 = reinterpret_cast<const float2*>(a.w);
+  f32x4 acc[RBW][NCB];
+#pragma unroll
+  for (int i = 0; i < RBW; ++i)
+#pragma unroll
+    for (int cb = 0; cb < NCB; ++cb) acc[i][cb] = (f32x4){0.f, 0.f, 0.f, 0.f};
+  for (int k8 = 0; k8 < nk8; ++k8) {
+    float2 b[NCB];
+#pragma unroll
+    for (int cb = 0; cb < NCB; ++cb) b[cb] = w2[(k8 * NCB + cb) * 64 + lane];
+#pragma unroll
+    for (int i = 0; i < RBW; ++i) {
+      const int rb = wave + 4 * i;
+      if (rb < nrb) {
+        const float2 av = lds2[(rb * 16 + mrow) * S2 + k8 * 4 + kq];
+#pragma unroll
+        for (int cb = 0; cb < NCB; ++cb)
+          acc[i][cb] = __builtin_amdgcn_mfma_f32_16x16x4f32(av.x, b[cb].x, acc[i][cb], 0, 0, 0);
+#pragma unroll
+        for (int cb = 0; cb < NCB; ++cb)
+          acc[i][cb] = __builtin_amdgcn_mfma_f32_16x16x4f32(av.y, b[cb].y, acc[i][cb], 0, 0, 0);
+      }
+    }
+  }
+  __syncthreads();
+#pragma unroll
+  for (int cb = 0; cb < NCB; ++cb) {
+    const int ch = cb * 16 + mrow;
+    const float bv = a.bias ? a.bias[ch] : 0.f;
+    if (ch < Jp) {
+#pragma unroll
+      for (int i = 0; i < RBW; ++i) {
+        const int rb = wave + 4 * i;
+        if (rb < nrb) {
+#pragma unroll
+          for (int r = 0; r < 4; ++r) tile[(rb * 16 + kq * 4 + r) * Jp + ch] = acc[i][cb][r] + bv;
+        }
+      }
+    }
+  }
+  __syncthreads();
+
+  const int c4 = tid % (Jp >> 2);
+  softargmax_chunk<true>([&](int p) { return *reinterpret_cast<const float4*>(tile + (p - p0) * Jp + c4 * 4); },
+                         partial, pmax, a.Gh, Jp, t, p0, p1, tile);
+}
+
+template <int NCB>
+int launch_tail_inst(const V2VTailArgs& a, double* partial, int* pmax, dim3 grid, size_t lds, hipStream_t s) {
+  auto kern = v2v_tail_kernel<NCB>;
+  static std::atomic<bool> big[64];
+  if (lds > 64 * 1024) {
+    int devid = 0;
+    JH_CHECK_HIP(hipGetDevice(&devid));
+    if (devid < 0 || devid >= 64 || !big[devid].load(std::memory_order_acquire)) {
+      JH_CHECK_HIP(hipFuncSetAttribute(reinterpret_cast<const void*>(kern),
+                                       hipFuncAttributeMaxDynamicSharedMemorySize, 160 * 1024));
+      if (devid >= 0 && devid < 64) big[devid].store(true, std::memory_order_release);
+    }
+  }
+  hipLaunchKernelGGL(kern, grid, dim3(256), lds, s, a, partial, pmax);
+  JH_CHECK_HIP(hipGetLastError());
+  return 0;
+}
+
+size_t tail_lds_bytes(int Cp, int Jp) {
+  const int ppb16 = round_up(softargmax_ppb(Jp), 16);
+  const size_t d = (size_t)ppb16 * (Cp + 4), red = (size_t)(256 / (Jp / 4)) * (Jp / 4) * 20;
+  return ((size_t)6 * Cp + std::max(d, red)) * sizeof(float);
+}
+
+}
+
+bool v2v_tail_eligible(int Cp, int Jp, int cout_p16) {
+  const int ncb = cout_p16 / 16;
+  if (Jp < 8 || Jp % 8 != 0 || Jp > cout_p16 || ncb < 1 || ncb > 4 || Cp % 8 != 0 || Cp < Jp) return false;
+  const int nrb = (softargmax_ppb(Jp) + 15) / 16;
+  return (nrb + 3) / 4 <= 16 / ncb && tail_lds_bytes(Cp, Jp) <= 160 * 1024;
+}
+
+int launch_v2v_tail(const V2VTailArgs& args, double* partial, int* pmax, int T, hipStream_t s) {
+  JH_REQUIRE(v2v_tail_eligible(args.Cp, args.Jp, args.cout_p16), "v2v tail shape");
+  V2VTailArgs a = args;
+  a.ppb = softargmax_ppb(a.Jp);
+  const int P = a.Gh * a.Gh * a.Gh;
+  const dim3 grid((P + a.ppb - 1) / a.ppb, T);
+  const size_t lds = tail_lds_bytes(a.Cp, a.Jp);
+  switch (a.cout_p16 / 16) {
+    case 1: return launch_tail_inst<1>(a, partial, pmax, grid, lds, s);
+    case 2: return launch_tail_inst<2>(a, partial, pmax, grid, lds, s);
+    case 3: return launch_tail_inst<3>(a, partial, pmax, grid, lds, s);
+    default: return launch_tail_inst<4>(a, partial, pmax, grid, lds, s);
+  }
+}
+
+}
```

After: 2160 multi-view frames/s, median of 6. +1.4%, better.
